# rmcar17/SpectralClusterSupertree

Hardware: AMD Instinct MI355X
Metric: top-level PCG build + Fiedler solve wall-time (s) at N taxa, 1/2/4/8 MI355X (lower is better)
Workload: dtype f64 (loop operator: fp32 image of W; fp64 renewal + confirmation)

## Files before the change

include/scs_hip.h:

```cpp
#ifndef SCS_HIP_H
#define SCS_HIP_H

#include <stddef.h>
#include <stdint.h>

#ifdef __cplusplus
extern "C" {
#endif

#define SCS_OK 0
#define SCS_EINVAL (-1)
#define SCS_EHIP (-2)
#define SCS_ENOMEM (-3)
#define SCS_ECOMM (-4)
#define SCS_ENOCONV (-5)
#define SCS_EUNSUP (-6)

#define SCS_UNIQUE_ID_BYTES 128

typedef struct scs_ctx scs_ctx;
typedef struct scs_tables scs_tables;
typedef struct scs_graph scs_graph;

typedef struct scs_stats {
    int32_t n_vertices;
    int32_t block;
    int32_t iterations;
    int32_t n_apply;
    int32_t converged;
    int32_t used_constraint;
    double lambda[2];
    double resid[2];
    double lambda_next;
    double apply_ms_total;
    double apply_ms_min;
    double solve_ms;
    double apply_bytes;
    double allgather_ms_total;
    double allgather_bytes;
    int32_t n_allgather;
    int32_t n_apply32;
    double apply32_ms_total;
    double apply32_bytes;
    int32_t lowp_renewals;
    int32_t reserved;
    double event_pair_ms;
} scs_stats;

typedef struct scs_build_stats {
    int32_t n_taxa;
    int32_t n_trees;
    int32_t row_begin, row_end;
    int32_t symmetric;
    int32_t n_tiles;
    int32_t n_batches;
    int32_t spec_batches;
    double cell_trees;
    double prep_ms;
    double accumulate_ms;
    double exchange_ms;
    double total_ms;
    double bytes_w;
    double bytes_tables;
    double exchange_bytes;
    int32_t tree_parallel_batches;
    int32_t spec_trees;
    double spec_ms;
    int32_t listed_batches;
    int32_t reserved;
} scs_build_stats;

int scs_version(void);
const char *scs_last_error(void);

int scs_device_count(void);


int scs_comm_unique_id(void *out128);

int scs_ctx_create(int device, int rank, int world, const void *unique_id128, scs_ctx **out);

typedef struct scs_local_group scs_local_group;
int scs_local_group_create(int world, scs_local_group **out);
int scs_local_group_destroy(scs_local_group *group);
int scs_ctx_create_local(int device, int rank, scs_local_group *group, scs_ctx **out);

int scs_ctx_destroy(scs_ctx *ctx);
int scs_ctx_synchronize(scs_ctx *ctx);
int scs_ctx_trim(scs_ctx *ctx, int64_t keep_bytes);
int scs_ctx_reserve(scs_ctx *ctx, int64_t bytes);
int scs_debug_arena_stats(int device, int64_t *out8);
int scs_ctx_comm_info(scs_ctx *ctx, int32_t *kind, int32_t *world, int32_t *rank,
                      int32_t *reported_world, int32_t *reported_rank);


typedef struct scs_forest scs_forest;
typedef struct scs_forest_info {
    int32_t n_trees;
    int32_t monotone;
    int64_t n_nodes;
    int64_t n_leaves;
} scs_forest_info;

int scs_forest_upload(scs_ctx *ctx, int32_t n_taxa, int32_t n_trees, const int64_t *node_off,
                      const int32_t *parent, const int32_t *taxon, const double *length,
                      const double *support, const double *weights, int64_t n_leaves, scs_forest **out);
int scs_forest_free(scs_ctx *ctx, scs_forest *forest);

int scs_forest_split(scs_ctx *ctx, const scs_forest *forest, const int32_t *part_of,
                     const int32_t *new_id, int32_t n_parts, const int32_t *part_taxa, int32_t strategy,
                     scs_forest **out_forests, scs_forest_info *info);

int scs_forest_tables_download(scs_ctx *ctx, const scs_forest *forest, int64_t *tree_off,
                               int32_t *leaf_taxon, int32_t *adj_depth, double *adj_val,
                               int32_t *tree_index, double *tree_w, uint8_t *present);

int scs_forest_tables_host(scs_ctx *ctx, const scs_forest *forest, const int64_t **tree_off,
                           const int32_t **leaf_taxon, const int32_t **adj_depth, const double **adj_val,
                           const int32_t **tree_index, const double **tree_w, const uint8_t **present);

int scs_forest_download(scs_ctx *ctx, const scs_forest *forest, int32_t t_begin, int32_t t_end,
                        int64_t *node_off, int32_t *parent, int32_t *taxon, double *length,
                        double *support, double *weights);

int scs_tables_from_forest(scs_ctx *ctx, const scs_forest *forest, const int32_t *relabel, int32_t n_taxa,
                           scs_tables **out);


int scs_forest_split_level(scs_ctx *ctx, const scs_forest *forest, const int32_t *part_of,
                           const int32_t *new_id, int32_t n_parts, int32_t child_taxa, int32_t strategy,
                           int32_t n_nodes, const int32_t *node_tree_end, scs_forest **out_union,
                           scs_forest_info *info, int32_t *child_trees, int64_t *child_leaves,
                           uint8_t *present, int32_t *comp_root, uint64_t *sig);

int scs_forest_slice(scs_ctx *ctx, const scs_forest *forest, int32_t t_begin, int32_t t_end, scs_forest **out);

int scs_forest_analyze(scs_ctx *ctx, const scs_forest *forest, int32_t *comp_root, uint64_t *sig);

int scs_forest_tables_download_range(scs_ctx *ctx, const scs_forest *forest, int32_t t_begin, int32_t t_end,
                                     int64_t *tree_off, int32_t *leaf_taxon, int32_t *adj_depth,
                                     double *adj_val, double *tree_w);

int scs_tables_from_forest_range(scs_ctx *ctx, const scs_forest *forest, int32_t t_begin, int32_t t_end,
                                 int32_t u_base, int32_t u_size, const int32_t *relabel, int32_t n_taxa,
                                 scs_tables **out);


int scs_host_alloc(size_t bytes, void **out);
int scs_host_free(void *p);

int scs_tables_upload(scs_ctx *ctx, int32_t n_taxa, int32_t n_trees, const int64_t *tree_off,
                      const int32_t *leaf_taxon, const int32_t *adj_depth, const double *adj_val,
                      const double *tree_w, scs_tables **out);
int scs_tables_free(scs_ctx *ctx, scs_tables *tables);


int scs_score_supertree(scs_ctx *ctx, const scs_tables *sources, int32_t n_nodes, const int32_t *parent,
                        const int32_t *taxon, int32_t max_batch_trees, int64_t *n_super, int64_t *n_source,
                        int64_t *shared, int64_t *informative, int64_t *supported);

int scs_score_parsimony(scs_ctx *ctx, const scs_tables *sources, int32_t n_nodes, const int32_t *parent,
                        const int32_t *taxon, int32_t max_batch_trees, int32_t max_pass_words, int64_t *mrp_chars,
                        int64_t *mrp_length, int64_t *mrp_perfect, int64_t *mrp_max, int64_t *char_off,
                        int32_t *char_len, int32_t *char_lo, int32_t *char_hi);

int scs_score_triplets(scs_ctx *ctx, const scs_tables *sources, int32_t n_nodes, const int32_t *parent,
                       const int32_t *taxon, int32_t max_batch_trees, int64_t *t_super, int64_t *t_source,
                       int64_t *t_shared);

int scs_score_conflicts(scs_ctx *ctx, const scs_tables *sources, int32_t n_nodes, const int32_t *parent,
                        const int32_t *taxon, int32_t max_batch_trees, int64_t *n_super_conflict,
                        int64_t *n_source_conflict, int64_t *conflicting);

int scs_score_concordance(scs_ctx *ctx, const scs_tables *sources, int32_t n_nodes, const int32_t *parent,
                          const int32_t *taxon, int32_t max_batch_trees, int64_t *n_decisive, int64_t *n_concordant,
                          int64_t *n_alternative, int64_t *decisive, int64_t *concordant, int64_t *alt1,
                          int64_t *alt2);

int scs_score_branch_triplets(scs_ctx *ctx, const scs_tables *sources, int32_t n_nodes, const int32_t *parent,
                              const int32_t *taxon, int32_t max_batch_trees, int64_t *n_bt_total,
                              int64_t *n_bt_concordant, int64_t *n_bt_alternative, int64_t *bt_total,
                              int64_t *bt_concordant, int64_t *bt_alt1, int64_t *bt_alt2);

int scs_score_taxon_triplets(scs_ctx *ctx, const scs_tables *sources, int32_t n_nodes, const int32_t *parent,
                             const int32_t *taxon, int32_t max_batch_trees, int32_t max_lds_bytes,
                             int64_t *tx_trees, int64_t *tx_total, int64_t *tx_super, int64_t *tx_source,
                             int64_t *tx_shared);

int scs_score_placements(scs_ctx *ctx, const scs_tables *sources, int32_t n_nodes, const int32_t *parent,
                         const int32_t *taxon, int32_t max_batch_trees, int32_t max_lds_bytes, int32_t n_queries,
                         const int32_t *queries, int64_t *pl_trees, int64_t *pl_total, int64_t *pl_source,
                         int64_t *pl_super, int64_t *pl_shared);

int scs_score_clade_placements(scs_ctx *ctx, const scs_tables *sources, int32_t n_nodes, const int32_t *parent,
                               const int32_t *taxon, int32_t max_batch_trees, int32_t max_lds_bytes,
                               int32_t n_queries, const int32_t *query_nodes, int64_t *cp_trees, int64_t *cp_total,
                               int64_t *cp_source, int64_t *cp_super, int64_t *cp_shared);

int scs_score_clade_moves(scs_ctx *ctx, const scs_tables *sources, int32_t n_nodes, const int32_t *parent,
                          const int32_t *taxon, int32_t max_batch_trees, int32_t max_lds_bytes, int32_t n_queries,
                          const int32_t *query_nodes, int32_t top_k, int64_t *cp_trees, int64_t *cp_total,
                          int64_t *cp_source, int64_t *mv_own_super, int64_t *mv_own_shared, int32_t *mv_node,
                          int64_t *mv_super, int64_t *mv_shared);

int scs_score_polytomies(scs_ctx *ctx, const scs_tables *sources, int32_t n_nodes, const int32_t *parent,
                         const int32_t *taxon, int32_t max_batch_trees, int32_t max_lds_bytes, int32_t n_queries,
                         const int32_t *query_nodes, int32_t *py_degree, int64_t *py_trees, int64_t *py_total,
                         int64_t *py_joint);

int scs_score_branch_resample(scs_ctx *ctx, const scs_tables *sources, int32_t n_nodes, const int32_t *parent,
                              const int32_t *taxon, int32_t max_batch_trees, int32_t n_rep, const int32_t *weights,
                              int64_t *rs_point, int32_t *rs_wins, int64_t *rs_rows);


#define SCS_BUILD_MONOTONE 1
#define SCS_BUILD_SHARED 2
#define SCS_BUILD_UPPER 4
#define SCS_BUILD_SCATTER 8
int scs_pcg_build(scs_ctx *ctx, const scs_tables *tables, int32_t row_begin, int32_t row_end,
                  int32_t flags, scs_graph **out, scs_build_stats *stats);

int scs_graph_contract(scs_ctx *ctx, scs_graph *graph, const int32_t *group_start,
                       int32_t n_groups, scs_graph **out);

int scs_graph_shape(const scs_graph *graph, int32_t *n_vertices, int32_t *row_begin,
                    int32_t *row_end);

int scs_graph_download(scs_ctx *ctx, const scs_graph *graph, double *out);

int scs_graph_download_rows(scs_ctx *ctx, const scs_graph *graph, int32_t first, int32_t count,
                            double *out);

int scs_graph_degrees(scs_ctx *ctx, scs_graph *graph, double *out);

int scs_graph_free(scs_ctx *ctx, scs_graph *graph);


int scs_fiedler(scs_ctx *ctx, scs_graph *graph, const double *x_init, double tol,
                int32_t max_iter, int32_t block, double *maps_out, scs_stats *stats);

int scs_graph_matrix_free(scs_ctx *ctx, const scs_tables *tables, int32_t max_block, scs_graph **out);


int scs_small_solve(scs_ctx *ctx, int32_t n_nodes, const int32_t *n_taxa, const int32_t *n_trees,
                    const int32_t *n_groups, const int32_t *tree_off, const int32_t *leaf_taxon,
                    const int32_t *adj_depth, const double *adj_val, const double *tree_w,
                    const int32_t *group_start, double *maps_out, double *lambda_out,
                    double *w_out);

int scs_small_solve_begin(scs_ctx *ctx, int32_t n_nodes, const int32_t *n_taxa,
                          const int32_t *n_trees, const int32_t *n_groups, const int32_t *tree_off,
                          const int32_t *leaf_taxon, const int32_t *adj_depth, const double *adj_val,
                          const double *tree_w, const int32_t *group_start, int32_t want_w,
                          int32_t *ticket_out);
int scs_small_solve_begin_forest(scs_ctx *ctx, const scs_forest *forest, const int32_t *relabel,
                                 int32_t n_taxa, int32_t n_groups, const int32_t *group_start,
                                 int32_t want_w, int32_t *ticket_out);
int scs_small_solve_begin_level(scs_ctx *ctx, const scs_forest *forest, int32_t n_nodes,
                                const int32_t *t_begin, const int32_t *n_trees, const int64_t *n_leaves,
                                const int32_t *u_base, const int32_t *u_size, const int32_t *relabel,
                                const int32_t *n_taxa, const int32_t *n_groups, const int32_t *group_start,
                                int32_t want_w, int32_t *ticket_out);
int scs_small_solve_end(scs_ctx *ctx, int32_t ticket, double *maps_out, double *lambda_out,
                        double *w_out);


int scs_debug_loop_policy(double tol, int32_t lowp_mode, double lowp_tol, double lowp_tol2, int32_t image,
                          int32_t n, const double *residuals, int32_t *actions_out);

int scs_debug_jacobi(scs_ctx *ctx, const double *a, int32_t n, double *w, double *v);

int scs_debug_gram(scs_ctx *ctx, const double *a, const double *b, int32_t n, int32_t ka,
                   int32_t kb, int32_t use_mfma, double *out);

int scs_debug_apply(scs_ctx *ctx, scs_graph *graph, const double *x, int32_t b, double *y);

int scs_debug_apply_ex(scs_ctx *ctx, scs_graph *graph, const double *x, int32_t b, int32_t image,
                       int32_t reps, double *y_out, int32_t *info_out);

int scs_debug_gram_ex(scs_ctx *ctx, const double *a, int32_t lda, int32_t a_col0, int32_t ka,
                      const double *b, int32_t ldb, int32_t b_col0, int32_t kb, int32_t n,
                      int32_t use_mfma, int32_t gram_blocks, double *out);

int scs_debug_update(scs_ctx *ctx, double *y, int32_t ldy, int32_t y_col0, int32_t kc, double alpha,
                     const double *a, int32_t lda, int32_t a_col0, int32_t ka, const double *c,
                     int32_t ldc, double sign, int32_t n);

int scs_debug_comm_selftest(scs_ctx *ctx, int32_t count, const double *host_in, double *host_out);

int scs_debug_copy_bandwidth(scs_ctx *ctx, int64_t bytes, int32_t reps, double *gbs_out);

int scs_debug_scan(scs_ctx *ctx, int32_t op, int32_t n_parts, int64_t n, const int32_t *in, int32_t *out);

int scs_debug_graph_raw(scs_ctx *ctx, scs_graph *graph, int32_t what, void *out, int32_t *info_out);

int scs_debug_split_plan(int32_t n_trees, const int64_t *node_off, int32_t *tpb_out, int32_t *n_groups_out,
                         uint8_t *staged_out);

int scs_debug_score_plan(const scs_tables *sources, int32_t n_trees, const int64_t *tree_off, int32_t super_leaves,
                         int32_t max_batch_trees, int64_t extra_per_leaf, int64_t extra_per_tree,
                         int32_t *n_batches_out, int32_t *bstart_out, int64_t *info_out, int32_t *words_out,
                         int32_t *zb_out, int64_t *wg_out);

int scs_debug_branch_plan(const scs_tables *sources, int32_t n_trees, const int64_t *tree_off, int32_t super_leaves,
                          int32_t max_batch_trees, int64_t extra_per_leaf, int64_t extra_per_tree,
                          int32_t max_lds_bytes, int32_t *n_batches_out, int32_t *bstart_out, int64_t *bt_out,
                          int64_t *tx_out, int64_t *call_out);

int scs_debug_placement_plan(const scs_tables *sources, int32_t n_trees, const int64_t *tree_off, int32_t super_leaves,
                             int32_t max_batch_trees, int32_t max_lds_bytes, int32_t n_queries,
                             int32_t n_sub_queries, int32_t n_degrees, const int32_t *degrees, int32_t *n_batches_out,
                             int32_t *bstart_out, int64_t *pl_out, int64_t *cp_out, int64_t *blk_out, int64_t *py_out);

int scs_debug_parsimony_plan(const scs_tables *sources, int32_t n_trees, const int64_t *tree_off, const int64_t *chars,
                             int32_t n_nodes, const int32_t *parent, int32_t max_batch_trees, int32_t max_pass_words,
                             int32_t *n_batches_out, int32_t *bstart_out, int64_t *info_out, int64_t *batch_out);

#ifdef __cplusplus
}
#endif
#endif
```

spectralclustersupertree_amd/_native.py:

```python

from __future__ import annotations

import ctypes as C
from pathlib import Path

import numpy as np

_PKG = Path(__file__).resolve().parent
LIB_PATH = _PKG / "libscs_hip.so"

UNIQUE_ID_BYTES = 128
BUILD_MONOTONE = 1
BUILD_SHARED = 2
BUILD_UPPER = 4
BUILD_SCATTER = 8


class ScsError(RuntimeError):

    def __init__(self, code: int, message: str) -> None:
        super().__init__(f"libscs_hip error {code}: {message}")
        self.code = code


EINVAL = -1
ENOMEM = -3
ENOCONV = -5
EUNSUP = -6


class ConvergenceError(ScsError):

    def __init__(self, message: str, maps, stats: dict) -> None:
        super().__init__(ENOCONV, message)
        self.maps = maps
        self.stats = stats


class Stats(C.Structure):
    _fields_ = [
        ("n_vertices", C.c_int32),
        ("block", C.c_int32),
        ("iterations", C.c_int32),
        ("n_apply", C.c_int32),
        ("converged", C.c_int32),
        ("used_constraint", C.c_int32),
        ("lambda_", C.c_double * 2),
        ("resid", C.c_double * 2),
        ("lambda_next", C.c_double),
        ("apply_ms_total", C.c_double),
        ("apply_ms_min", C.c_double),
        ("solve_ms", C.c_double),
        ("apply_bytes", C.c_double),
        ("allgather_ms_total", C.c_double),
        ("allgather_bytes", C.c_double),
        ("n_allgather", C.c_int32),
        ("n_apply32", C.c_int32),
        ("apply32_ms_total", C.c_double),
        ("apply32_bytes", C.c_double),
        ("lowp_renewals", C.c_int32),
        ("reserved", C.c_int32),
        ("event_pair_ms", C.c_double),
    ]

    def as_dict(self) -> dict:
        out = {}
        for name, _ in self._fields_:
            v = getattr(self, name)
            out[name.rstrip("_")] = list(v) if hasattr(v, "__len__") else v
        return out


class ForestInfo(C.Structure):
    _fields_ = [
        ("n_trees", C.c_int32),
        ("monotone", C.c_int32),
        ("n_nodes", C.c_int64),
        ("n_leaves", C.c_int64),
    ]


class BuildStats(C.Structure):
    _fields_ = [
        ("n_taxa", C.c_int32),
        ("n_trees", C.c_int32),
        ("row_begin", C.c_int32),
        ("row_end", C.c_int32),
        ("symmetric", C.c_int32),
        ("n_tiles", C.c_int32),
        ("n_batches", C.c_int32),
        ("spec_batches", C.c_int32),
        ("cell_trees", C.c_double),
        ("prep_ms", C.c_double),
        ("accumulate_ms", C.c_double),
        ("exchange_ms", C.c_double),
        ("total_ms", C.c_double),
        ("bytes_w", C.c_double),
        ("bytes_tables", C.c_double),
        ("exchange_bytes", C.c_double),
        ("tree_parallel_batches", C.c_int32),
        ("spec_trees", C.c_int32),
        ("spec_ms", C.c_double),
        ("listed_batches", C.c_int32),
        ("reserved", C.c_int32),
    ]

    def as_dict(self) -> dict:
        return {name: getattr(self, name) for name, _ in self._fields_}


_P = C.c_void_p
_PP = C.POINTER(C.c_void_p)
_I32 = C.c_int32
_DP = _IP = _LP = C.c_void_p
ABI_VERSION = 109

SIGNATURES = {
    "scs_version": (C.c_int, []),
    "scs_last_error": (C.c_char_p, []),
    "scs_device_count": (C.c_int, []),
    "scs_comm_unique_id": (C.c_int, [_P]),
    "scs_ctx_create": (C.c_int, [C.c_int, C.c_int, C.c_int, _P, _PP]),
    "scs_local_group_create": (C.c_int, [C.c_int, _PP]),
    "scs_local_group_destroy": (C.c_int, [_P]),
    "scs_ctx_create_local": (C.c_int, [C.c_int, C.c_int, _P, _PP]),
    "scs_ctx_destroy": (C.c_int, [_P]),
    "scs_ctx_synchronize": (C.c_int, [_P]),
    "scs_ctx_trim": (C.c_int, [_P, C.c_int64]),
    "scs_debug_arena_stats": (C.c_int, [C.c_int, C.POINTER(C.c_int64)]),
    "scs_ctx_reserve": (C.c_int, [_P, C.c_int64]),
    "scs_ctx_comm_info": (C.c_int, [_P, _P, _P, _P, _P, _P]),
    "scs_forest_upload": (C.c_int, [_P, _I32, _I32, _LP, _IP, _IP, _DP, _DP, _DP, C.c_int64, _PP]),
    "scs_forest_free": (C.c_int, [_P, _P]),
    "scs_forest_split": (C.c_int, [_P, _P, _IP, _IP, _I32, _IP, _I32, _P, _P]),
    "scs_forest_tables_download": (C.c_int, [_P, _P, _LP, _IP, _IP, _DP, _IP, _DP, _P]),
    "scs_forest_tables_host": (C.c_int, [_P, _P, _P, _P, _P, _P, _P, _P, _P]),
    "scs_tables_from_forest": (C.c_int, [_P, _P, _IP, _I32, _PP]),
    "scs_forest_download": (C.c_int, [_P, _P, _I32, _I32, _LP, _IP, _IP, _DP, _DP, _DP]),
    "scs_forest_split_level": (C.c_int, [_P, _P, _IP, _IP, _I32, _I32, _I32, _I32, _IP, _PP, _P, _IP, _LP, _P, _IP, _P]),
    "scs_forest_analyze": (C.c_int, [_P, _P, _IP, _P]),
    "scs_forest_slice": (C.c_int, [_P, _P, _I32, _I32, _PP]),
    "scs_forest_tables_download_range": (C.c_int, [_P, _P, _I32, _I32, _LP, _IP, _IP, _DP, _DP]),
    "scs_tables_from_forest_range": (C.c_int, [_P, _P, _I32, _I32, _I32, _I32, _IP, _I32, _PP]),
    "scs_small_solve_begin_level": (C.c_int, [_P, _P, _I32, _IP, _IP, _LP, _IP, _IP, _IP, _IP, _IP, _IP, _I32,
                                              C.POINTER(C.c_int32)]),
    "scs_host_alloc": (C.c_int, [C.c_size_t, _PP]),
    "scs_host_free": (C.c_int, [_P]),
    "scs_tables_upload": (C.c_int, [_P, _I32, _I32, _LP, _IP, _IP, _DP, _DP, _PP]),
    "scs_tables_free": (C.c_int, [_P, _P]),
    "scs_score_supertree": (C.c_int, [_P, _P, _I32, _IP, _IP, _I32, _LP, _LP, _LP, _LP, _LP]),
    "scs_score_triplets": (C.c_int, [_P, _P, _I32, _IP, _IP, _I32, _LP, _LP, _LP]),
    "scs_score_conflicts": (C.c_int, [_P, _P, _I32, _IP, _IP, _I32, _LP, _LP, _LP]),
    "scs_score_concordance": (C.c_int, [_P, _P, _I32, _IP, _IP, _I32, _LP, _LP, _LP, _LP, _LP, _LP, _LP]),
    "scs_score_branch_triplets": (C.c_int, [_P, _P, _I32, _IP, _IP, _I32, _LP, _LP, _LP, _LP, _LP, _LP, _LP]),
    "scs_score_taxon_triplets": (C.c_int, [_P, _P, _I32, _IP, _IP, _I32, _I32, _LP, _LP, _LP, _LP, _LP]),
    "scs_score_placements": (C.c_int, [_P, _P, _I32, _IP, _IP, _I32, _I32, _I32, _IP, _LP, _LP, _LP, _LP, _LP]),
    "scs_score_clade_placements": (C.c_int, [_P, _P, _I32, _IP, _IP, _I32, _I32, _I32, _IP, _LP, _LP, _LP, _LP, _LP]),
    "scs_score_clade_moves": (C.c_int, [_P, _P, _I32, _IP, _IP, _I32, _I32, _I32, _IP, _I32, _LP, _LP, _LP, _LP, _LP,
                                        _IP, _LP, _LP]),
    "scs_score_polytomies": (C.c_int, [_P, _P, _I32, _IP, _IP, _I32, _I32, _I32, _IP, _IP, _LP, _LP, _LP]),
    "scs_score_branch_resample": (C.c_int, [_P, _P, _I32, _IP, _IP, _I32, _I32, _IP, _LP, _IP, _LP]),
    "scs_score_parsimony": (C.c_int, [_P, _P, _I32, _IP, _IP, _I32, _I32, _LP, _LP, _LP, _LP, _LP, _IP, _IP, _IP]),
    "scs_pcg_build": (C.c_int, [_P, _P, _I32, _I32, _I32, _PP, C.POINTER(BuildStats)]),
    "scs_graph_contract": (C.c_int, [_P, _P, _IP, _I32, _PP]),
    "scs_graph_matrix_free": (C.c_int, [_P, _P, _I32, _PP]),
    "scs_graph_shape": (C.c_int, [_P, _IP, _IP, _IP]),
    "scs_graph_download": (C.c_int, [_P, _P, _DP]),
    "scs_graph_download_rows": (C.c_int, [_P, _P, _I32, _I32, _DP]),
    "scs_graph_degrees": (C.c_int, [_P, _P, _DP]),
    "scs_graph_free": (C.c_int, [_P, _P]),
    "scs_fiedler": (C.c_int, [_P, _P, _DP, C.c_double, _I32, _I32, _DP, C.POINTER(Stats)]),
    "scs_small_solve": (C.c_int, [_P, _I32, _IP, _IP, _IP, _IP, _IP, _IP, _DP, _DP, _IP, _DP, _DP, _DP]),
    "scs_small_solve_begin": (C.c_int, [_P, _I32, _IP, _IP, _IP, _IP, _IP, _IP, _DP, _DP, _IP, _I32,
                                        C.POINTER(C.c_int32)]),
    "scs_small_solve_begin_forest": (C.c_int, [_P, _P, _IP, _I32, _I32, _IP, _I32, _P]),
    "scs_small_solve_end": (C.c_int, [_P, _I32, _DP, _DP, _DP]),
    "scs_debug_loop_policy": (C.c_int, [C.c_double, _I32, C.c_double, C.c_double, _I32, _I32, _DP, _IP]),
    "scs_debug_jacobi": (C.c_int, [_P, _DP, _I32, _DP, _DP]),
    "scs_debug_gram": (C.c_int, [_P, _DP, _DP, _I32, _I32, _I32, _I32, _DP]),
    "scs_debug_apply": (C.c_int, [_P, _P, _DP, _I32, _DP]),
    "scs_debug_apply_ex": (C.c_int, [_P, _P, _DP, _I32, _I32, _I32, _DP, _IP]),
    "scs_debug_gram_ex": (C.c_int, [_P, _DP, _I32, _I32, _I32, _DP, _I32, _I32, _I32, _I32, _I32, _I32, _DP]),
    "scs_debug_update": (C.c_int, [_P, _DP, _I32, _I32, _I32, C.c_double, _DP, _I32, _I32, _I32, _DP, _I32,
                                   C.c_double, _I32]),
    "scs_debug_comm_selftest": (C.c_int, [_P, _I32, _DP, _DP]),
    "scs_debug_copy_bandwidth": (C.c_int, [_P, C.c_int64, _I32, _DP]),
    "scs_debug_scan": (C.c_int, [_P, _I32, _I32, C.c_int64, _IP, _IP]),
    "scs_debug_split_plan": (C.c_int, [_I32, _LP, _P, _P, _P]),
    "scs_debug_graph_raw": (C.c_int, [_P, _P, _I32, _P, _IP]),
    "scs_debug_score_plan": (C.c_int, [_P, _I32, _LP, _I32, _I32, C.c_int64, C.c_int64, _P, _IP, _LP, _IP, _IP, _LP]),
    "scs_debug_branch_plan": (C.c_int, [_P, _I32, _LP, _I32, _I32, C.c_int64, C.c_int64, _I32, _P, _IP, _LP, _LP, _LP]),
    "scs_debug_placement_plan": (C.c_int, [_P, _I32, _LP, _I32, _I32, _I32, _I32, _I32, _I32, _IP, _IP, _IP, _LP, _LP,
                                           _LP, _LP]),
    "scs_debug_parsimony_plan": (C.c_int, [_P, _I32, _LP, _LP, _I32, _IP, _I32, _I32, _P, _IP, _LP, _LP]),
}

_lib = None


def load_library() -> C.CDLL:
    global _lib
    if _lib is not None:
        return _lib
    if not LIB_PATH.exists():
        msg = (
            f"{LIB_PATH} not found: build it with `python -c 'import __graft_entry__ as g; g.build()'` "
            "or `make -C spectralclustersupertree_amd/csrc`.  There is no CPU fallback."
        )
        raise ImportError(msg)
    lib = C.CDLL(str(LIB_PATH))
    for name, (restype, argtypes) in SIGNATURES.items():
        fn = getattr(lib, name)
        fn.restype = restype
        fn.argtypes = argtypes
    have = int(lib.scs_version())
    if have != ABI_VERSION:
        msg = f"{LIB_PATH} reports ABI version {have}, this package binds {ABI_VERSION}: rebuild the library"
        raise ImportError(msg)
    _lib = lib
    return lib


def check(rc: int) -> None:
    if rc != 0:
        msg = load_library().scs_last_error()
        raise ScsError(rc, msg.decode() if msg else "unknown error")


class _PinnedBlock:

    def __init__(self, nbytes: int) -> None:
        self._lib = load_library()
        self.ptr = C.c_void_p()
        check(self._lib.scs_host_alloc(nbytes, C.byref(self.ptr)))
        self.nbytes = nbytes

    def __del__(self) -> None:
        try:
            if self.ptr:
                self._lib.scs_host_free(self.ptr)
                self.ptr = C.c_void_p()
        except Exception:
            pass


def pinned_empty(shape, dtype) -> np.ndarray:
    dt = np.dtype(dtype)
    count = int(np.prod(shape)) if np.ndim(shape) else int(shape)
    block = _PinnedBlock(max(count * dt.itemsize, 1))
    buf = (C.c_char * block.nbytes).from_address(block.ptr.value)
    buf._scs_owner = block
    return np.frombuffer(buf, dtype=dt, count=count).reshape(shape)


def dptr(a: np.ndarray):
    assert a.dtype == np.float64
    return a.ctypes.data


def iptr(a: np.ndarray):
    assert a.dtype == np.int32
    return a.ctypes.data


def lptr(a: np.ndarray):
    assert a.dtype == np.int64
    return a.ctypes.data
```

spectralclustersupertree_amd/backend.py:

```python

from __future__ import annotations

import ctypes as C
import os

import numpy as np

from spectralclustersupertree_amd import _env
from spectralclustersupertree_amd import _native as nv
from spectralclustersupertree_amd.flatten import TreeTables

DEFAULT_TOL = 1e-13
DEFAULT_MAX_ITER = 2000

_M, _N, _Q, _QN, _QK = ("m",), ("n_nodes",), ("nq",), ("nq", "n_nodes"), ("nq", "top_k")


def _resident_solve() -> bool:
    return bool(int(_env.probe("SCS_RESIDENT_SOLVE", "1")))


class Device:

    def __init__(self, device: int = 0, rank: int = 0, world: int = 1, unique_id: bytes | None = None,
# ... 435 lines not shown
        return comp_root, sig

    def tables_range(self, t_begin: int, t_end: int):
        m = int(t_end - t_begin)
        tree_off = np.zeros(m + 1, dtype=np.int64)
        nv.check(self.dev._lib.scs_forest_tables_download_range(self.dev._ctx, self._h, int(t_begin), int(t_end),
                                                                nv.lptr(tree_off), None, None, None, None))
        l = int(tree_off[-1])
        leaf_taxon = np.empty(l, dtype=np.int32)
        adj_depth = np.empty(l, dtype=np.int32)
        adj_val = np.empty(l, dtype=np.float64)
        tree_w = np.empty(m, dtype=np.float64)
        nv.check(self.dev._lib.scs_forest_tables_download_range(
            self.dev._ctx, self._h, int(t_begin), int(t_end), nv.lptr(tree_off), nv.iptr(leaf_taxon) if l else None,
            nv.iptr(adj_depth) if l else None, nv.dptr(adj_val) if l else None, nv.dptr(tree_w) if m else None))
        return tree_off, leaf_taxon, adj_depth, adj_val, tree_w

    def tables(self):
        m, l = self.n_trees, self.n_leaves
        ptrs = [C.c_void_p() for _ in range(7)]
        nv.check(self.dev._lib.scs_forest_tables_host(self.dev._ctx, self._h, *[C.byref(x) for x in ptrs]))

        def view(ptr, dtype, count):
            dt = np.dtype(dtype)
            if count == 0:
                return np.empty(0, dtype=dt)
            buf = (C.c_char * (count * dt.itemsize)).from_address(ptr.value)
            buf._scs_owner = self
            a = np.frombuffer(buf, dtype=dt, count=count)
            a.flags.writeable = False
            return a

        return (view(ptrs[0], np.int64, m + 1), view(ptrs[1], np.int32, l), view(ptrs[2], np.int32, l),
                view(ptrs[3], np.float64, l), view(ptrs[4], np.int32, m), view(ptrs[5], np.float64, m),
                view(ptrs[6], np.uint8, max(self.n_taxa, 0)))

    def download(self, t_begin: int = 0, t_end: int | None = None):
        t_end = self.n_trees if t_end is None else t_end
        m = t_end - t_begin
        node_off = np.zeros(m + 1, dtype=np.int64)
        nv.check(self.dev._lib.scs_forest_download(self.dev._ctx, self._h, t_begin, t_end, nv.lptr(node_off),
                                                   None, None, None, None, None))
        n = int(node_off[-1])
        parent = np.empty(n, dtype=np.int32)
        taxon = np.empty(n, dtype=np.int32)
        length = np.empty(n, dtype=np.float64)
        support = np.empty(n, dtype=np.float64)
        weights = np.empty(m, dtype=np.float64)
        nv.check(self.dev._lib.scs_forest_download(self.dev._ctx, self._h, t_begin, t_end, nv.lptr(node_off),
                                                   nv.iptr(parent) if n else None, nv.iptr(taxon) if n else None,
                                                   nv.dptr(length) if n else None, nv.dptr(support) if n else None,
                                                   nv.dptr(weights) if m else None))
        return node_off, parent, taxon, length, support, weights


def debug_split_plan(node_off: np.ndarray):
    node_off = np.ascontiguousarray(node_off, dtype=np.int64)
    m = len(node_off) - 1
    tpb, groups = C.c_int32(0), C.c_int32(0)
    staged = np.zeros((m + 7) // 8 + 1, dtype=np.uint8)
    nv.check(nv.load_library().scs_debug_split_plan(m, nv.lptr(node_off), C.byref(tpb), C.byref(groups), staged.ctypes.data))
    return int(tpb.value), staged[: groups.value].astype(bool)


def debug_score_plan(sources, super_leaves: int, batch_trees: int = 0, extra_per_leaf: int = 0,
                     extra_per_tree: int = 0) -> dict:
    handle, off = (sources._h, None) if isinstance(sources, DeviceTables) else (None, sources)
    if off is not None:
        off = np.ascontiguousarray(off, dtype=np.int64)
    m = sources.n_trees if off is None else len(off) - 1
    nb = C.c_int32(0)
    bstart = np.zeros(m + 1, dtype=np.int32)
    info = np.zeros(2, dtype=np.int64)
    words, zb = np.zeros(max(m, 1), dtype=np.int32), np.zeros(max(m, 1), dtype=np.int32)
    wg = np.zeros(max(m, 1), dtype=np.int64)
    nv.check(nv.load_library().scs_debug_score_plan(
        handle, m, None if off is None else nv.lptr(off), int(super_leaves), int(batch_trees), int(extra_per_leaf),
        int(extra_per_tree), C.byref(nb), nv.iptr(bstart), nv.lptr(info), nv.iptr(words), nv.iptr(zb), nv.lptr(wg)))
    k = int(nb.value)
    return {"bstart": bstart[: k + 1].astype(np.int64), "levels": int(info[0]), "row_stride": int(info[1]),
            "words": words[:k].astype(np.int64), "zb": zb[:k].astype(np.int64), "workgroups": wg[:k].copy()}


def debug_branch_plan(sources, super_leaves: int, batch_trees: int = 0, extra_per_leaf: int = 0,
                      extra_per_tree: int = 0, lds_bytes: int = 0) -> dict:
    handle, off = (sources._h, None) if isinstance(sources, DeviceTables) else (None, sources)
    if off is not None:
        off = np.ascontiguousarray(off, dtype=np.int64)
    m = sources.n_trees if off is None else len(off) - 1
    nb = C.c_int32(0)
    bstart = np.zeros(m + 1, dtype=np.int32)
    bt = np.zeros((max(m, 1), 4), dtype=np.int64)
    tx = np.zeros((max(m, 1), 14), dtype=np.int64)
    call = np.zeros(3, dtype=np.int64)
    nv.check(nv.load_library().scs_debug_branch_plan(
        handle, m, None if off is None else nv.lptr(off), int(super_leaves), int(batch_trees), int(extra_per_leaf),
        int(extra_per_tree), int(lds_bytes), C.byref(nb), nv.iptr(bstart), nv.lptr(bt), nv.lptr(tx), nv.lptr(call)))
    k = int(nb.value)
    bins = tx[:k, :12].reshape(k, 3, 4)
    return {"bstart": bstart[: k + 1].astype(np.int64), "bt_words": bt[:k, 0].copy(), "bt_zb": bt[:k, 1].copy(),
            "bt_lds": bt[:k, 2].copy(), "bt_workgroups": bt[:k, 3].copy(), "tx_zb": bins[:, :, 0].copy(),
            "tx_dcap": bins[:, :, 1].copy(), "tx_lds": bins[:, :, 2].copy(), "tx_workgroups": bins[:, :, 3].copy(),
            "tx_slab_launch": tx[:k, 12].copy(), "tx_slab_lds": tx[:k, 13].copy(), "need_slab": int(call[0]),
            "slab_wgs": int(call[1]),
            "slab_stride": int(call[2])}


def debug_placement_plan(sources, super_leaves: int, batch_trees: int = 0, lds_bytes: int = 0, n_queries: int = 1,
                         n_sub_queries: int = 1, degrees=()) -> dict:
    handle, off = (sources._h, None) if isinstance(sources, DeviceTables) else (None, sources)
    if off is not None:
        off = np.ascontiguousarray(off, dtype=np.int64)
    m = sources.n_trees if off is None else len(off) - 1
    deg = np.ascontiguousarray(degrees, dtype=np.int32)
    nb = np.zeros(3, dtype=np.int32)
    bstart = np.zeros((3, m + 1), dtype=np.int32)
    pair = np.zeros((2, max(m, 1), 6), dtype=np.int64)
    blk = np.zeros((2, m + 1), dtype=np.int64)
    py = np.zeros((max(m, 1), max(len(deg), 1), 4), dtype=np.int64)
    nv.check(nv.load_library().scs_debug_placement_plan(
        handle, m, None if off is None else nv.lptr(off), int(super_leaves), int(batch_trees), int(lds_bytes),
        int(n_queries), int(n_sub_queries), len(deg), nv.iptr(deg) if len(deg) else None, nv.iptr(nb),
        nv.iptr(bstart), nv.lptr(pair[0]), nv.lptr(pair[1]), nv.lptr(blk), nv.lptr(py)))
    out = {}
    for x, name in enumerate(("pl", "cp")):
        k = int(nb[x])
        out[f"{name}_bstart"] = bstart[x, : k + 1].astype(np.int64)
        for i, key in enumerate(("words", "zb", "sums", "lds_full", "lds_last", "workgroups")):
            out[f"{name}_{key}"] = pair[x, :k, i].copy()
        out[f"{name}_blk"] = np.diff(blk[x])
    k = int(nb[2])
    out["py_bstart"] = bstart[2, : k + 1].astype(np.int64)
    rows = py.reshape(-1)[: k * len(deg) * 4].reshape(k, len(deg), 4)
    for i, key in enumerate(("words", "stride", "acc_lds", "lds")):
        out[f"py_{key}"] = rows[:, :, i].copy()
    return out


def debug_parsimony_plan(sources, parent, chars=None, batch_trees: int = 0, pass_words: int = 0) -> dict:
    handle, off = (sources._h, None) if isinstance(sources, DeviceTables) else (None, sources)
    if off is not None:
        off = np.ascontiguousarray(off, dtype=np.int64)
    m = sources.n_trees if off is None else len(off) - 1
    parent = np.ascontiguousarray(parent, dtype=np.int32)
    if chars is not None:
        chars = np.ascontiguousarray(chars, dtype=np.int64)
        if chars.shape != (m,):
            msg = f"chars must have one entry per source tree ({m}), not shape {chars.shape}"
            raise ValueError(msg)
    nb = C.c_int32(0)
    bstart = np.zeros(m + 1, dtype=np.int32)
    info = np.zeros(8, dtype=np.int64)
    rows = np.zeros((max(m, 1), 2), dtype=np.int64)
    nv.check(nv.load_library().scs_debug_parsimony_plan(
        handle, m, None if off is None else nv.lptr(off), None if chars is None else nv.lptr(chars), len(parent),
        nv.iptr(parent), int(batch_trees), int(pass_words), C.byref(nb), nv.iptr(bstart), nv.lptr(info),
        nv.lptr(rows)))
    k = int(nb.value)
    keys = ("pass_words", "frame_depth", "counter_bits", "lds_bytes", "frames_in_block", "extra_per_leaf",
            "extra_per_tree", "super_tips")
    return {"bstart": bstart[: k + 1].astype(np.int64), "passes": rows[:k, 0].copy(), "words": rows[:k, 1].copy(),
            **{key: int(info[i]) for i, key in enumerate(keys)}}


_FAIL_SMALL_FOR_TESTS = False


def _refuse_nonfinite_maps(maps: np.ndarray, lam: np.ndarray, n_groups: np.ndarray) -> None:
    if np.isfinite(maps).all():
        return
    at = 0
    for i, v in enumerate(n_groups):
        if not np.isfinite(maps[at:at + int(v)]).all():
            lam[i] = np.nan
        at += int(v)


class SmallTicket:

    def __init__(self, dev: Device, ticket: int, n_groups: np.ndarray, want_w: bool, nodes=None) -> None:
        self.dev, self._ticket, self._n_groups, self._want_w = dev, ticket, n_groups, want_w
        self._nodes = nodes
        self._out = None

    def _general_path(self, i: int):
        tables, group_start = self._nodes[i]
        dtab = self.dev.upload(tables)
        try:
            graph = dtab.build()
        finally:
            dtab.free()
        try:
            if group_start is not None:
                graph = graph.contract(group_start)
            last = None
            widths = [(b, it) for b, it in ((4, DEFAULT_MAX_ITER), (8, 4 * DEFAULT_MAX_ITER)) if graph.shape[0] > 3 * b + 2]
            for block, iters in widths or [(0, 4 * DEFAULT_MAX_ITER)]:
                try:
                    maps, stats = graph.fiedler(None, block=block, max_iter=iters)
                    lam = np.array([stats["lambda"][0], stats["lambda"][1], stats["lambda_next"]])
                    return maps, lam, (graph.download() if self._want_w else None)
                except nv.ConvergenceError as exc:
                    last = exc
            msg = f"small-node eigen-solve did not converge, nor did the general path ({last})"
            raise RuntimeError(msg)
        finally:
            graph.free()

    def raw(self):
        n_groups = self._n_groups
        maps = np.empty((int(n_groups.sum()), 2))
        lam = np.empty((len(n_groups), 3))
        ticket, self._ticket = self._ticket, -1
        nv.check(self.dev._lib.scs_small_solve_end(self.dev._ctx, ticket, nv.dptr(maps), nv.dptr(lam), None))
        _refuse_nonfinite_maps(maps, lam, n_groups)
        return maps, lam

    def result(self):
        if self._out is None:
            n_groups, want_w = self._n_groups, self._want_w
            k = len(n_groups)
            maps = np.empty((int(n_groups.sum()), 2))
            lam = np.empty((k, 3))
            w = np.empty(int((n_groups.astype(np.int64) ** 2).sum())) if want_w else None
            ticket, self._ticket = self._ticket, -1
            nv.check(self.dev._lib.scs_small_solve_end(self.dev._ctx, ticket, nv.dptr(maps), nv.dptr(lam),
                                                       nv.dptr(w) if want_w else None))
            redo = {}
            _refuse_nonfinite_maps(maps, lam, n_groups)
            if _FAIL_SMALL_FOR_TESTS:
                lam[n_groups > 64] = np.nan
            if not np.all(np.isfinite(lam)):
                bad = [i for i in range(k) if not np.all(np.isfinite(lam[i]))]
                if self._nodes is None:
                    msg = f"small-node eigen-solve did not converge (nodes {bad} of a batch of {k})"
                    raise RuntimeError(msg)
                for i in bad:
                    redo[i] = self._general_path(i)
            out, at, wat = [], 0, 0
            for i in range(k):
                v = int(n_groups[i])
                if i in redo:
                    item = (redo[i][0], redo[i][1]) + ((redo[i][2],) if want_w else ())
                else:
                    item = (maps[at:at + v], lam[i])
                    if want_w:
                        item += (w[wat:wat + v * v].reshape(v, v),)
                if want_w:
                    wat += v * v
                out.append(item)
                at += v
            self._nodes = None
            self._out = out
        return self._out

    def __del__(self) -> None:
        try:
            if self._ticket >= 0 and self.dev._ctx:
                self.dev._lib.scs_small_solve_end(self.dev._ctx, self._ticket, None, None, None)
        except Exception:
            pass


class DeviceTables:
    def __init__(self, dev: Device, handle, n_taxa: int, n_trees: int, monotone: bool = False) -> None:
        self.dev, self._h = dev, handle
        self.n_taxa, self.n_trees = n_taxa, n_trees
        self.monotone = monotone

    def free(self) -> None:
        if self._h:
            self.dev._lib.scs_tables_free(self.dev._ctx, self._h)
            self._h = C.c_void_p()

    def __del__(self) -> None:
        try:
            self.free()
        except Exception:
            pass

    def build(self, row_begin: int = 0, row_end: int | None = None,
              shared: bool | None = None, upper: bool = False, scatter: bool = False) -> "DeviceGraph":
        if row_end is None:
            row_end = self.n_taxa
        handle = C.c_void_p()
        stats = nv.BuildStats()
        flags = nv.BUILD_MONOTONE if self.monotone else 0
        if upper:
            flags |= nv.BUILD_UPPER
            shared = False
        if scatter:
            flags |= nv.BUILD_SCATTER
            shared = False
        if shared is None:
            shared = self.dev.world > 1
        if shared:
            flags |= nv.BUILD_SHARED
        nv.check(self.dev._lib.scs_pcg_build(self.dev._ctx, self._h, row_begin, row_end, flags,
                                             C.byref(handle), C.byref(stats)))
        graph = DeviceGraph(self.dev, handle, stats.as_dict())
        graph.upper = bool(upper)
        return graph


    def matrix_free_graph(self, max_block: int = 8) -> "DeviceGraph":
        handle = C.c_void_p()
        nv.check(self.dev._lib.scs_graph_matrix_free(self.dev._ctx, self._h, int(max_block), C.byref(handle)))
        return DeviceGraph(self.dev, handle, {})


class DeviceGraph:
    def __init__(self, dev: Device, handle, build_stats: dict | None = None) -> None:
        self.dev, self._h = dev, handle
        self.build_stats = build_stats or {}
        self.upper = False

    def free(self) -> None:
        if self._h:
            self.dev._lib.scs_graph_free(self.dev._ctx, self._h)
            self._h = C.c_void_p()

    def __del__(self) -> None:
        try:
            self.free()
        except Exception:
            pass

    @property
    def shape(self) -> tuple[int, int, int]:
        n, rb, re_ = C.c_int32(), C.c_int32(), C.c_int32()
        nv.check(self.dev._lib.scs_graph_shape(self._h, C.byref(n), C.byref(rb), C.byref(re_)))
        return n.value, rb.value, re_.value

    def contract(self, group_start: np.ndarray) -> "DeviceGraph":
        gs = np.ascontiguousarray(group_start, dtype=np.int32)
        handle = C.c_void_p()
        nv.check(self.dev._lib.scs_graph_contract(self.dev._ctx, self._h, nv.iptr(gs), len(gs) - 1,
                                                  C.byref(handle)))
        self._h = C.c_void_p()
        return DeviceGraph(self.dev, handle, self.build_stats)

    def download(self) -> np.ndarray:
        n, rb, re_ = self.shape
        out = np.empty((re_ - rb, n))
        nv.check(self.dev._lib.scs_graph_download(self.dev._ctx, self._h, nv.dptr(out)))
        return out

    def download_rows(self, first: int, count: int) -> np.ndarray:
        out = np.empty((count, self.shape[0]))
        nv.check(self.dev._lib.scs_graph_download_rows(self.dev._ctx, self._h, first, count,
                                                       nv.dptr(out)))
        return out

    def degrees(self) -> np.ndarray:
        n, rb, re_ = self.shape
        out = np.empty(re_ - rb)
        nv.check(self.dev._lib.scs_graph_degrees(self.dev._ctx, self._h, nv.dptr(out)))
        return out

    def apply(self, x: np.ndarray) -> np.ndarray:
        x = np.ascontiguousarray(x, dtype=np.float64)
        n, rb, re_ = self.shape
        y = np.empty((re_ - rb, x.shape[1]))
        nv.check(self.dev._lib.scs_debug_apply(self.dev._ctx, self._h, nv.dptr(x), x.shape[1],
                                               nv.dptr(y)))
        return y

    APPLY_INFO = ("symmetric", "image", "tiles", "segments", "tile_width", "n_apply32", "partial", "matrix_free")

    def apply_ex(self, x: np.ndarray, image: bool = False, reps: int = 1):
        x = np.ascontiguousarray(x, dtype=np.float64)
        n, rb, re_ = self.shape
        y = np.empty((reps, re_ - rb, x.shape[1]))
        info = np.zeros(8, dtype=np.int32)
        nv.check(self.dev._lib.scs_debug_apply_ex(self.dev._ctx, self._h, nv.dptr(x), x.shape[1], int(image),
                                                  int(reps), nv.dptr(y), nv.iptr(info)))
        return y, dict(zip(self.APPLY_INFO, (int(v) for v in info)))

    def raw(self, what: int = 0):
        if what not in (0, 1):
            msg = f"DeviceGraph.raw: what must be 0 (W) or 1 (image), not {what!r}"
            raise ValueError(msg)
        info = np.zeros(4, dtype=np.int32)
        nv.check(self.dev._lib.scs_debug_graph_raw(self.dev._ctx, self._h, int(what), None, nv.iptr(info)))
        rows, ld = int(info[0]), int(info[1])
        out = np.empty((rows, ld), dtype=np.float32 if what else np.float64)
        nv.check(self.dev._lib.scs_debug_graph_raw(self.dev._ctx, self._h, int(what), out.ctypes.data, nv.iptr(info)))
        rb = self.shape[1]
        first = (np.zeros(rows, dtype=np.int64) if (not what or info[3])
                 else (rb + np.arange(rows, dtype=np.int64)) // 512 * 512)
        return out, {"rows": rows, "ld": ld, "col0": int(info[2]), "first_col": first}

    def degrees_all(self) -> np.ndarray:
        info = np.zeros(4, dtype=np.int32)
        out = np.empty(self.shape[0])
        nv.check(self.dev._lib.scs_debug_graph_raw(self.dev._ctx, self._h, 2, out.ctypes.data, nv.iptr(info)))
        return out

    def fiedler(self, x_init: np.ndarray | None = None, tol: float = DEFAULT_TOL,
                max_iter: int = DEFAULT_MAX_ITER, block: int = 0):
        n = self.shape[0]
        maps = np.empty((n, 2))
        stats = nv.Stats()
        x0 = None
        if x_init is not None:
            x_init = np.ascontiguousarray(x_init, dtype=np.float64)
            if x_init.shape != (n,):
                msg = f"x_init must have shape ({n},)"
                raise ValueError(msg)
            x0 = nv.dptr(x_init)
        rc = self.dev._lib.scs_fiedler(self.dev._ctx, self._h, x0, tol, max_iter, block,
                                       nv.dptr(maps), C.byref(stats))
        if rc == nv.ENOCONV:
            msg = self.dev._lib.scs_last_error()
            raise nv.ConvergenceError(msg.decode() if msg else "not converged", maps, stats.as_dict())
        nv.check(rc)
        return maps, stats.as_dict()
```

spectralclustersupertree_amd/csrc/scs_build.hip:

```cpp

#include <algorithm>

#include "scs_internal.h"

typedef unsigned long long u64;
typedef unsigned int u32;

constexpr u32 DEPTH_INF = 0xFFFFFFFFu;


__device__ __forceinline__ void rmq_offsets(int m, int a, int b, int (&o)[2]) {
    const int k = 31 - __clz(b - a);
    o[0] = k * m + a;
    o[1] = k * m + b - (1 << k);
}

template <typename K>
__device__ __forceinline__ K rmq_min(const K *__restrict__ base, int m, int a, int b) {
    int o[2];
    rmq_offsets(m, a, b, o);
    const K x = base[o[0]], y = base[o[1]];
    return x < y ? x : y;
}

__global__ void k_positions_values(const int64_t *__restrict__ tree_off,
                                   const int32_t *__restrict__ leaf_taxon,
                                   const int32_t *__restrict__ adj_depth,
                                   const double *__restrict__ adj_val,
                                   const double *__restrict__ tree_w, int t0,
                                   int32_t *__restrict__ pos, int64_t npad,
                                   const int64_t *__restrict__ st_off, double *__restrict__ stv) {
    const int tl = blockIdx.y;
    const int t = t0 + tl;
    const int64_t off = tree_off[t];
    const int n = (int)(tree_off[t + 1] - off);
    const int p = blockIdx.x * blockDim.x + threadIdx.x;
    if (p >= n) return;
    const unsigned tx = (unsigned)leaf_taxon[off + p];
    if (tx < (unsigned)npad) pos[(int64_t)tl * npad + tx] = p;
    if (p < n - 1)
        stv[st_off[tl] + p] = adj_depth[off + p] ? adj_val[off + p] * tree_w[t] : 0.0;
}

template <typename K>
__global__ void k_sparse_level(const int64_t *__restrict__ tree_off, int t0, int k,
                               const int64_t *__restrict__ st_off, K *__restrict__ st) {
    const int tl = blockIdx.y;
    const int m = (int)(tree_off[t0 + tl + 1] - tree_off[t0 + tl]) - 1;
    const int p = blockIdx.x * blockDim.x + threadIdx.x;
    if (m < (1 << k) || p > m - (1 << k)) return;
    K *base = st + st_off[tl];
    const K a = base[(int64_t)(k - 1) * m + p], b = base[(int64_t)(k - 1) * m + p + (1 << (k - 1))];
    base[(int64_t)k * m + p] = a < b ? a : b;
}

template <typename K, typename MIN>
__global__ __launch_bounds__(1024) void k_sparse_levels_fused(const int64_t *__restrict__ tree_off, int t0,
                                                               const int64_t *__restrict__ st_off,
                                                               K *__restrict__ st, MIN pick) {
    const int tl = blockIdx.x;
    const int m = (int)(tree_off[t0 + tl + 1] - tree_off[t0 + tl]) - 1;
    K *base = st + st_off[tl];
    for (int k = 1; (1 << k) <= m; ++k) {
        const K *prev = base + (int64_t)(k - 1) * m;
        K *cur = base + (int64_t)k * m;
        const int half = 1 << (k - 1), last = m - (1 << k);
        for (int p = threadIdx.x; p <= last; p += 1024) cur[p] = pick(prev[p], prev[p + half]);
        __syncthreads();
    }
}
constexpr int SPARSE_FUSED_MAX_LEAVES = 32768;
struct pick_smaller_value {
    __device__ double operator()(double a, double b) const { return a < b ? a : b; }
};

__device__ __forceinline__ double min_f64(double a, double b) {
#ifdef SCS_MIN_ASM
    double r;
    asm("v_min_f64 %0, %1, %2" : "=v"(r) : "v"(a), "v"(b));
    return r;
#else
    return __builtin_fmin(a, b);
#endif
}

#include "scs_mono.h"
#include "scs_mono_wide.h"
#include "scs_gen.h"
struct pick_shallower_pair {
    __device__ gap_entry operator()(const gap_entry a, const gap_entry b) const { return gap_min(a, b); }
};

__global__ __launch_bounds__(256) void k_scatter_atomic(const int64_t *__restrict__ tree_off,
                                                         const int32_t *__restrict__ leaf_taxon, int t0,
                                                         const int64_t *__restrict__ st_off,
                                                         const double *__restrict__ stv,
                                                         double *__restrict__ w, int64_t ld) {
    const int tl = blockIdx.y;
    const int64_t off = tree_off[t0 + tl];
    const int nl = (int)(tree_off[t0 + tl + 1] - off);
    const int m = nl - 1;
    const int nbk = (nl + 63) / 64;
    int I = 0, rest = blockIdx.x;
    while (I < nbk && rest >= nbk - I) {
        rest -= nbk - I;
        ++I;
    }
    if (I >= nbk) return;
    const int J = I + rest;
    __shared__ int s_ta[64], s_tb[64];
    const int tid = threadIdx.x;
    if (tid < 64) s_ta[tid] = I * 64 + tid < nl ? leaf_taxon[off + I * 64 + tid] : -1;
    else if (tid < 128) s_tb[tid - 64] = J * 64 + tid - 64 < nl ? leaf_taxon[off + J * 64 + tid - 64] : -1;
    __syncthreads();
    const double *st = stv + st_off[tl];
    const int bj = tid & 63;
    const int pb = J * 64 + bj;
#pragma unroll 4
    for (int q = 0; q < 16; ++q) {
        const int ai = (tid >> 6) + 4 * q;
        const int pa = I * 64 + ai;
        if (pa >= pb || pb >= nl) continue;
        const double v = rmq_min<double>(st, m, pa, pb);
        if (v != 0.0) {
            const int ta = s_ta[ai], tb2 = s_tb[bj];
            atomicAdd(&w[(int64_t)ta * ld + tb2], v);
            atomicAdd(&w[(int64_t)tb2 * ld + ta], v);
        }
    }
}

__global__ __launch_bounds__(1024) void k_unpack_tiles(const double *__restrict__ gathered,
                                                      const int2 *__restrict__ tiles, int world,
                                                      int64_t chunk_doubles, int n, int row_begin,
                                                      int row_end, double *__restrict__ w,
                                                      int64_t ld) {
    const int tcw = blockDim.x;
    const int t = blockIdx.x;
    const int2 tile = tiles[t];
    const double *src = gathered + (int64_t)(t % world) * chunk_doubles +
                        (int64_t)(t / world) * SCS_TR * tcw;
    const int c = tile.y * tcw + threadIdx.x;
    if (c >= n) return;
    const int r0 = tile.x * SCS_TR;
    const bool col_is_my_row = c >= row_begin && c < row_end;
    for (int i = 0; i < SCS_TR; ++i) {
        const int r = r0 + i;
        if (r >= n) break;
        const double v = src[i * tcw + threadIdx.x];
        if (r >= row_begin && r < row_end) w[(int64_t)(r - row_begin) * ld + c] = v;
        if (col_is_my_row && ((r / tcw) + 1) * tcw <= (c / SCS_TR) * SCS_TR)
            w[(int64_t)(c - row_begin) * ld + r] = v;
    }
}

__global__ __launch_bounds__(256) void k_pack_tiles(const double *__restrict__ tile_out,
                                                    const int32_t *__restrict__ src_slot, int tcw,
                                                    double *__restrict__ sendbuf) {
    const double2 *src = (const double2 *)(tile_out + (int64_t)src_slot[blockIdx.x] * SCS_TR * tcw);
    double2 *dst = (double2 *)(sendbuf + (int64_t)blockIdx.x * SCS_TR * tcw);
    for (int q = threadIdx.x; q < SCS_TR * tcw / 2; q += 256) dst[q] = src[q];
}

__global__ __launch_bounds__(1024) void k_unpack_received(const double *__restrict__ recvbuf,
                                                         const int2 *__restrict__ tiles, int n,
                                                         int row_begin, int row_end,
                                                         double *__restrict__ w, int64_t ld) {
    const int tcw = blockDim.x;
    const int2 tile = tiles[blockIdx.x];
    const double *src = recvbuf + (int64_t)blockIdx.x * SCS_TR * tcw;
    const int c = tile.y * tcw + threadIdx.x;
    if (c >= n) return;
    const int r0 = tile.x * SCS_TR;
    const bool col_is_my_row = c >= row_begin && c < row_end;
    for (int i = 0; i < SCS_TR; ++i) {
        const int r = r0 + i;
        if (r >= n) break;
        const double v = src[i * tcw + threadIdx.x];
        if (r >= row_begin && r < row_end) w[(int64_t)(r - row_begin) * ld + c] = v;
        if (col_is_my_row && ((r / tcw) + 1) * tcw <= (c / SCS_TR) * SCS_TR)
            w[(int64_t)(c - row_begin) * ld + r] = v;
    }
}

__global__ void k_contract(const double *__restrict__ w, int64_t ld, int old_row_begin,
                           const int32_t *__restrict__ gstart, int g_begin, int g_end, int n_groups,
                           double *__restrict__ out, int64_t ld_out) {
    const int h = blockIdx.x * blockDim.x + threadIdx.x;
    if (h >= n_groups) return;
    const int c0 = gstart[h], c1 = gstart[h + 1];
    for (int g = g_begin + blockIdx.y; g < g_end; g += gridDim.y) {
        double best = 0.0;
        if (h != g) {
            const int r0 = gstart[g], r1 = gstart[g + 1];
            best = w[(int64_t)(r0 - old_row_begin) * ld + c0];
            for (int r = r0; r < r1; ++r)
                for (int c = c0; c < c1; ++c) {
                    const double v = w[(int64_t)(r - old_row_begin) * ld + c];
                    best = v > best ? v : best;
                }
        }
        out[(int64_t)(g - g_begin) * ld_out + h] = best;
    }
}

template <bool IMG>
__global__ __launch_bounds__(256) void k_degrees(const double *__restrict__ w, int64_t ld, int n,
                                                  int rows, int row_begin,
                                                  double *__restrict__ deg_full,
                                                  float *__restrict__ w32 = nullptr, int w32_full = 0) {
    const int lane = threadIdx.x & 63;
    const int r = blockIdx.x * 4 + (threadIdx.x >> 6);
    if (r >= rows) return;
    const double *row = w + (int64_t)r * ld;
    double s0 = 0.0, s1 = 0.0;
    const int n2 = n & ~1;
    const int c0 = w32_full ? 0 : (row_begin + r) / 512 * 512;
    float *row32 = IMG ? w32 + (int64_t)r * ld : nullptr;
    for (int j = lane * 2; j < n2; j += 128) {
        const double2 v = *(const double2 *)(row + j);
        s0 += v.x;
        s1 += v.y;
        if (IMG && j >= c0) *(float2 *)(row32 + j) = make_float2((float)v.x, (float)v.y);
    }
    if (IMG)
        for (int j = n2 + lane; j < ld; j += 64) row32[j] = (float)row[j];
    if ((n & 1) && lane == 0) s0 += row[n - 1];
    double s = s0 + s1;
#pragma unroll
    for (int o = 32; o > 0; o >>= 1) s += __shfl_xor(s, o, 64);
    if (lane == 0) deg_full[row_begin + r] = s;
}

__global__ __launch_bounds__(256) void k_degrees_upper_rows(const double *__restrict__ w, int64_t ld, int n,
                                                             int rows, int row_begin, int col0,
                                                             double *__restrict__ part) {
    const int lane = threadIdx.x & 63;
    const int rl = blockIdx.x * 4 + (threadIdx.x >> 6);
    if (rl >= rows) return;
    const int r = row_begin + rl;
    const int c0 = r / 256 * 256;
    const double *row = w + (int64_t)rl * ld + (c0 - col0);
    const int cnt = n - c0;
    double s0 = 0.0, s1 = 0.0;
    const int n2 = cnt & ~1;
    for (int j = lane * 2; j < n2; j += 128) {
        const double2 v = *(const double2 *)(row + j);
        s0 += v.x;
        s1 += v.y;
    }
    if ((cnt & 1) && lane == 0) s0 += row[cnt - 1];
    double s = s0 + s1;
#pragma unroll
    for (int o = 32; o > 0; o >>= 1) s += __shfl_xor(s, o, 64);
    if (lane == 0) part[r] = s;
}

__global__ __launch_bounds__(256) void k_degrees_upper_cols(const double *__restrict__ w, int64_t ld, int n,
                                                             int row_begin, int row_end, int col0,
                                                             double *__restrict__ part) {
    const int c = col0 + blockIdx.x * blockDim.x + threadIdx.x;
    if (c >= n) return;
    const int r_end = min(row_end, c / 256 * 256);
    double s = 0.0;
    for (int r = row_begin; r < r_end; ++r) s += w[(int64_t)(r - row_begin) * ld + (c - col0)];
    if (r_end > row_begin) part[c] += s;
}

__global__ void k_combine_degrees(const double *__restrict__ gathered, int world, int n,
                                  double *__restrict__ deg) {
    const int i = blockIdx.x * blockDim.x + threadIdx.x;
    if (i >= n) return;
    double d = 0.0;
    for (int r = 0; r < world; ++r) d += gathered[(int64_t)r * n + i];
    deg[i] = d;
}

__global__ void k_dinv(const double *__restrict__ deg, int n, double *__restrict__ dinv) {
    const int i = blockIdx.x * blockDim.x + threadIdx.x;
    if (i >= n) return;
    const double d = deg[i];
    dinv[i] = d == 0.0 ? 1.0 : 1.0 / sqrt(d);
}

namespace {

struct dev_buf {
    scs_ctx *ctx;
    void *p = nullptr;
    explicit dev_buf(scs_ctx *c) : ctx(c) {}
    ~dev_buf() {
        if (p) scs_dev_free(p);
    }
    int alloc(size_t bytes) {
        if (p) scs_dev_free(p);
        p = nullptr;
        SCS_HIP_CHECK(scs_dev_malloc(ctx, &p, bytes ? bytes : 16));
        return SCS_OK;
    }
};

struct cached_buf {
    scs_ctx *ctx;
    void *p = nullptr;
    explicit cached_buf(scs_ctx *c) : ctx(c) {}
    ~cached_buf() {
        if (p) scs_block_release(ctx, p);
    }
    int alloc(size_t bytes) {
        if (p) scs_block_release(ctx, p);
        p = nullptr;
        return scs_block_alloc(ctx, bytes, &p);
    }
};

struct pooled_buf {
    scs_ctx *ctx = nullptr;
    int slot = 0;
    void *p = nullptr;
    pooled_buf(scs_ctx *c, int s) : ctx(c), slot(s) {}
    ~pooled_buf() {
        auto &sl = ctx->scratch[slot];
        if (sl.cap > SCS_SCRATCH_KEEP) {
            scs_dev_free(sl.p);
            sl.p = nullptr;
            sl.cap = 0;
        }
    }
    int alloc(size_t bytes) {
        auto &sl = ctx->scratch[slot];
        if (bytes < 16) bytes = 16;
        if (sl.cap < bytes) {
            if (sl.p) scs_dev_free(sl.p);
            sl.p = nullptr;
            sl.cap = 0;
            SCS_HIP_CHECK(scs_dev_malloc(ctx, &sl.p, bytes));
            sl.cap = bytes;
        }
        p = sl.p;
        return SCS_OK;
    }
};

struct ev_pair {
    hipEvent_t a = nullptr, b = nullptr;
    ~ev_pair() {
        if (a) hipEventDestroy(a);
        if (b) hipEventDestroy(b);
    }
    int init() {
        SCS_HIP_CHECK(hipEventCreate(&a));
        SCS_HIP_CHECK(hipEventCreate(&b));
        return SCS_OK;
    }
};

int levels_for(int64_t m) {
    int l = 0;
    while (((int64_t)1 << l) <= m) ++l;
    return l;
}

}

static int graph_alloc(scs_ctx *ctx, int32_t n, int32_t row_begin, int32_t row_end,
                       hipStream_t stream, scs_graph **out, int32_t col0 = 0) {
    auto *g = new scs_graph();
    g->n = n;
    g->row_begin = row_begin;
    g->row_end = row_end;
    g->col0 = col0;
    g->upper = col0 > 0 || false;
    g->ld = scs_round_up(n - col0, SCS_LD_ALIGN);
    const size_t rows = (size_t)(row_end - row_begin);
    size_t bytes = rows * (size_t)g->ld * sizeof(double);
    if (bytes < 16) bytes = 16;
    {
        const int rc = scs_block_alloc(ctx, bytes, (void **)&g->d_w);
        if (rc != SCS_OK) {
            delete g;
            return rc;
        }
        g->w_bytes = bytes;
        g->w_block = true;
    }
    if (g->ld > n - col0) {
        hipError_t e = hipMemset2DAsync(g->d_w + (n - col0), (size_t)g->ld * 8, 0,
                                        (size_t)(g->ld - (n - col0)) * 8, rows, stream);
        if (e != hipSuccess) {
            if (g->w_block) scs_block_release(ctx, g->d_w);
            else scs_dev_free(g->d_w);
            delete g;
            scs_set_error("cannot clear the padding of W: %s", hipGetErrorString(e));
            return SCS_EHIP;
        }
    }
    *out = g;
    return SCS_OK;
}

extern "C" int scs_graph_free(scs_ctx *ctx, scs_graph *g) {
    if (!g) return SCS_OK;
    if (ctx) hipSetDevice(ctx->device);
    if (g->mf) {
        if (ctx) hipStreamSynchronize(ctx->stream);
        scs_matfree_release(g);
    }
    if (ctx && g->d_w && g->w_block) {
        scs_block_release(ctx, g->d_w);
    } else if (ctx && g->d_w) {
        if (!ctx->w_cache || g->w_bytes >= ctx->w_cache_bytes) {
            if (ctx->w_cache) scs_dev_free(ctx->w_cache);
            ctx->w_cache = g->d_w;
            ctx->w_cache_bytes = g->w_bytes;
        } else {
            scs_dev_free(g->d_w);
        }
    } else {
        scs_dev_free(g->d_w);
    }
    if (ctx && g->deg_stage) {
        hipStreamSynchronize(ctx->stream);
        scs_pinned_release(ctx, g->deg_stage);
    }
    if (ctx) {
        if (g->d_w32) {
            std::lock_guard<std::mutex> lock(ctx->cache_mu);
            if (scs_dbg("SCS_TRACE_SOLVES") && atoi(scs_dbg("SCS_TRACE_SOLVES")) && ctx->w32_cache)
                fprintf(stderr, "[image] hipFree of %.2f GB\n",
                        std::min(g->w32_bytes, ctx->w32_cache_bytes) / 1073741824.0);
            scs_dev_free(g->d_w32);
        }
        if (g->d_deg) scs_block_release(ctx, g->d_deg);
        if (g->d_dinv) scs_block_release(ctx, g->d_dinv);
    } else {
        scs_dev_free(g->d_w32);
        scs_dev_free(g->d_deg);
        scs_dev_free(g->d_dinv);
    }
    delete g;
    return SCS_OK;
}

extern "C" int scs_graph_shape(const scs_graph *g, int32_t *n, int32_t *rb, int32_t *re) {
    SCS_REQUIRE(g != nullptr, "scs_graph_shape: null graph");
    if (n) *n = g->n;
    if (rb) *rb = g->row_begin;
    if (re) *re = g->row_end;
    return SCS_OK;
}

int scs_gather_row_splits(scs_ctx *ctx, int32_t row_begin, int32_t row_end, int32_t n,
                          std::vector<int32_t> &splits) {
    const int world = ctx->comm.world;
    splits.assign(world + 1, 0);
    if (world == 1) {
        splits[0] = row_begin;
        splits[1] = row_end;
        return SCS_OK;
    }
    dev_buf send(ctx), recv(ctx);
    SCS_TRY(send.alloc(8));
    SCS_TRY(recv.alloc(8 * (size_t)world));
    double v = (double)row_begin;
    SCS_HIP_CHECK(hipMemcpyAsync(send.p, &v, 8, hipMemcpyHostToDevice, ctx->stream));
    SCS_TRY(scs_comm_allgather_f64(&ctx->comm, (const double *)send.p, (double *)recv.p, 1, ctx->stream));
    std::vector<double> h(world);
    SCS_HIP_CHECK(hipMemcpyAsync(h.data(), recv.p, 8 * (size_t)world, hipMemcpyDeviceToHost, ctx->stream));
    SCS_HIP_CHECK(hipStreamSynchronize(ctx->stream));
    for (int r = 0; r < world; ++r) splits[r] = (int32_t)h[r];
    splits[world] = n;
    for (int r = 0; r < world; ++r)
        SCS_REQUIRE(splits[r] < splits[r + 1], "row partition is not contiguous by rank");
    SCS_REQUIRE(splits[0] == 0 && splits[ctx->comm.rank] == row_begin && splits[ctx->comm.rank + 1] == row_end,
                "row partition does not tile [0, V)");
    return SCS_OK;
}

__global__ __launch_bounds__(64) void k_col_presence(const int32_t *__restrict__ pos, int64_t npad, int n,
                                                      int cols_per_group, int n_batch,
                                                      unsigned char *__restrict__ pcol) {
    const int cg = blockIdx.x, t = blockIdx.y, lane = threadIdx.x;
    bool any = false;
    for (int c = cg * cols_per_group + lane; c < min(n, (cg + 1) * cols_per_group); c += 64)
        any = any || pos[(int64_t)t * npad + c] >= 0;
    if (__ballot(any) != 0 && lane == 0) pcol[(int64_t)cg * n_batch + t] = 1;
    if (__ballot(any) == 0 && lane == 0) pcol[(int64_t)cg * n_batch + t] = 0;
}

__global__ void k_tile_lists(const int2 *__restrict__ tiles, int n_tiles, const unsigned char *__restrict__ rec,
                             int rec_bytes, int cnt_off, int n_batch, const unsigned char *__restrict__ pcol,
                             int32_t *__restrict__ lists, int32_t *__restrict__ list_cnt) {
    const int i = blockIdx.x * blockDim.x + threadIdx.x;
    if (i >= n_tiles) return;
    const int2 tile = tiles[i];
    const unsigned char *rb = rec + (int64_t)tile.x * n_batch * rec_bytes + cnt_off;
    const unsigned char *pc = pcol + (int64_t)tile.y * n_batch;
    int32_t *out = lists + (int64_t)i * n_batch;
    int c = 0;
    for (int t = 0; t < n_batch; ++t)
        if (pc[t] && *(const int *)(rb + (int64_t)t * rec_bytes) > 0) out[c++] = t;
    list_cnt[i] = c;
}

extern "C" int scs_pcg_build(scs_ctx *ctx, const scs_tables *tb, int32_t row_begin,
                             int32_t row_end, int32_t flags, scs_graph **out,
                             scs_build_stats *stats) {
    SCS_REQUIRE(ctx && tb && out, "scs_pcg_build: null argument");
    SCS_REQUIRE((flags & ~(SCS_BUILD_MONOTONE | SCS_BUILD_SHARED | SCS_BUILD_UPPER | SCS_BUILD_SCATTER)) == 0,
                "scs_pcg_build: unknown flag bits 0x%x", flags);
    const bool scatter = (flags & SCS_BUILD_SCATTER) != 0;
    if (scatter && tb) SCS_TRY(scs_tables_finish(ctx, tb));
    if (scatter) {
        if (!(flags & SCS_BUILD_MONOTONE) || (flags & (SCS_BUILD_SHARED | SCS_BUILD_UPPER)) ||
            row_begin != 0 || row_end != tb->n_taxa || ctx->comm.world != 1) {
            scs_set_error("scs_pcg_build: SCS_BUILD_SCATTER (the atomic comparison variant) takes monotone "
                          "tables, the whole matrix, one rank");
            return SCS_EUNSUP;
        }
    }
    SCS_REQUIRE((flags & (SCS_BUILD_SHARED | SCS_BUILD_UPPER)) != (SCS_BUILD_SHARED | SCS_BUILD_UPPER),
                "scs_pcg_build: SCS_BUILD_SHARED and SCS_BUILD_UPPER exclude each other");
    const bool monotone = (flags & SCS_BUILD_MONOTONE) != 0 &&
                          !(scs_dbg("SCS_NO_MONOTONE") && atoi(scs_dbg("SCS_NO_MONOTONE")));
    const int n = tb->n_taxa;
    SCS_REQUIRE(row_begin >= 0 && row_begin < row_end && row_end <= n,
                "scs_pcg_build: bad row range [%d, %d) for %d taxa", row_begin, row_end, n);
    SCS_HIP_CHECK(hipSetDevice(ctx->device));
    hipStream_t s = ctx->stream;
    const int world = ctx->comm.world, rank = ctx->comm.rank;
    const int cols_per_tile = MONO_TCW;
    static_assert(MONO_TCW == SCS_TCW, "one tile width for all kernels");
    const size_t entry_bytes = monotone ? 8 : sizeof(gap_entry);
    size_t rec_bytes = monotone ? R3_BYTES : G3_BYTES;
    const int n_cgroups = (n + cols_per_tile - 1) / cols_per_tile;
    const int64_t npad = scs_round_up((int64_t)n_cgroups * cols_per_tile, SCS_NPAD);
    bool shared = (flags & SCS_BUILD_SHARED) != 0 && world > 1;
    if (shared) {
        const int64_t nb_all = (n + SCS_TR - 1) / SCS_TR;
        const double tile_bytes = 0.5 * (double)nb_all * n_cgroups * SCS_TR * cols_per_tile * 8.0;
        if (tile_bytes * (1.0 + 1.0 / world) > 96.0 * 1024 * 1024 * 1024) shared = false;
    }
    const int b_row_begin = shared ? 0 : row_begin, b_row_end = shared ? n : row_end;
    const bool sym = !shared && (row_begin == 0 && row_end == n && world == 1);
    const bool trapezoid = (flags & SCS_BUILD_UPPER) != 0;
    if (trapezoid)
        SCS_REQUIRE(row_begin % cols_per_tile == 0,
                    "scs_pcg_build: SCS_BUILD_UPPER needs row_begin (%d) to be a multiple of %d", row_begin,
                    cols_per_tile);
    const bool upper = sym || shared || trapezoid;
    const int gb0 = b_row_begin / SCS_TR;
    const int rows = row_end - row_begin;
    const int n_blocks = (b_row_end - b_row_begin + SCS_TR - 1) / SCS_TR;

    scs_graph *g = nullptr;
    SCS_TRY(graph_alloc(ctx, n, row_begin, row_end, s, &g, trapezoid ? row_begin : 0));
    g->upper = trapezoid;
    if (scatter) SCS_HIP_CHECK(hipMemsetAsync(g->d_w, 0, (size_t)rows * (size_t)g->ld * 8, s));
    double *w_base = g->d_w - g->col0;
    struct guard {
        scs_ctx *c;
        scs_graph *g;
        ~guard() {
            if (g) scs_graph_free(c, g);
        }
    } gd{ctx, g};

    std::vector<int2> tiles;
    tiles.reserve((size_t)n_blocks * n_cgroups);
    for (int b = 0; b < n_blocks; ++b)
        for (int c = 0; c < n_cgroups; ++c) {
            if (upper && (int64_t)(c + 1) * cols_per_tile <= (int64_t)(gb0 + b) * SCS_TR) continue;
            tiles.push_back(make_int2(b, c));
        }
    {
        const bool per_xcd = !(scs_dbg("SCS_TILE_ORDER") && atoi(scs_dbg("SCS_TILE_ORDER")) == 0);
        auto xcd_reorder = [](std::vector<int2> &v) {
            if (v.size() <= 8) return;
            std::vector<int2> per[8];
            for (const int2 &t : v) per[t.x & 7].push_back(t);
            std::vector<int2> ordered;
            ordered.reserve(v.size());
            size_t at[8] = {0, 0, 0, 0, 0, 0, 0, 0};
            while (ordered.size() < v.size())
                for (int x = 0; x < 8; ++x)
                    if (at[x] < per[x].size()) ordered.push_back(per[x][at[x]++]);
            v.swap(ordered);
        };
        if (per_xcd && !shared) {
            xcd_reorder(tiles);
        } else if (per_xcd) {
            std::vector<std::vector<int2>> share(world);
            for (size_t i = 0; i < tiles.size(); ++i) share[i % world].push_back(tiles[i]);
            for (auto &v : share) xcd_reorder(v);
            for (int r = 0; r < world; ++r)
                for (size_t k = 0; k < share[r].size(); ++k) tiles[(size_t)world * k + r] = share[r][k];
        }
    }
    std::vector<int2> all_tiles;
    dev_buf d_all_tiles(ctx);
    cached_buf d_tile_out(ctx), d_gathered(ctx);
    size_t chunk_doubles = 0;
    const bool exchange_allgather =
        scs_dbg("SCS_EXCHANGE") && std::string(scs_dbg("SCS_EXCHANGE")) == "allgather";
    if (shared) {
        all_tiles.swap(tiles);
        for (size_t i = rank; i < all_tiles.size(); i += world) tiles.push_back(all_tiles[i]);
        const size_t slots = (all_tiles.size() + world - 1) / world;
        chunk_doubles = slots * SCS_TR * cols_per_tile;
        SCS_TRY(d_all_tiles.alloc(all_tiles.size() * sizeof(int2)));
        SCS_HIP_CHECK(hipMemcpyAsync(d_all_tiles.p, all_tiles.data(),
                                     all_tiles.size() * sizeof(int2), hipMemcpyHostToDevice, s));
        SCS_TRY(d_tile_out.alloc(chunk_doubles * 8));
        if (exchange_allgather) SCS_TRY(d_gathered.alloc(chunk_doubles * 8 * world));
        if (tiles.size() < slots)
            SCS_HIP_CHECK(hipMemsetAsync((double *)d_tile_out.p + (slots - 1) * SCS_TR * cols_per_tile,
                                         0, (size_t)SCS_TR * cols_per_tile * 8, s));
    }
    pooled_buf d_tiles(ctx, 0);
    SCS_TRY(d_tiles.alloc(std::max<size_t>(tiles.size(), 1) * sizeof(int2)));
    SCS_HIP_CHECK(hipMemcpyAsync(d_tiles.p, tiles.data(), tiles.size() * sizeof(int2),
                                 hipMemcpyHostToDevice, s));

    bool tree_par = sym && !scatter && !tiles.empty() && tiles.size() <= 24 && tb->n_trees >= 128;
    if (const char *e = scs_dbg("SCS_TREE_PARALLEL")) tree_par = sym && !scatter && !tiles.empty() && atoi(e) != 0;
    const size_t cells_per_tree = tiles.size() * (size_t)SCS_TR * cols_per_tile * 8;

    constexpr int PIPE_NG = 2;
    const size_t wide_min_tiles = 13;
    bool listed = monotone && !scatter && !tiles.empty() && tb->n_trees > 0 &&
                  (double)tb->n_leaves / ((double)tb->n_trees * std::max(n, 1)) < 1.0 / 64.0;
    if (const char *e = scs_dbg("SCS_TILE_LISTS")) listed = monotone && !scatter && !tiles.empty() && atoi(e) != 0;
    if (listed) tree_par = false;
    int wide_mode = (monotone && !scatter && !tree_par && !listed && tiles.size() >= wide_min_tiles) ? 3 : 0;
    bool wide_forced = false;
    if (const char *e = scs_dbg("SCS_WIDE")) {
        wide_mode = (monotone && !scatter && !tiles.empty() && atoi(e)) ? 3 : 0;
        wide_forced = wide_mode != 0;
        if (wide_mode) listed = false;
    }
    if (wide_mode && ctx->max_lds_bytes < (int)spec_layout::LDS_BYTES) {
        wide_mode = 0;
        wide_forced = false;
    }
    if (wide_mode) tree_par = false;
    const bool wide = wide_mode != 0;
    const int group_tiles = PIPE_NG;
    std::vector<int4> groups;
    dev_buf d_groups(ctx);
    if (wide) {
        rec_bytes = wide_layout<PIPE_NG>::BYTES;
        std::vector<std::vector<int>> of_block((size_t)n_blocks);
        for (size_t i = 0; i < tiles.size(); ++i) of_block[(size_t)tiles[i].x].push_back((int)i);
        std::vector<int4> per[8];
        for (int b = 0; b < n_blocks; ++b) {
            const std::vector<int> &v = of_block[(size_t)b];
            for (size_t k = 0; k < v.size(); k += group_tiles)
                per[b & 7].push_back(make_int4(v[k], k + 1 < v.size() ? v[k + 1] : -1,
                                               (group_tiles > 2 && k + 2 < v.size()) ? v[k + 2] : -1, 0));
        }
        size_t total = 0, at[8] = {0, 0, 0, 0, 0, 0, 0, 0};
        for (auto &v : per) total += v.size();
        groups.reserve(total);
        while (groups.size() < total)
            for (int x = 0; x < 8; ++x)
                if (at[x] < per[x].size()) groups.push_back(per[x][at[x]++]);
        SCS_TRY(d_groups.alloc(groups.size() * sizeof(int4)));
        SCS_HIP_CHECK(hipMemcpyAsync(d_groups.p, groups.data(), groups.size() * sizeof(int4),
                                     hipMemcpyHostToDevice, s));
    }

    auto table_entries = [](int64_t m) -> int64_t { return (int64_t)levels_for(m) * m; };

    const int M = tb->n_trees;
    std::vector<int> batch_start{0};
    {
        const int batch_trees_env = scs_dbg("SCS_BATCH_TREES") ? atoi(scs_dbg("SCS_BATCH_TREES")) : 0;
        int max_batch_trees = 256;
        {
            const double avg_leaves = (double)tb->n_leaves / std::max(M, 1);
            const double table_bytes =
                (double)table_entries((int64_t)std::max(avg_leaves - 1.0, 1.0)) * (double)entry_bytes;
            max_batch_trees = (int)std::min(256.0, std::max(64.0, 600e6 / std::max(table_bytes, 1.0)));
        }
        if (n <= 2048) max_batch_trees = 4096;
        const int arrived = tb->late_start.empty() ? M : tb->late_start[0];
        if (wide) {
            const int rest = M - (arrived < M ? arrived : 0);
            const int k = std::max(1, (rest + 511) / 512);
            max_batch_trees = std::max(96, (rest + k - 1) / k);
        }
        if (tree_par)
            max_batch_trees = (int)std::max<size_t>(16, std::min<size_t>((size_t)max_batch_trees,
                                                                         SCS_SCRATCH_KEEP / cells_per_tree));
        if (batch_trees_env > 0) max_batch_trees = batch_trees_env;
        if (tree_par)
            max_batch_trees = (int)std::max<size_t>(1, std::min<size_t>((size_t)max_batch_trees,
                                                                        SCS_SCRATCH_KEEP / std::max<size_t>(cells_per_tree, 1)));
        size_t used = 0;
        for (int t = 0; t < M; ++t) {
            const int64_t nt = tb->h_tree_off[t + 1] - tb->h_tree_off[t];
            const int64_t m = nt - 1;
            const size_t need =
                (size_t)table_entries(m) * entry_bytes + (size_t)npad * 4 + (size_t)n_blocks * rec_bytes;
            if ((used + need > ctx->ws_limit || t - batch_start.back() >= max_batch_trees ||
                 (t == arrived && batch_start.size() == 1)) &&
                t > batch_start.back()) {
                batch_start.push_back(t);
                used = 0;
            }
            used += need;
        }
        batch_start.push_back(M);
    }
    const int n_batches = (int)batch_start.size() - 1;

    struct ev_ref {
        hipEvent_t a, b;
    } ev_total, ev_prep, ev_acc;
    for (auto &e : ctx->build_events)
        if (!e) SCS_HIP_CHECK(hipEventCreate(&e));
    ev_total = {ctx->build_events[0], ctx->build_events[1]};
    ev_prep = {ctx->build_events[2], ctx->build_events[3]};
    ev_acc = {ctx->build_events[4], ctx->build_events[5]};
    float prep_ms = 0.f, acc_ms = 0.f;
    SCS_HIP_CHECK(hipEventRecord(ev_total.a, s));

    int spec_batches = 0, spec_trees = 0;
    float spec_ms = 0.f;
    bool single_batch_spec = false;
    pooled_buf d_pos(ctx, 1), d_st(ctx, 3), d_stoff(ctx, 4), d_rec(ctx, 5), d_cells(ctx, 6);
    dev_buf d_pcol(ctx), d_lists(ctx), d_list_cnt(ctx);
    int listed_batches = 0;
    for (int bi = 0; bi < n_batches; ++bi) {
        const int t0 = batch_start[bi], t1 = batch_start[bi + 1];
        const int nb = t1 - t0;
        std::vector<int64_t> st_off(nb + 1);
        int max_levels = 0;
        int64_t max_n = 0;
        st_off[0] = 0;
        for (int t = t0; t < t1; ++t) {
            const int64_t nt = tb->h_tree_off[t + 1] - tb->h_tree_off[t];
            st_off[t - t0 + 1] = st_off[t - t0] + table_entries(nt - 1);
            max_levels = std::max(max_levels, levels_for(nt - 1));
            max_n = std::max(max_n, nt);
        }
        const size_t need_pos = (size_t)nb * npad * 4;
        const size_t need_st = (size_t)st_off[nb] * entry_bytes + 64;
        const size_t need_stoff = (size_t)(nb + 1) * 8;
        const size_t need_rec = (size_t)n_blocks * nb * rec_bytes;
        const int wide_min_trees = wide_forced ? 1 : 96;
        const bool wide_b = wide && (nb >= wide_min_trees || (groups.size() >= 8 * 256 && nb >= 16));
        if (wide_b) {
            ++spec_batches;
            spec_trees += nb;
            single_batch_spec = true;
        }
        SCS_TRY(d_pos.alloc(need_pos));
        SCS_TRY(d_st.alloc(need_st));
        SCS_TRY(d_stoff.alloc(need_stoff));
        SCS_TRY(d_rec.alloc(need_rec));

        SCS_HIP_CHECK(hipEventRecord(ev_prep.a, s));
        SCS_TRY(scs_tables_wait(ctx, tb, t1, s));
        SCS_HIP_CHECK(hipMemcpyAsync(d_stoff.p, st_off.data(), need_stoff, hipMemcpyHostToDevice, s));
        SCS_HIP_CHECK(hipMemsetAsync(d_pos.p, 0xFF, need_pos, s));
        dim3 grid_l((unsigned)((max_n + 255) / 256), (unsigned)nb);
        if (monotone) {
            k_positions_values<<<grid_l, 256, 0, s>>>(tb->d_tree_off, tb->d_leaf_taxon,
                                                      tb->d_adj_depth, tb->d_adj_val, tb->d_tree_w,
                                                      t0, (int32_t *)d_pos.p, npad,
                                                      (const int64_t *)d_stoff.p, (double *)d_st.p);
            if (max_n <= SPARSE_FUSED_MAX_LEAVES && max_levels > 1)
                k_sparse_levels_fused<double><<<(unsigned)nb, 1024, 0, s>>>(
                    tb->d_tree_off, t0, (const int64_t *)d_stoff.p, (double *)d_st.p, pick_smaller_value{});
            else
            for (int k = 1; k < max_levels; ++k)
                k_sparse_level<double><<<grid_l, 256, 0, s>>>(tb->d_tree_off, t0, k,
                                                              (const int64_t *)d_stoff.p,
                                                              (double *)d_st.p);
            if (wide_b)
                k_block_records_wide<PIPE_NG><<<dim3((unsigned)n_blocks, (unsigned)nb), 64, 0, s>>>(
                    tb->d_tree_off, t0, nb, (const int32_t *)d_pos.p, npad, (const int64_t *)d_stoff.p,
                    (const double *)d_st.p, b_row_begin, b_row_end, (unsigned char *)d_rec.p);
            else if (!scatter)
            k_block_records_mono<<<dim3((unsigned)n_blocks, (unsigned)nb), 64, 0, s>>>(
                tb->d_tree_off, t0, nb, (const int32_t *)d_pos.p, npad, (const int64_t *)d_stoff.p,
                (const double *)d_st.p, b_row_begin, b_row_end, (unsigned char *)d_rec.p);
        } else {
            k_positions_pairs<<<grid_l, 256, 0, s>>>(tb->d_tree_off, tb->d_leaf_taxon,
                                                     tb->d_adj_depth, tb->d_adj_val, tb->d_tree_w,
                                                     t0, (int32_t *)d_pos.p, npad,
                                                     (const int64_t *)d_stoff.p, (gap_entry *)d_st.p);
            if (max_n <= SPARSE_FUSED_MAX_LEAVES && max_levels > 1)
                k_sparse_levels_fused<gap_entry><<<(unsigned)nb, 1024, 0, s>>>(
                    tb->d_tree_off, t0, (const int64_t *)d_stoff.p, (gap_entry *)d_st.p, pick_shallower_pair{});
            else
            for (int k = 1; k < max_levels; ++k)
                k_sparse_level_pairs<<<grid_l, 256, 0, s>>>(tb->d_tree_off, t0, k,
                                                            (const int64_t *)d_stoff.p,
                                                            (gap_entry *)d_st.p);
            k_block_records_gen<<<dim3((unsigned)n_blocks, (unsigned)nb), 64, 0, s>>>(
                tb->d_tree_off, t0, nb, (const int32_t *)d_pos.p, npad, (const int64_t *)d_stoff.p,
                (const gap_entry *)d_st.p, b_row_begin, b_row_end, (unsigned char *)d_rec.p);
        }
        SCS_HIP_CHECK(hipEventRecord(ev_prep.b, s));

        SCS_HIP_CHECK(hipEventRecord(ev_acc.a, s));
        const unsigned nt = (unsigned)tiles.size();
        if (scatter) {
            const int64_t nbk = (max_n + 63) / 64;
            k_scatter_atomic<<<dim3((unsigned)(nbk * (nbk + 1) / 2), (unsigned)nb), 256, 0, s>>>(
                tb->d_tree_off, tb->d_leaf_taxon, t0, (const int64_t *)d_stoff.p, (const double *)d_st.p,
                g->d_w, g->ld);
        } else if (monotone) {
            mono_params mp;
            mp.tiles = (const int2 *)d_tiles.p;
            mp.rec = (const unsigned char *)d_rec.p;
            mp.pos = (const int32_t *)d_pos.p;
            mp.npad = npad;
            mp.stv = (const double *)d_st.p;
            mp.n_batch = nb;
            mp.w = w_base;
            mp.ld = g->ld;
            mp.n = n;
            mp.row_begin = b_row_begin;
            mp.row_end = b_row_end;
            mp.load_w = bi > 0;
            mp.mirror = (sym && bi == n_batches - 1) ? 1 : 0;
            mp.tile_out = shared ? (double *)d_tile_out.p : nullptr;
            mp.stamps = nullptr;
            mp.split_tiles = 0;
            mp.lists = nullptr;
            mp.list_cnt = nullptr;
            const bool stamp = scs_dbg("SCS_ACC_STAMP") && atoi(scs_dbg("SCS_ACC_STAMP"));
            if (wide_b) {
                wide_params wp;
                wp.m = mp;
                wp.groups = (const int4 *)d_groups.p;
                wp.producer_prio = 2;
                const unsigned ng = (unsigned)groups.size();
                dev_buf d_st8(ctx);
                if (stamp) {
                    SCS_TRY(d_st8.alloc(64));
                    SCS_HIP_CHECK(hipMemsetAsync(d_st8.p, 0, 64, s));
                    wp.m.stamps = (unsigned long long *)d_st8.p;
                }
#define SCS_LAUNCH_SPEC(SYM_, STAMP_)                                                                   \
    do {                                                                                                \
        SCS_HIP_CHECK(hipFuncSetAttribute((const void *)k_accumulate_spec<SYM_, STAMP_>,                \
                                          hipFuncAttributeMaxDynamicSharedMemorySize,                   \
                                          (int)spec_layout::LDS_BYTES));                                \
        k_accumulate_spec<SYM_, STAMP_><<<ng, spec_layout::THREADS, spec_layout::LDS_BYTES, s>>>(wp);   \
    } while (0)
                if (ng) {
                    if (stamp && sym) SCS_LAUNCH_SPEC(true, true);
                    else if (stamp) SCS_LAUNCH_SPEC(false, true);
                    else if (sym) SCS_LAUNCH_SPEC(true, false);
                    else SCS_LAUNCH_SPEC(false, false);
                }
#undef SCS_LAUNCH_SPEC
                if (stamp) {
                    unsigned long long h[8];
                    SCS_HIP_CHECK(hipMemcpyAsync(h, d_st8.p, 64, hipMemcpyDeviceToHost, s));
                    SCS_HIP_CHECK(hipStreamSynchronize(s));
                    const char *nm[5] = {"producer: pairs of the next tree", "producer: records + search + wait",
                                         "consumer: pair + table state", "consumer: cells + expansion", "barrier"};
                    double tot = 0;
                    for (int i = 0; i < 5; ++i) tot += (double)h[i];
                    for (int i = 0; i < 5; ++i)
                        fprintf(stderr, "[stamp spec] %-36s %6.2f %%  (%.0f cycles per wave-step)\n", nm[i],
                                100.0 * h[i] / tot, (double)h[i] / ((double)h[7] * nb));
                }
            } else if (nt && stamp) {
                dev_buf d_st8(ctx);
                SCS_TRY(d_st8.alloc(64));
                SCS_HIP_CHECK(hipMemsetAsync(d_st8.p, 0, 64, s));
                mp.stamps = (unsigned long long *)d_st8.p;
                if (sym) k_accumulate_mono<true, true><<<nt, MONO_TCW, 0, s>>>(mp);
                else k_accumulate_mono<false, true><<<nt, MONO_TCW, 0, s>>>(mp);
                unsigned long long h[8];
                SCS_HIP_CHECK(hipMemcpyAsync(h, d_st8.p, 64, hipMemcpyDeviceToHost, s));
                SCS_HIP_CHECK(hipStreamSynchronize(s));
                const char *nm[7] = {"wait loads+record", "barrier A", "combine", "search + issue",
                                     "expand", "barrier B", "cells"};
                double tot = 0;
                for (int i = 0; i < 7; ++i) tot += (double)h[i];
                for (int i = 0; i < 7; ++i)
                    fprintf(stderr, "[stamp] %-24s %6.2f %%  (%.0f cycles per wave-step)\n", nm[i],
                            100.0 * h[i] / tot, (double)h[i] / ((double)h[7] * nb));
            } else if (nt && tree_par) {
                SCS_TRY(d_cells.alloc((size_t)nb * cells_per_tree));
                mono_params ap = mp;
                ap.split_tiles = (int)nt;
                ap.load_w = 0;
                ap.mirror = 0;
                ap.tile_out = (double *)d_cells.p;
                k_accumulate_mono<true, false><<<nt * (unsigned)nb, MONO_TCW, 0, s>>>(ap);
                k_sum_tree_tiles<true, mono_params><<<nt * SCS_TR, MONO_TCW, 0, s>>>(mp, (const double *)d_cells.p,
                                                                                    (int)nt);
            } else if (nt && listed) {
                SCS_TRY(d_pcol.alloc((size_t)n_cgroups * nb));
                SCS_TRY(d_lists.alloc((size_t)nt * nb * 4));
                SCS_TRY(d_list_cnt.alloc((size_t)nt * 4));
                k_col_presence<<<dim3((unsigned)n_cgroups, (unsigned)nb), 64, 0, s>>>(
                    (const int32_t *)d_pos.p, npad, n, cols_per_tile, nb, (unsigned char *)d_pcol.p);
                k_tile_lists<<<(nt + 255) / 256, 256, 0, s>>>((const int2 *)d_tiles.p, (int)nt,
                                                             (const unsigned char *)d_rec.p, R3_BYTES, R3_CNT, nb,
                                                             (const unsigned char *)d_pcol.p, (int32_t *)d_lists.p,
                                                             (int32_t *)d_list_cnt.p);
                mp.lists = (const int32_t *)d_lists.p;
                mp.list_cnt = (const int32_t *)d_list_cnt.p;
                if (sym) k_accumulate_mono<true, false, true><<<nt, MONO_TCW, 0, s>>>(mp);
                else k_accumulate_mono<false, false, true><<<nt, MONO_TCW, 0, s>>>(mp);
                ++listed_batches;
            } else if (nt) {
                if (sym) k_accumulate_mono<true, false><<<nt, MONO_TCW, 0, s>>>(mp);
                else k_accumulate_mono<false, false><<<nt, MONO_TCW, 0, s>>>(mp);
            }
        } else {
            gen_params gp;
            gp.tiles = (const int2 *)d_tiles.p;
            gp.rec = (const unsigned char *)d_rec.p;
            gp.pos = (const int32_t *)d_pos.p;
            gp.npad = npad;
            gp.ste = (const gap_entry *)d_st.p;
            gp.n_batch = nb;
            gp.w = w_base;
            gp.ld = g->ld;
            gp.n = n;
            gp.row_begin = b_row_begin;
            gp.row_end = b_row_end;
            gp.load_w = bi > 0;
            gp.mirror = (sym && bi == n_batches - 1) ? 1 : 0;
            gp.tile_out = shared ? (double *)d_tile_out.p : nullptr;
            gp.split_tiles = 0;
            if (nt && tree_par) {
                SCS_TRY(d_cells.alloc((size_t)nb * cells_per_tree));
                gen_params ap = gp;
                ap.split_tiles = (int)nt;
                ap.load_w = 0;
                ap.mirror = 0;
                ap.tile_out = (double *)d_cells.p;
                k_accumulate_gen<true><<<nt * (unsigned)nb, MONO_TCW, 0, s>>>(ap);
                k_sum_tree_tiles<true, gen_params><<<nt * SCS_TR, MONO_TCW, 0, s>>>(gp, (const double *)d_cells.p,
                                                                                   (int)nt);
            } else if (nt) {
                if (sym) k_accumulate_gen<true><<<nt, MONO_TCW, 0, s>>>(gp);
                else k_accumulate_gen<false><<<nt, MONO_TCW, 0, s>>>(gp);
            }
        }
        SCS_HIP_CHECK(hipGetLastError());
        SCS_HIP_CHECK(hipEventRecord(ev_acc.b, s));
        if (n_batches > 1) {
            SCS_HIP_CHECK(hipEventSynchronize(ev_acc.b));
            float ms = 0.f;
            SCS_HIP_CHECK(hipEventElapsedTime(&ms, ev_prep.a, ev_prep.b));
            prep_ms += ms;
            SCS_HIP_CHECK(hipEventElapsedTime(&ms, ev_acc.a, ev_acc.b));
            acc_ms += ms;
            if (wide_b) spec_ms += ms;
        }
    }
    float exch_ms = 0.f;
    double exch_bytes = 0.0;
    if (shared && exchange_allgather) {
        ev_pair ev_x;
        SCS_TRY(ev_x.init());
        SCS_HIP_CHECK(hipEventRecord(ev_x.a, s));
        SCS_TRY(scs_comm_allgather_f64(&ctx->comm, (const double *)d_tile_out.p,
                                       (double *)d_gathered.p, chunk_doubles, s));
        k_unpack_tiles<<<(unsigned)all_tiles.size(), cols_per_tile, 0, s>>>(
            (const double *)d_gathered.p, (const int2 *)d_all_tiles.p, world,
            (int64_t)chunk_doubles, n, row_begin, row_end, g->d_w, g->ld);
        SCS_HIP_CHECK(hipGetLastError());
        SCS_HIP_CHECK(hipEventRecord(ev_x.b, s));
        SCS_HIP_CHECK(hipEventSynchronize(ev_x.b));
        SCS_HIP_CHECK(hipEventElapsedTime(&exch_ms, ev_x.a, ev_x.b));
        exch_bytes = (double)chunk_doubles * 8.0 * (world - 1);
    } else if (shared) {
        std::vector<int32_t> splits;
        SCS_TRY(scs_gather_row_splits(ctx, row_begin, row_end, n, splits));
        auto needs = [&](int dst, const int2 &t) {
            const int64_t lo = splits[dst], hi = splits[dst + 1];
            const int64_t r_lo = (int64_t)t.x * SCS_TR, r_hi = std::min<int64_t>(r_lo + SCS_TR, n);
            const int64_t c_lo = (int64_t)t.y * cols_per_tile, c_hi = std::min<int64_t>(c_lo + cols_per_tile, n);
            return (r_lo < hi && lo < r_hi) || (c_lo < hi && lo < c_hi);
        };
        std::vector<int64_t> send_off(world + 1, 0), recv_off(world + 1, 0);
        std::vector<int32_t> send_slots;
        std::vector<int2> recv_tiles;
        for (int p = 0; p < world; ++p) {
            for (size_t i = rank; i < all_tiles.size(); i += world)
                if (needs(p, all_tiles[i])) send_slots.push_back((int32_t)(i / world));
            send_off[p + 1] = (int64_t)send_slots.size() * SCS_TR * cols_per_tile;
            for (size_t i = p; i < all_tiles.size(); i += world)
                if (needs(rank, all_tiles[i])) recv_tiles.push_back(all_tiles[i]);
            recv_off[p + 1] = (int64_t)recv_tiles.size() * SCS_TR * cols_per_tile;
        }
        cached_buf d_send(ctx), d_recv(ctx);
        dev_buf d_slots(ctx), d_rtiles(ctx);
        SCS_TRY(d_send.alloc((size_t)send_off[world] * 8));
        SCS_TRY(d_recv.alloc((size_t)recv_off[world] * 8));
        SCS_TRY(d_slots.alloc(send_slots.size() * 4));
        SCS_TRY(d_rtiles.alloc(recv_tiles.size() * sizeof(int2)));
        ev_pair ev_x;
        SCS_TRY(ev_x.init());
        SCS_HIP_CHECK(hipEventRecord(ev_x.a, s));
        SCS_HIP_CHECK(hipMemcpyAsync(d_slots.p, send_slots.data(), send_slots.size() * 4,
                                     hipMemcpyHostToDevice, s));
        SCS_HIP_CHECK(hipMemcpyAsync(d_rtiles.p, recv_tiles.data(), recv_tiles.size() * sizeof(int2),
                                     hipMemcpyHostToDevice, s));
        if (!send_slots.empty())
            k_pack_tiles<<<(unsigned)send_slots.size(), 256, 0, s>>>(
                (const double *)d_tile_out.p, (const int32_t *)d_slots.p, cols_per_tile, (double *)d_send.p);
        SCS_HIP_CHECK(hipGetLastError());
        SCS_TRY(scs_comm_alltoallv_f64(&ctx->comm, (const double *)d_send.p, send_off.data(),
                                       (double *)d_recv.p, recv_off.data(), s));
        if (!recv_tiles.empty())
            k_unpack_received<<<(unsigned)recv_tiles.size(), cols_per_tile, 0, s>>>(
                (const double *)d_recv.p, (const int2 *)d_rtiles.p, n, row_begin, row_end, g->d_w,
                g->ld);
        SCS_HIP_CHECK(hipGetLastError());
        SCS_HIP_CHECK(hipEventRecord(ev_x.b, s));
        SCS_HIP_CHECK(hipEventSynchronize(ev_x.b));
        SCS_HIP_CHECK(hipEventElapsedTime(&exch_ms, ev_x.a, ev_x.b));
        exch_bytes = (double)(recv_off[world] - (recv_off[rank + 1] - recv_off[rank])) * 8.0;
    }
    SCS_HIP_CHECK(hipEventRecord(ev_total.b, s));
    SCS_HIP_CHECK(hipEventSynchronize(ev_total.b));
    SCS_TRY(scs_tables_finish(ctx, tb));
    float total_ms = 0.f;
    SCS_HIP_CHECK(hipEventElapsedTime(&total_ms, ev_total.a, ev_total.b));
    if (n_batches == 1) {
        SCS_HIP_CHECK(hipEventElapsedTime(&prep_ms, ev_prep.a, ev_prep.b));
        SCS_HIP_CHECK(hipEventElapsedTime(&acc_ms, ev_acc.a, ev_acc.b));
        if (single_batch_spec) spec_ms = acc_ms;
    }

    if (stats) {
        memset(stats, 0, sizeof(*stats));
        stats->n_taxa = n;
        stats->n_trees = M;
        stats->row_begin = row_begin;
        stats->row_end = row_end;
        stats->symmetric = shared ? 2 : (sym ? 1 : 0);
        stats->exchange_ms = exch_ms;
        stats->exchange_bytes = exch_bytes;
        stats->n_tiles = (int32_t)tiles.size();
        stats->n_batches = n_batches;
        stats->spec_batches = spec_batches;
        stats->tree_parallel_batches = tree_par ? n_batches : 0;
        stats->spec_trees = spec_trees;
        stats->listed_batches = listed_batches;
        stats->spec_ms = spec_ms;
        stats->cell_trees = (double)tiles.size() * SCS_TR * cols_per_tile * (double)M;
        stats->prep_ms = prep_ms;
        stats->accumulate_ms = acc_ms;
        stats->total_ms = total_ms;
        stats->bytes_w = 8.0 * rows * (double)n;
        stats->bytes_tables = 16.0 * (double)tb->n_leaves + 8.0 * M;
    }
    gd.g = nullptr;
    *out = g;
    return SCS_OK;
}

extern "C" int scs_graph_contract(scs_ctx *ctx, scs_graph *g, const int32_t *group_start,
                                  int32_t n_groups, scs_graph **out) {
    SCS_REQUIRE(ctx && g && group_start && out, "scs_graph_contract: null argument");
    if (g->mf) {
        scs_set_error("scs_graph_contract: a matrix-free graph has no matrix to contract");
        return SCS_EUNSUP;
    }
    if (g->upper) {
        scs_set_error("scs_graph_contract: an SCS_BUILD_UPPER graph holds no whole rows; build it "
                      "row-partitioned (SCS_BUILD_SHARED) when the node contracts");
        return SCS_EUNSUP;
    }
    SCS_REQUIRE(n_groups >= 1 && n_groups <= g->n, "scs_graph_contract: bad group count %d",
                n_groups);
    SCS_REQUIRE(group_start[0] == 0 && group_start[n_groups] == g->n,
                "scs_graph_contract: group_start must span [0, %d]", g->n);
    int g_begin = -1, g_end = -1;
    for (int i = 0; i < n_groups; ++i) {
        SCS_REQUIRE(group_start[i] < group_start[i + 1], "scs_graph_contract: empty group %d", i);
        if (group_start[i] == g->row_begin) g_begin = i;
        if (group_start[i + 1] == g->row_end) g_end = i + 1;
    }
    SCS_REQUIRE(g_begin >= 0 && g_end > g_begin,
                "scs_graph_contract: a group straddles this rank's row block [%d, %d)",
                g->row_begin, g->row_end);
    SCS_HIP_CHECK(hipSetDevice(ctx->device));
    scs_graph *ng = nullptr;
    SCS_TRY(graph_alloc(ctx, n_groups, g_begin, g_end, ctx->stream, &ng));
    int32_t *d_gs = nullptr;
    hipError_t e = scs_dev_malloc(ctx, (void **)&d_gs, (size_t)(n_groups + 1) * 4);
    if (e != hipSuccess) {
        scs_graph_free(ctx, ng);
        scs_set_error("scs_graph_contract: hipMalloc failed: %s", hipGetErrorString(e));
        return SCS_ENOMEM;
    }
    hipMemcpyAsync(d_gs, group_start, (size_t)(n_groups + 1) * 4, hipMemcpyHostToDevice,
                   ctx->stream);
    dim3 grid((unsigned)((n_groups + 255) / 256), (unsigned)std::min(g_end - g_begin, 65535));
    k_contract<<<grid, 256, 0, ctx->stream>>>(g->d_w, g->ld, g->row_begin, d_gs, g_begin, g_end,
                                              n_groups, ng->d_w, ng->ld);
    e = hipGetLastError();
    if (e == hipSuccess) e = hipStreamSynchronize(ctx->stream);
    scs_dev_free(d_gs);
    if (e != hipSuccess) {
        scs_graph_free(ctx, ng);
        scs_set_error("scs_graph_contract: kernel failed: %s", hipGetErrorString(e));
        return SCS_EHIP;
    }
    scs_graph_free(ctx, g);
    *out = ng;
    return SCS_OK;
}

extern "C" int scs_graph_download_rows(scs_ctx *ctx, const scs_graph *g, int32_t first, int32_t count,
                                       double *out);

extern "C" int scs_graph_download(scs_ctx *ctx, const scs_graph *g, double *out) {
    SCS_REQUIRE(ctx && g && out, "scs_graph_download: null argument");
    SCS_REQUIRE(!g->mf, "scs_graph_download: a matrix-free graph has no matrix");
    SCS_HIP_CHECK(hipSetDevice(ctx->device));
    SCS_HIP_CHECK(hipStreamSynchronize(ctx->stream));
    const size_t rows = (size_t)(g->row_end - g->row_begin);
    if (g->upper) return scs_graph_download_rows(ctx, g, g->row_begin, (int32_t)rows, out);
    SCS_HIP_CHECK(hipMemcpy2D(out, (size_t)g->n * 8, g->d_w, (size_t)g->ld * 8, (size_t)g->n * 8,
                              rows, hipMemcpyDeviceToHost));
    return SCS_OK;
}

extern "C" int scs_graph_download_rows(scs_ctx *ctx, const scs_graph *g, int32_t first,
                                       int32_t count, double *out) {
    SCS_REQUIRE(ctx && g && out, "scs_graph_download_rows: null argument");
    SCS_REQUIRE(!g->mf, "scs_graph_download_rows: a matrix-free graph has no matrix");
    SCS_REQUIRE(count >= 1 && first >= g->row_begin && first + count <= g->row_end,
                "scs_graph_download_rows: rows [%d, %d) outside this rank's block [%d, %d)", first,
                first + count, g->row_begin, g->row_end);
    SCS_HIP_CHECK(hipSetDevice(ctx->device));
    SCS_HIP_CHECK(hipStreamSynchronize(ctx->stream));
    if (g->upper) {
        const size_t wcols = (size_t)(g->n - g->col0);
        for (int32_t i = 0; i < count; ++i) memset(out + (size_t)i * g->n, 0, (size_t)g->n * 8);
        SCS_HIP_CHECK(hipMemcpy2D(out + g->col0, (size_t)g->n * 8,
                                  g->d_w + (int64_t)(first - g->row_begin) * g->ld, (size_t)g->ld * 8,
                                  wcols * 8, (size_t)count, hipMemcpyDeviceToHost));
        for (int32_t i = 0; i < count; ++i) {
            const int32_t c0 = (first + i) / 256 * 256;
            if (c0 > g->col0) memset(out + (size_t)i * g->n + g->col0, 0, (size_t)(c0 - g->col0) * 8);
        }
        return SCS_OK;
    }
    SCS_HIP_CHECK(hipMemcpy2D(out, (size_t)g->n * 8, g->d_w + (int64_t)(first - g->row_begin) * g->ld,
                              (size_t)g->ld * 8, (size_t)g->n * 8, (size_t)count,
                              hipMemcpyDeviceToHost));
    return SCS_OK;
}

int scs_graph_prepare_degrees_begin(scs_ctx *ctx, scs_graph *g, bool want_w32) {
    if (g->deg_stage) return SCS_OK;
    const int n = g->n;
    const int rows = g->row_end - g->row_begin;
    if (g->mf && !g->have_deg) {
        SCS_HIP_CHECK(hipSetDevice(ctx->device));
        hipStream_t s = ctx->stream;
        if (!g->d_deg) SCS_TRY(scs_block_alloc(ctx, (size_t)n * 8, (void **)&g->d_deg));
        if (!g->d_dinv) SCS_TRY(scs_block_alloc(ctx, (size_t)n * 8, (void **)&g->d_dinv));
        SCS_TRY(scs_matfree_apply(ctx, g, nullptr, 0, 4, nullptr, s));
        k_dinv<<<(n + 255) / 256, 256, 0, s>>>(g->d_deg, n, g->d_dinv);
        SCS_HIP_CHECK(hipGetLastError());
        SCS_TRY(scs_pinned_get(ctx, (size_t)n * 8, &g->deg_stage));
        SCS_HIP_CHECK(hipMemcpyAsync(g->deg_stage, g->d_deg, (size_t)n * 8, hipMemcpyDeviceToHost, s));
        return SCS_OK;
    }
    const bool img_rows = ctx->comm.world > 1 && !g->upper;
    bool need_img = want_w32 && !g->have_w32 && !g->upper &&
                    (img_rows || (ctx->comm.world == 1 && g->row_begin == 0 && rows == n));
    if (g->have_deg && !need_img) return SCS_OK;
    SCS_HIP_CHECK(hipSetDevice(ctx->device));
    hipStream_t s = ctx->stream;
    if (need_img && !g->d_w32) {
        const size_t need = (size_t)rows * g->ld * 4;
        std::lock_guard<std::mutex> lock(ctx->cache_mu);
        if (ctx->w32_cache && ctx->w32_cache_bytes >= need) {
            g->d_w32 = ctx->w32_cache;
            g->w32_bytes = ctx->w32_cache_bytes;
            ctx->w32_cache = nullptr;
            ctx->w32_cache_bytes = 0;
        } else if (scs_dev_malloc(ctx, (void **)&g->d_w32, need) == hipSuccess) {
            g->w32_bytes = need;
            if (scs_dbg("SCS_TRACE_SOLVES") && atoi(scs_dbg("SCS_TRACE_SOLVES")))
                fprintf(stderr, "[image] hipMalloc of %.2f GB\n", need / 1073741824.0);
        } else {
            (void)hipGetLastError();
            g->d_w32 = nullptr;
            need_img = false;
        }
    }
    if (!need_img && g->have_deg) return SCS_OK;
    if (need_img && img_rows && g->have_deg) {
        dev_buf tmp(ctx);
        SCS_TRY(tmp.alloc((size_t)n * 8));
        k_degrees<true><<<(rows + 3) / 4, 256, 0, s>>>(g->d_w, g->ld, n, rows, g->row_begin, (double *)tmp.p, g->d_w32, 1);
        SCS_HIP_CHECK(hipGetLastError());
        SCS_HIP_CHECK(hipStreamSynchronize(s));
        g->have_w32 = true;
        return SCS_OK;
    }
    if (!g->d_deg) SCS_TRY(scs_block_alloc(ctx, (size_t)n * 8, (void **)&g->d_deg));
    if (!g->d_dinv) SCS_TRY(scs_block_alloc(ctx, (size_t)n * 8, (void **)&g->d_dinv));
    const int world = ctx->comm.world;
    if (need_img && !img_rows) {
        k_degrees<true><<<(rows + 3) / 4, 256, 0, s>>>(g->d_w, g->ld, n, rows, g->row_begin, g->d_deg, g->d_w32);
        g->have_w32 = true;
    } else if (world == 1 && !g->upper) {
        k_degrees<false><<<(rows + 3) / 4, 256, 0, s>>>(g->d_w, g->ld, n, rows, g->row_begin, g->d_deg);
    } else {
        dev_buf send(ctx), recv(ctx);
        SCS_TRY(send.alloc((size_t)n * 8));
        SCS_TRY(recv.alloc((size_t)n * 8 * world));
        SCS_HIP_CHECK(hipMemsetAsync(send.p, 0, (size_t)n * 8, s));
        if (g->upper) {
            k_degrees_upper_rows<<<(rows + 3) / 4, 256, 0, s>>>(g->d_w, g->ld, n, rows, g->row_begin,
                                                                g->col0, (double *)send.p);
            k_degrees_upper_cols<<<(n - g->col0 + 255) / 256, 256, 0, s>>>(
                g->d_w, g->ld, n, g->row_begin, g->row_end, g->col0, (double *)send.p);
        } else if (need_img) {
            k_degrees<true><<<(rows + 3) / 4, 256, 0, s>>>(g->d_w, g->ld, n, rows, g->row_begin, (double *)send.p,
                                                           g->d_w32, 1);
            g->have_w32 = true;
        } else
        k_degrees<false><<<(rows + 3) / 4, 256, 0, s>>>(g->d_w, g->ld, n, rows, g->row_begin,
                                                        (double *)send.p);
        SCS_TRY(scs_comm_allgather_f64(&ctx->comm, (const double *)send.p, (double *)recv.p,
                                       (size_t)n, s));
        k_combine_degrees<<<(n + 255) / 256, 256, 0, s>>>((const double *)recv.p, world, n, g->d_deg);
        SCS_HIP_CHECK(hipGetLastError());
        SCS_HIP_CHECK(hipStreamSynchronize(s));
    }
    if (g->have_deg) {
        SCS_HIP_CHECK(hipGetLastError());
        return SCS_OK;
    }
    k_dinv<<<(n + 255) / 256, 256, 0, s>>>(g->d_deg, n, g->d_dinv);
    SCS_HIP_CHECK(hipGetLastError());
    SCS_TRY(scs_pinned_get(ctx, (size_t)n * 8, &g->deg_stage));
    SCS_HIP_CHECK(hipMemcpyAsync(g->deg_stage, g->d_deg, (size_t)n * 8, hipMemcpyDeviceToHost, s));
    return SCS_OK;
}

int scs_graph_prepare_degrees(scs_ctx *ctx, scs_graph *g) {
    if (g->have_deg) return SCS_OK;
    SCS_TRY(scs_graph_prepare_degrees_begin(ctx, g));
    const hipError_t e = hipStreamSynchronize(ctx->stream);
    const double *deg = (const double *)g->deg_stage;
    int iso = 0;
    double nrm2 = 0.0;
    if (e == hipSuccess)
        for (int i = 0; i < g->n; ++i) {
            if (deg[i] == 0.0) {
                ++iso;
                nrm2 += 1.0;
            } else {
                nrm2 += deg[i];
            }
        }
    scs_pinned_release(ctx, g->deg_stage);
    g->deg_stage = nullptr;
    SCS_HIP_CHECK(e);
    g->n_isolated = iso;
    g->dd_norm = sqrt(nrm2);
    g->have_deg = true;
    return SCS_OK;
}

extern "C" int scs_graph_degrees(scs_ctx *ctx, scs_graph *g, double *out) {
    SCS_REQUIRE(ctx && g && out, "scs_graph_degrees: null argument");
    SCS_TRY(scs_graph_prepare_degrees(ctx, g));
    SCS_HIP_CHECK(hipMemcpy(out, g->d_deg + g->row_begin,
                            (size_t)(g->row_end - g->row_begin) * 8, hipMemcpyDeviceToHost));
    return SCS_OK;
}

extern "C" int scs_debug_graph_raw(scs_ctx *ctx, scs_graph *g, int32_t what, void *out, int32_t *info_out) {
    SCS_REQUIRE(ctx && g && info_out, "scs_debug_graph_raw: null argument");
    SCS_REQUIRE(what >= 0 && what <= 2, "scs_debug_graph_raw: what must be 0 (W), 1 (image) or 2 (degrees), not %d",
                what);
    if (g->mf && what != 2) {
        scs_set_error("scs_debug_graph_raw: a matrix-free graph has neither a matrix nor an image");
        return SCS_EUNSUP;
    }
    const int rows = g->row_end - g->row_begin;
    const bool img_rows = ctx->comm.world > 1;
    if (what == 1) {
        if (g->upper) {
            scs_set_error("scs_debug_graph_raw: an SCS_BUILD_UPPER graph has no image");
            return SCS_EUNSUP;
        }
        if (!img_rows && !(g->row_begin == 0 && rows == g->n)) {
            scs_set_error("scs_debug_graph_raw: a row block [%d, %d) of %d on one rank has no image", g->row_begin,
                          g->row_end, g->n);
            return SCS_EUNSUP;
        }
    }
    info_out[0] = rows;
    info_out[1] = (int32_t)g->ld;
    info_out[2] = g->col0;
    info_out[3] = (what == 1 && img_rows) ? 1 : 0;
    if (!out) return SCS_OK;
    SCS_HIP_CHECK(hipSetDevice(ctx->device));
    if (what == 1) {
        SCS_TRY(scs_graph_prepare_degrees_begin(ctx, g, true));
        SCS_TRY(scs_graph_prepare_degrees(ctx, g));
        if (!g->have_w32 || !g->d_w32) {
            scs_set_error("scs_debug_graph_raw: the image could not be made (no memory)");
            return SCS_EUNSUP;
        }
    }
    if (what == 2) SCS_TRY(scs_graph_prepare_degrees(ctx, g));
    SCS_HIP_CHECK(hipStreamSynchronize(ctx->stream));
    if (what == 2)
        SCS_HIP_CHECK(hipMemcpy(out, g->d_deg, (size_t)g->n * 8, hipMemcpyDeviceToHost));
    else if (what == 1)
        SCS_HIP_CHECK(hipMemcpy(out, g->d_w32, (size_t)rows * (size_t)g->ld * 4, hipMemcpyDeviceToHost));
    else
        SCS_HIP_CHECK(hipMemcpy(out, g->d_w, (size_t)rows * (size_t)g->ld * 8, hipMemcpyDeviceToHost));
    return SCS_OK;
}
```

spectralclustersupertree_amd/csrc/scs_gen.h:

```cpp
#pragma once

struct __attribute__((aligned(16))) gap_entry {
    u32 d;
    u32 vlo, vhi;
    u32 pad;
    __device__ __forceinline__ double v() const { return __hiloint2double((int)vhi, (int)vlo); }
    __device__ __forceinline__ void set_v(double x) {
        vlo = (u32)__double2loint(x);
        vhi = (u32)__double2hiint(x);
    }
};
typedef u32 gap_words __attribute__((ext_vector_type(3)));

__device__ __forceinline__ gap_entry gap_min(const gap_entry a, const gap_entry b) {
    return b.d < a.d ? b : a;
}

__device__ __forceinline__ gap_entry rmq_gap(const gap_entry *__restrict__ base, int m, int a, int b) {
    int o[2];
    rmq_offsets(m, a, b, o);
    return gap_min(base[o[0]], base[o[1]]);
}

constexpr int G3_SPOS = 0;
constexpr int G3_GV = 256;
constexpr int G3_GD = 768;
constexpr int G3_SEEDV = G3_GD + 6 * 256;
constexpr int G3_SEEDD = G3_SEEDV + (MONO_WAVES - 1) * 512;
constexpr int G3_ARGPOS = G3_SEEDD + (MONO_WAVES - 1) * 256;
constexpr int G3_SORIG = G3_ARGPOS + 256;
constexpr int G3_RANK = G3_SORIG + 64;
constexpr int G3_PIV = G3_RANK + 64;
constexpr int G3_CNT = G3_PIV + 32;
constexpr int G3_M = G3_CNT + 4;
constexpr int G3_STOFF = G3_M + 4;
constexpr int G3_PIECE = (G3_STOFF + 8 + MONO_WAVES * 16 - 1) / (MONO_WAVES * 16) * 16;
constexpr int G3_BYTES = G3_PIECE * MONO_WAVES;
static_assert(G3_PIECE > 1024 && G3_PIECE <= 2048, "a wave stages its piece of a record with two DMAs");

__global__ void k_positions_pairs(const int64_t *__restrict__ tree_off,
                                  const int32_t *__restrict__ leaf_taxon,
                                  const int32_t *__restrict__ adj_depth,
                                  const double *__restrict__ adj_val,
                                  const double *__restrict__ tree_w, int t0,
                                  int32_t *__restrict__ pos, int64_t npad,
                                  const int64_t *__restrict__ st_off, gap_entry *__restrict__ ste) {
    const int tl = blockIdx.y;
    const int t = t0 + tl;
    const int64_t off = tree_off[t];
    const int n = (int)(tree_off[t + 1] - off);
    const int p = blockIdx.x * blockDim.x + threadIdx.x;
    if (p >= n) return;
    const unsigned tx = (unsigned)leaf_taxon[off + p];
    if (tx < (unsigned)npad) pos[(int64_t)tl * npad + tx] = p;
    if (p < n - 1) {
        gap_entry e;
        e.d = (u32)adj_depth[off + p];
        e.set_v(e.d ? adj_val[off + p] * tree_w[t] : 0.0);
        e.pad = 0;
        ste[st_off[tl] + p] = e;
    }
}

__global__ void k_sparse_level_pairs(const int64_t *__restrict__ tree_off, int t0, int k,
                                     const int64_t *__restrict__ st_off,
                                     gap_entry *__restrict__ ste) {
    const int tl = blockIdx.y;
    const int m = (int)(tree_off[t0 + tl + 1] - tree_off[t0 + tl]) - 1;
    const int p = blockIdx.x * blockDim.x + threadIdx.x;
    if (m < (1 << k) || p > m - (1 << k)) return;
    gap_entry *base = ste + st_off[tl];
    base[(int64_t)k * m + p] =
        gap_min(base[(int64_t)(k - 1) * m + p], base[(int64_t)(k - 1) * m + p + (1 << (k - 1))]);
}

__global__ __launch_bounds__(64) void k_block_records_gen(
    const int64_t *__restrict__ tree_off, int t0, int n_batch, const int32_t *__restrict__ pos,
    int64_t npad, const int64_t *__restrict__ st_off, const gap_entry *__restrict__ ste,
    int row_begin, int row_end, unsigned char *__restrict__ rec_all) {
    const int blk = blockIdx.x;
    const int tl = blockIdx.y;
    const int lane = threadIdx.x;
    const int m = (int)(tree_off[t0 + tl + 1] - tree_off[t0 + tl]) - 1;
    const int row = row_begin + blk * SCS_TR + lane;
    int p = -1;
    if (row < row_end) p = pos[(int64_t)tl * npad + row];
    const u32 pk = p < 0 ? 0x7FFFFFFFu : (u32)p;
    u64 key = ((u64)pk << 32) | (u32)lane;
    for (int k = 2; k <= 64; k <<= 1) {
        for (int j = k >> 1; j > 0; j >>= 1) {
            const u64 other = __shfl_xor(key, j, 64);
            const bool take_min = ((lane & j) == 0) == ((lane & k) == 0);
            const u64 lo = key < other ? key : other;
            const u64 hi = key < other ? other : key;
            key = take_min ? lo : hi;
        }
    }
    const int spos = (int)(key >> 32);
    const int orig = (int)(key & 63);
    const bool present = spos != 0x7FFFFFFF;
    const int cnt = __popcll(__ballot(present));
    const int next_pos = __shfl_down(spos, 1, 64);
    const gap_entry *st = ste + st_off[tl];
    u32 gd = 0;
    double gv = 0.0;
    int argpos = 0;
    if (lane < cnt - 1) {
        const gap_entry g = rmq_gap(st, m, spos, next_pos);
        gd = g.d;
        gv = g.v();
        int lo = spos, hi = next_pos;
        while (hi - lo > 1) {
            const int mid = (lo + hi) >> 1;
            if (rmq_gap(st, m, lo, mid).d == gd) hi = mid;
            else lo = mid;
        }
        argpos = lo;
    }
    unsigned char *rec = rec_all + ((int64_t)blk * n_batch + tl) * G3_BYTES;
    ((int *)(rec + G3_SPOS))[lane] = spos;
    ((double *)(rec + G3_GV))[lane] = gv;
    ((int *)(rec + G3_ARGPOS))[lane] = argpos;
    if ((lane & 7) == 7) ((int *)(rec + G3_PIV))[lane >> 3] = spos;
    rec[G3_SORIG + lane] = (unsigned char)orig;
    rec[G3_RANK + orig] = (unsigned char)lane;
    if (lane == 0) {
        *(int *)(rec + G3_CNT) = cnt;
        *(int *)(rec + G3_M) = m;
        *(int64_t *)(rec + G3_STOFF) = st_off[tl];
    }
    {
        u32 *sp = (u32 *)(rec + G3_GD);
        u32 mine = gd;
        sp[lane] = mine;
#pragma unroll
        for (int j = 1; j < 6; ++j) {
            const u32 other = __shfl_down(mine, 1 << (j - 1), 64);
            if (lane + (1 << (j - 1)) < 64) mine = other < mine ? other : mine;
            sp[j * 64 + lane] = mine;
        }
    }
    {
        double *seedv = (double *)(rec + G3_SEEDV);
        u32 *seedd = (u32 *)(rec + G3_SEEDD);
#pragma unroll
        for (int w = 1; w < MONO_WAVES; ++w) {
            const int end = mono_seg(w);
            u32 md = lane < end ? gd : DEPTH_INF;
            double mv = gv;
#pragma unroll
            for (int off = 1; off < 64; off <<= 1) {
                const u32 od = __shfl_down(md, off, 64);
                const double ov = __shfl_down(mv, off, 64);
                if (lane + off < end && od < md) {
                    md = od;
                    mv = ov;
                }
            }
            seedd[(w - 1) * 64 + lane] = md;
            seedv[(w - 1) * 64 + lane] = mv;
        }
    }
}

struct gen_params {
    const int2 *tiles;
    const unsigned char *rec;
    const int32_t *pos;
    int64_t npad;
    const gap_entry *ste;
    int n_batch;
    double *w;
    int64_t ld;
    int n;
    int row_begin, row_end;
    int load_w;
    int mirror;
    double *tile_out;
    int split_tiles;
};

template <bool SYM>
__global__ __launch_bounds__(MONO_TCW, 3) void k_accumulate_gen(gen_params p) {
    __shared__ __attribute__((aligned(16))) double s_dv[DT_DOUBLES];
    __shared__ __attribute__((aligned(16))) unsigned char s_rec[2][G3_BYTES];
    typedef __attribute__((address_space(3))) void *lds_ptr;

    const int tid = threadIdx.x;
    const int lane = tid & 63;
    const int wave = __builtin_amdgcn_readfirstlane(tid >> 6);
    const int split = p.split_tiles;
    const int2 tile = p.tiles[split > 0 ? (int)blockIdx.x % split : (int)blockIdx.x];
    const int blk = tile.x;
    const int row0 = p.row_begin + blk * SCS_TR;
    const int col = tile.y * MONO_TCW + tid;
    const int nt = p.n_batch;
    const int tl0 = split > 0 ? (int)blockIdx.x / split : 0;
    const int tl1 = split > 0 ? tl0 + 1 : nt;
    const int self = (col >= row0 && col < row0 + SCS_TR && col < p.row_end) ? col - row0 : -1;

    double acc[SCS_TR];
#pragma unroll
    for (int i = 0; i < SCS_TR; ++i) {
        double v = 0.0;
        if (p.load_w && p.tile_out)
            v = p.tile_out[((int64_t)blockIdx.x * SCS_TR + i) * MONO_TCW + tid];
        else if (p.load_w && col < p.n && row0 + i < p.row_end)
            v = p.w[(int64_t)(row0 - p.row_begin + i) * p.ld + col];
        acc[i] = v;
    }

    const unsigned char *rec_base = p.rec + (int64_t)blk * nt * G3_BYTES;
    const __amdgpu_buffer_rsrc_t r_rec =
        __builtin_amdgcn_make_buffer_rsrc((void *)rec_base, 0, nt * G3_BYTES, 0x00020000);
    const __amdgpu_buffer_rsrc_t r_pos =
        __builtin_amdgcn_make_buffer_rsrc((void *)p.pos, 0, (int)(nt * p.npad * 4), 0x00020000);
    const int lane16 = lane * 16;
    const int col4 = col * 4;
    auto issue_record = [&](int tl, int b) {
        __builtin_amdgcn_raw_ptr_buffer_load_lds(r_rec, (lds_ptr)(s_rec[b] + wave * G3_PIECE), 16,
                                                 lane16, tl * G3_BYTES + wave * G3_PIECE, 0, 0);
        if (lane < (G3_PIECE - 1024) / 16)
            __builtin_amdgcn_raw_ptr_buffer_load_lds(r_rec, (lds_ptr)(s_rec[b] + wave * G3_PIECE + 1024),
                                                     16, lane16, tl * G3_BYTES + wave * G3_PIECE + 1024,
                                                     0, 0);
    };

    gap_words qx = {0, 0, 0}, qy = {0, 0, 0};
    int cstate = 0;
    int cpos_next = -1;

    auto column_issue = [&](int tl, int cpos) {
        const unsigned char *rb = s_rec[tl & 1];
        const int *s_spos = (const int *)(rb + G3_SPOS);
        const int *s_arg = (const int *)(rb + G3_ARGPOS);
        const unsigned char *s_sorig = rb + G3_SORIG;
        const int *s_piv = (const int *)(rb + G3_PIV);
        const int cnt = __builtin_amdgcn_readfirstlane(*(const int *)(rb + G3_CNT));
        const bool present = cpos >= 0 && cnt > 0;
        int lo;
        {
            const int4 pa = *(const int4 *)&s_piv[0];
            const int4 pb = *(const int4 *)&s_piv[4];
            lo = ((pa.x < cpos) + (pa.y < cpos) + (pa.z < cpos) + (pa.w < cpos) + (pb.x < cpos) +
                  (pb.y < cpos) + (pb.z < cpos) + (pb.w < cpos)) * 8;
            const int base = min(lo, 56);
            int l2 = base;
#pragma unroll
            for (int s = 4; s > 0; s >>= 1)
                if (s_spos[l2 + s - 1] < cpos) l2 += s;
            lo = lo == 64 ? 64 : l2;
        }
        const bool hasl = present && self < 0 && lo > 0;
        const bool hasr = present && self < 0 && lo < cnt;
        const int il = max(lo - 1, 0), ir = min(lo, 63);
        const bool left = hasl && (!hasr || s_arg[il] >= cpos);
        const int ra = left ? il : ir;
        const int q_anchor = s_spos[ra];
        const int nbrow = s_sorig[ra];
        cstate = nbrow | ((hasl || hasr) ? 256 : 0) | ((present && self >= 0) ? 512 : 0) |
                 (left ? 1024 : 0) | (ra << 16);
        const int m = __builtin_amdgcn_readfirstlane(*(const int *)(rb + G3_M));
        const unsigned so_lo = __builtin_amdgcn_readfirstlane(*(const unsigned *)(rb + G3_STOFF));
        const unsigned so_hi = __builtin_amdgcn_readfirstlane(*(const unsigned *)(rb + G3_STOFF + 4));
        const unsigned char *st = (const unsigned char *)(p.ste + (((u64)so_hi << 32) | so_lo));
        const bool any = hasl || hasr;
        int o[2];
        rmq_offsets(m, any ? (left ? q_anchor : cpos) : 0, any ? (left ? cpos : q_anchor) : 1, o);
        qx = *(const gap_words *)(st + (unsigned)o[0] * 16u);
        qy = *(const gap_words *)(st + (unsigned)o[1] * 16u);
        cpos_next = __builtin_amdgcn_raw_buffer_load_b32(
            r_pos, col4, min(tl + 1, nt - 1) * (int)p.npad * 4, 0);
    };

    auto expand = [&](int tl) {
        const unsigned char *rb = s_rec[tl & 1];
        const int b0 = mono_seg(wave), b1 = mono_seg(wave + 1);
        const double gv_rank = ((const double *)(rb + G3_GV))[lane];
        const int gd_rank = ((const int *)(rb + G3_GD))[lane];
        const int so_rank = rb[G3_SORIG + lane];
        const int rho = rb[G3_RANK + lane];
        u32 curd = DEPTH_INF;
        double curv = 0.0;
        if (rho < b0) {
            curd = ((const u32 *)(rb + G3_SEEDD))[(wave - 1) * 64 + rho];
            curv = ((const double *)(rb + G3_SEEDV))[(wave - 1) * 64 + rho];
        }
        double *row_a = &s_dv[lane * DV_LD];
        double *col_a = &s_dv[lane];
#pragma unroll
        for (int j = 0; j < MONO_MAXSEG; ++j) {
            const int b = b0 + j;
            if (b >= b1) break;
            const int lo32 = __builtin_amdgcn_readlane((int)__double2loint(gv_rank), b);
            const int hi32 = __builtin_amdgcn_readlane(__double2hiint(gv_rank), b);
            const u32 gdb = (u32)__builtin_amdgcn_readlane(gd_rank, b);
            const int so_b = __builtin_amdgcn_readlane(so_rank, b);
            const double gvb = __hiloint2double(hi32, lo32);
            if (rho <= b) {
                row_a[so_b] = curv;
                col_a[so_b * DV_LD] = curv;
                const bool take = gdb < curd;
                curd = take ? gdb : curd;
                curv = take ? gvb : curv;
            }
        }
    };

    issue_record(tl0, tl0 & 1);
    issue_record(min(tl0 + 1, nt - 1), (tl0 + 1) & 1);
    cpos_next = __builtin_amdgcn_raw_buffer_load_b32(r_pos, col4, tl0 * (int)p.npad * 4, 0);
    asm volatile("s_waitcnt vmcnt(0)" ::: "memory");
    __syncthreads();
    column_issue(tl0, cpos_next);

    for (int tl = tl0; tl < tl1; ++tl) {
        asm volatile("s_waitcnt vmcnt(0)" ::: "memory");
        SCS_BARE_BARRIER();
        const unsigned char *rb = s_rec[tl & 1];
        int nb = 0;
        double vv = 0.0;
        unsigned tlo = 0, tw = 63;
        if (cstate & 256) {
            const gap_words g = qy.x < qx.x ? qy : qx;
            const u32 dn = g.x;
            vv = __hiloint2double((int)g.z, (int)g.y);
            nb = cstate & 255;
            const int ra = (cstate >> 16) & 63;
            const bool left = (cstate & 1024) != 0;
            const u32 *sp = (const u32 *)(rb + G3_GD);
            int pos = ra;
#pragma unroll
            for (int j = 5; j >= 0; --j) {
                const int step = 1 << j;
                const int idx = left ? pos - step : pos;
                const bool ok = left ? idx >= 0 : pos + step <= 63;
                const u32 dmin = sp[j * 64 + (ok ? idx : 0)];
                if (ok && dmin >= dn) pos = left ? idx : pos + step;
            }
            tlo = left ? pos : ra;
            tw = left ? ra - pos : pos - ra;
        } else if (cstate & 512) {
            nb = self;
            tlo = 64;
            tw = 0;
        }
        column_issue(min(tl + 1, nt - 1), cpos_next);
        expand(tl);
        const int rank_pack = ((const int *)(rb + G3_RANK))[lane & 15];
        SCS_BARE_BARRIER();
        issue_record(min(tl + 2, nt - 1), tl & 1);
        {
            int rp[16];
#pragma unroll
            for (int k = 0; k < 16; ++k) rp[k] = __builtin_amdgcn_readlane(rank_pack, k);
            double tmp[SCS_CELLS_GEN_DEPTH];
            unsigned tt;
            int sr;
            const unsigned addr =
                (unsigned)(size_t)(__attribute__((address_space(3))) double *)&s_dv[nb * DV_LD];
            SCS_CELLS_GEN_ASM(acc, tmp, tt, sr, addr, vv, tlo, tw, rp);
        }
    }

    tile_store<SYM>(p, acc, tile, row0, col, self, tid, lane, wave, s_dv);
}
```

spectralclustersupertree_amd/csrc/scs_mono.h:

```cpp
#pragma once

#include "scs_cells_asm.h"

constexpr int DV_LD = 65;
constexpr int DT_DOUBLES = 64 * DV_LD;
constexpr int R3_SPOS = 0;
constexpr int R3_G = 256;
constexpr int MONO_WAVES = 4;
constexpr int MONO_TCW = 64 * MONO_WAVES;
__host__ __device__ constexpr int mono_seg(int w) { return 64 * w / MONO_WAVES; }
constexpr int MONO_MAXSEG = (64 + MONO_WAVES - 1) / MONO_WAVES;
constexpr int R3_SEED = 768;
constexpr int R3_ARGPOS = R3_SEED + (MONO_WAVES - 1) * 512;
constexpr int R3_SORIG = R3_ARGPOS + 256;
constexpr int R3_RANK = R3_SORIG + 64;
constexpr int R3_PIV = R3_RANK + 64;
constexpr int R3_CNT = R3_PIV + 32;
constexpr int R3_M = R3_CNT + 4;
constexpr int R3_STOFF = R3_M + 4;
constexpr int R3_PIECE = (R3_STOFF + 8 + MONO_WAVES * 16 - 1) / (MONO_WAVES * 16) * 16;
constexpr int R3_BYTES = R3_PIECE * MONO_WAVES;
static_assert(R3_STOFF + 8 <= R3_BYTES && R3_PIECE <= 1024, "record layout");

#define SCS_BARE_BARRIER()                                        \
    do {                                                          \
        asm volatile("s_waitcnt lgkmcnt(0)" ::: "memory");        \
        __builtin_amdgcn_s_barrier();                             \
        asm volatile("" ::: "memory");                            \
    } while (0)

__global__ __launch_bounds__(64) void k_block_records_mono(
    const int64_t *__restrict__ tree_off, int t0, int n_batch, const int32_t *__restrict__ pos,
    int64_t npad, const int64_t *__restrict__ st_off, const double *__restrict__ stv,
    int row_begin, int row_end, unsigned char *__restrict__ rec_all) {
    const int blk = blockIdx.x;
    const int tl = blockIdx.y;
    const int lane = threadIdx.x;
    const int m = (int)(tree_off[t0 + tl + 1] - tree_off[t0 + tl]) - 1;
    const int row = row_begin + blk * SCS_TR + lane;
    int p = -1;
    if (row < row_end) p = pos[(int64_t)tl * npad + row];
    const u32 pk = p < 0 ? 0x7FFFFFFFu : (u32)p;
    u64 key = ((u64)pk << 32) | (u32)lane;
    for (int k = 2; k <= 64; k <<= 1) {
        for (int j = k >> 1; j > 0; j >>= 1) {
            const u64 other = __shfl_xor(key, j, 64);
            const bool take_min = ((lane & j) == 0) == ((lane & k) == 0);
            const u64 lo = key < other ? key : other;
            const u64 hi = key < other ? other : key;
            key = take_min ? lo : hi;
        }
    }
    const int spos = (int)(key >> 32);
    const int orig = (int)(key & 63);
    const bool present = spos != 0x7FFFFFFF;
    const int cnt = __popcll(__ballot(present));
    const int next_pos = __shfl_down(spos, 1, 64);
    const double *st = stv + st_off[tl];
    double g = 0.0;
    int argpos = 0;
    if (lane < cnt - 1) {
        g = rmq_min<double>(st, m, spos, next_pos);
        int lo = spos, hi = next_pos;
        while (hi - lo > 1) {
            const int mid = (lo + hi) >> 1;
            if (rmq_min<double>(st, m, lo, mid) == g) hi = mid;
            else lo = mid;
        }
        argpos = lo;
    }
    unsigned char *rec = rec_all + ((int64_t)blk * n_batch + tl) * R3_BYTES;
    ((int *)(rec + R3_SPOS))[lane] = spos;
    ((double *)(rec + R3_G))[lane] = g;
    ((int *)(rec + R3_ARGPOS))[lane] = argpos;
    if ((lane & 7) == 7) ((int *)(rec + R3_PIV))[lane >> 3] = spos;
    rec[R3_SORIG + lane] = (unsigned char)orig;
    rec[R3_RANK + orig] = (unsigned char)lane;
    if (lane == 0) {
        *(int *)(rec + R3_CNT) = cnt;
        *(int *)(rec + R3_M) = m;
        *(int64_t *)(rec + R3_STOFF) = st_off[tl];
    }
    {
        const double inf = __longlong_as_double(0x7FF0000000000000ll);
        double *seed = (double *)(rec + R3_SEED);
#pragma unroll
        for (int w = 1; w < MONO_WAVES; ++w) {
            const int end = mono_seg(w);
            double mine = lane < end ? g : inf;
#pragma unroll
            for (int off = 1; off < 64; off <<= 1) {
                const double other = __shfl_down(mine, off, 64);
                if (lane + off < end) mine = min_f64(mine, other);
            }
            seed[(w - 1) * 64 + lane] = mine;
        }
    }
}

struct mono_params {
    const int2 *tiles;
    const unsigned char *rec;
    const int32_t *pos;
    int64_t npad;
    const double *stv;
    int n_batch;
    double *w;
    int64_t ld;
    int n;
    int row_begin, row_end;
    int load_w;
    int mirror;
    double *tile_out;
    unsigned long long *stamps;
    int split_tiles;
    const int32_t *lists;
    const int32_t *list_cnt;
};

template <bool SYM, typename P>
__device__ __forceinline__ void tile_store(const P &p, double (&acc)[SCS_TR], const int2 tile,
                                           const int row0, const int col, const int self,
                                           const int tid, const int lane, const int wave,
                                           double *s_dv) {
    if (self >= 0) {
#pragma unroll
        for (int i = 0; i < SCS_TR; ++i)
            if (i == self) acc[i] = 0.0;
    }
    if (p.tile_out) {
        double *tp = p.tile_out + (int64_t)blockIdx.x * SCS_TR * MONO_TCW + tid;
        if (p.split_tiles > 0) {
            if (col < p.n) {
#pragma unroll
                for (int i = 0; i < SCS_TR; ++i)
                    if (row0 + i < p.row_end) tp[i * MONO_TCW] = acc[i];
            }
            return;
        }
#pragma unroll
        for (int i = 0; i < SCS_TR; ++i) tp[i * MONO_TCW] = acc[i];
        return;
    }
    if (col < p.n) {
#pragma unroll
        for (int i = 0; i < SCS_TR; ++i) {
            const int r = row0 + i;
            if (r < p.row_end) p.w[(int64_t)(r - p.row_begin) * p.ld + col] = acc[i];
        }
    }
    if (SYM && p.mirror) {
        __shared__ double t_own[MONO_TCW * 9 > DT_DOUBLES ? MONO_TCW * 9 : 1];
        double *t = MONO_TCW * 9 > DT_DOUBLES ? t_own : s_dv;
        const bool wave_mirrors = ((row0 / MONO_TCW) + 1) * MONO_TCW <= ((tile.y * MONO_TCW + wave * 64) / SCS_TR) * SCS_TR;
#pragma unroll
        for (int q = 0; q < SCS_TR / 8; ++q) {
            SCS_BARE_BARRIER();
#pragma unroll
            for (int j = 0; j < 8; ++j) t[tid * 9 + j] = acc[q * 8 + j];
            SCS_BARE_BARRIER();
            if (wave_mirrors) {
#pragma unroll
                for (int it = 0; it < 8; ++it) {
                    const int cl = wave * 64 + it * 8 + (lane >> 3);
                    const int c = tile.y * MONO_TCW + cl;
                    const int r = row0 + q * 8 + (lane & 7);
                    if (c < p.n && r < p.row_end) p.w[(int64_t)c * p.ld + r] = t[cl * 9 + (lane & 7)];
                }
            }
        }
    }
}

template <bool SYM, bool STAMPED, bool LISTED = false>
__global__ __launch_bounds__(MONO_TCW, MONO_TCW / 256) void k_accumulate_mono(mono_params p) {
    __shared__ __attribute__((aligned(16))) double s_dv[DT_DOUBLES];
    __shared__ __attribute__((aligned(16))) unsigned char s_rec[2][R3_BYTES];
    typedef __attribute__((address_space(3))) void *lds_ptr;

    unsigned long long ts[7] = {0, 0, 0, 0, 0, 0, 0}, tprev = 0;
    auto stamp = [&](int k) {
        if (STAMPED) {
            __builtin_amdgcn_sched_barrier(0);
            unsigned long long tnow;
            asm volatile("s_memtime %0\n\ts_waitcnt lgkmcnt(0)" : "=s"(tnow)::"memory");
            ts[k] += tnow - tprev;
            tprev = tnow;
            __builtin_amdgcn_sched_barrier(0);
        }
    };

    const int tid = threadIdx.x;
    const int lane = tid & 63;
    const int wave = __builtin_amdgcn_readfirstlane(tid >> 6);
    const int split = p.split_tiles;
    const int2 tile = p.tiles[split > 0 ? (int)blockIdx.x % split : (int)blockIdx.x];
    const int blk = tile.x;
    const int row0 = p.row_begin + blk * SCS_TR;
    const int col = tile.y * MONO_TCW + tid;
    const int nt = p.n_batch;
    typedef const __attribute__((address_space(4))) int32_t *clist;
    const clist lst = LISTED ? (clist)(size_t)(p.lists + (int64_t)blockIdx.x * nt) : nullptr;
    const int nl = LISTED ? __builtin_amdgcn_readfirstlane(p.list_cnt[blockIdx.x]) : nt;
    auto T = [&](int k) -> int { return LISTED ? lst[min(k, max(nl - 1, 0))] : k; };
    const int tl0 = LISTED ? 0 : (split > 0 ? (int)blockIdx.x / split : 0);
    const int tl1 = LISTED ? nl : (split > 0 ? tl0 + 1 : nt);
    const double inf = __longlong_as_double(0x7FF0000000000000ll);
    const int self = (col >= row0 && col < row0 + SCS_TR && col < p.row_end) ? col - row0 : -1;

    double acc[SCS_TR];
#pragma unroll
    for (int i = 0; i < SCS_TR; ++i) {
        double v = 0.0;
        if (p.load_w && p.tile_out)
            v = p.tile_out[((int64_t)blockIdx.x * SCS_TR + i) * MONO_TCW + tid];
        else if (p.load_w && col < p.n && row0 + i < p.row_end)
            v = p.w[(int64_t)(row0 - p.row_begin + i) * p.ld + col];
        acc[i] = v;
    }

    const unsigned char *rec_base = p.rec + (int64_t)blk * nt * R3_BYTES;
    const __amdgpu_buffer_rsrc_t r_rec =
        __builtin_amdgcn_make_buffer_rsrc((void *)rec_base, 0, nt * R3_BYTES, 0x00020000);
    const __amdgpu_buffer_rsrc_t r_pos =
        __builtin_amdgcn_make_buffer_rsrc((void *)p.pos, 0, (int)(nt * p.npad * 4), 0x00020000);
    const int lane16 = lane * 16;
    const int col4 = col * 4;
    auto issue_record = [&](int tl, int b) {
        if (lane < R3_PIECE / 16)
            __builtin_amdgcn_raw_ptr_buffer_load_lds(r_rec, (lds_ptr)(s_rec[b] + wave * R3_PIECE), 16,
                                                     lane16, tl * R3_BYTES + wave * R3_PIECE, 0, 0);
    };

    double qx = 0.0, qy = 0.0;
    int cstate = 0;
    int cpos_next = -1;

    auto column_issue = [&](int tl, int cpos, int t_next) {
        const unsigned char *rb = s_rec[tl & 1];
        const int *s_spos = (const int *)(rb + R3_SPOS);
        const int *s_arg = (const int *)(rb + R3_ARGPOS);
        const unsigned char *s_sorig = rb + R3_SORIG;
        const int *s_piv = (const int *)(rb + R3_PIV);
        const int cnt = __builtin_amdgcn_readfirstlane(*(const int *)(rb + R3_CNT));
        const bool present = cpos >= 0 && cnt > 0;
        int lo;
        {
            const int4 pa = *(const int4 *)&s_piv[0];
            const int4 pb = *(const int4 *)&s_piv[4];
            lo = ((pa.x < cpos) + (pa.y < cpos) + (pa.z < cpos) + (pa.w < cpos) + (pb.x < cpos) +
                  (pb.y < cpos) + (pb.z < cpos) + (pb.w < cpos)) * 8;
            const int base = min(lo, 56);
            int l2 = base;
#pragma unroll
            for (int s = 4; s > 0; s >>= 1)
                if (s_spos[l2 + s - 1] < cpos) l2 += s;
            lo = lo == 64 ? 64 : l2;
        }
        const bool hasl = present && self < 0 && lo > 0;
        const bool hasr = present && self < 0 && lo < cnt;
        const int il = max(lo - 1, 0), ir = min(lo, 63);
        const bool left = hasl && (!hasr || s_arg[il] >= cpos);
        const int q_anchor = s_spos[left ? il : ir];
        const int nbrow = s_sorig[left ? il : ir];
        cstate = nbrow | ((hasl || hasr) ? 256 : 0) | ((present && self >= 0) ? 512 : 0);
        const int m = __builtin_amdgcn_readfirstlane(*(const int *)(rb + R3_M));
        const unsigned so_lo = __builtin_amdgcn_readfirstlane(*(const unsigned *)(rb + R3_STOFF));
        const unsigned so_hi = __builtin_amdgcn_readfirstlane(*(const unsigned *)(rb + R3_STOFF + 4));
        const unsigned char *st = (const unsigned char *)(p.stv + (((u64)so_hi << 32) | so_lo));
        const bool any = hasl || hasr;
        int o[2];
        rmq_offsets(m, any ? (left ? q_anchor : cpos) : 0, any ? (left ? cpos : q_anchor) : 1, o);
        qx = *(const double *)(st + (unsigned)o[0] * 8u);
        qy = *(const double *)(st + (unsigned)o[1] * 8u);
        cpos_next = __builtin_amdgcn_raw_buffer_load_b32(r_pos, col4, t_next * (int)p.npad * 4, 0);
    };

    auto expand = [&](int tl) {
        const unsigned char *rb = s_rec[tl & 1];
        const int b0 = mono_seg(wave), b1 = mono_seg(wave + 1);
        const double g_rank = ((const double *)(rb + R3_G))[lane];
        const int so_rank = rb[R3_SORIG + lane];
        const int rho = rb[R3_RANK + lane];
        double cur = inf;
        if (rho < b0) cur = ((const double *)(rb + R3_SEED))[(wave - 1) * 64 + rho];
        double *row_a = &s_dv[lane * DV_LD];
        double *col_a = &s_dv[lane];
#pragma unroll
        for (int j = 0; j < MONO_MAXSEG; ++j) {
            const int b = b0 + j;
            if (b >= b1) break;
            const int lo32 = __builtin_amdgcn_readlane((int)__double2loint(g_rank), b);
            const int hi32 = __builtin_amdgcn_readlane(__double2hiint(g_rank), b);
            const int so_b = __builtin_amdgcn_readlane(so_rank, b);
            const double gb = __hiloint2double(hi32, lo32);
            if (rho <= b) {
                row_a[so_b] = cur;
                col_a[so_b * DV_LD] = cur;
                cur = min_f64(cur, gb);
            }
        }
    };

    if (LISTED && nl == 0) {
        tile_store<SYM>(p, acc, tile, row0, col, self, tid, lane, wave, s_dv);
        return;
    }
    issue_record(T(tl0), tl0 & 1);
    issue_record(T(min(tl0 + 1, nl - 1)), (tl0 + 1) & 1);
    cpos_next = __builtin_amdgcn_raw_buffer_load_b32(r_pos, col4, T(tl0) * (int)p.npad * 4, 0);
    asm volatile("s_waitcnt vmcnt(0)" ::: "memory");
    __syncthreads();
    column_issue(tl0, cpos_next, T(min(tl0 + 1, nl - 1)));
    if (STAMPED) asm volatile("s_memtime %0\n\ts_waitcnt lgkmcnt(0)" : "=s"(tprev)::"memory");

    for (int tl = tl0; tl < tl1; ++tl) {
        asm volatile("s_waitcnt vmcnt(0)" ::: "memory");
        stamp(0);
        SCS_BARE_BARRIER();
        stamp(1);
        int nb = 0;
        double vn = 0.0;
        if (cstate & 256) {
            vn = min_f64(qx, qy);
            nb = cstate & 255;
        } else if (cstate & 512) {
            nb = self;
            vn = inf;
        }
        stamp(2);
        column_issue(min(tl + 1, nl - 1), cpos_next, T(min(tl + 2, nl - 1)));
        stamp(3);
        expand(tl);
        stamp(4);
        SCS_BARE_BARRIER();
        stamp(5);
        issue_record(T(min(tl + 2, nl - 1)), tl & 1);
        {
            double tmp[SCS_CELLS_DEPTH];
            const unsigned addr =
                (unsigned)(size_t)(__attribute__((address_space(3))) double *)&s_dv[nb * DV_LD];
            SCS_CELLS_ASM(acc, tmp, addr, vn);
        }
        stamp(6);
    }

    if (STAMPED && lane == 0 && p.stamps) {
#pragma unroll
        for (int k = 0; k < 7; ++k) atomicAdd(&p.stamps[k], ts[k]);
        atomicAdd(&p.stamps[7], 1ull);
    }
    tile_store<SYM>(p, acc, tile, row0, col, self, tid, lane, wave, s_dv);
}

template <bool SYM, typename P>
__global__ __launch_bounds__(MONO_TCW) void k_sum_tree_tiles(P p, const double *__restrict__ cells, int n_tiles) {
    const int tile_i = (int)blockIdx.x / SCS_TR, i = (int)blockIdx.x % SCS_TR;
    const int2 tile = p.tiles[tile_i];
    const int row = p.row_begin + tile.x * SCS_TR + i;
    const int col = tile.y * MONO_TCW + (int)threadIdx.x;
    if (row >= p.row_end || col >= p.n) return;
    double *wcell = p.w + (int64_t)(row - p.row_begin) * p.ld + col;
    double acc = p.load_w ? *wcell : 0.0;
    const double *src = cells + ((int64_t)tile_i * SCS_TR + i) * MONO_TCW + threadIdx.x;
    const int64_t stride = (int64_t)n_tiles * SCS_TR * MONO_TCW;
    int t = 0;
    for (; t + 16 <= p.n_batch; t += 16) {
        double v[16];
#pragma unroll
        for (int k = 0; k < 16; ++k) v[k] = src[(int64_t)(t + k) * stride];
#pragma unroll
        for (int k = 0; k < 16; ++k) acc += v[k];
    }
// ... 6 lines not shown
```

spectralclustersupertree_amd/csrc/scs_mono_wide.h:

```cpp
#pragma once

template <int NG>
struct wide_layout {
    static constexpr int NSEG = 4 * NG;
    static constexpr int SPOS = 0;
    static constexpr int G = 256;
    static constexpr int SEED = 768;
    static constexpr int ARGPOS = SEED + (NSEG - 1) * 512;
    static constexpr int SORIG = ARGPOS + 256;
    static constexpr int RANK = SORIG + 64;
    static constexpr int PIV = RANK + 64;
    static constexpr int CNT = PIV + 32;
    static constexpr int M = CNT + 4;
    static constexpr int STOFF = M + 4;
    static constexpr int BYTES = (STOFF + 8 + 15) / 16 * 16;
    static constexpr int PIECES = (BYTES + 1023) / 1024;
    __host__ __device__ static constexpr int seg(int w) { return 64 * w / NSEG; }
    static constexpr int MAXSEG = (64 + NSEG - 1) / NSEG;
    static_assert(STOFF % 8 == 0 && PIECES <= NSEG, "record layout");
};

template <int NG>
__global__ __launch_bounds__(64) void k_block_records_wide(
    const int64_t *__restrict__ tree_off, int t0, int n_batch, const int32_t *__restrict__ pos,
    int64_t npad, const int64_t *__restrict__ st_off, const double *__restrict__ stv,
    int row_begin, int row_end, unsigned char *__restrict__ rec_all) {
    using L = wide_layout<NG>;
    const int blk = blockIdx.x;
    const int tl = blockIdx.y;
    const int lane = threadIdx.x;
    const int m = (int)(tree_off[t0 + tl + 1] - tree_off[t0 + tl]) - 1;
    const int row = row_begin + blk * SCS_TR + lane;
    int p = -1;
    if (row < row_end) p = pos[(int64_t)tl * npad + row];
    const u32 pk = p < 0 ? 0x7FFFFFFFu : (u32)p;
    u64 key = ((u64)pk << 32) | (u32)lane;
    for (int k = 2; k <= 64; k <<= 1) {
        for (int j = k >> 1; j > 0; j >>= 1) {
            const u64 other = __shfl_xor(key, j, 64);
            const bool take_min = ((lane & j) == 0) == ((lane & k) == 0);
            const u64 lo = key < other ? key : other;
            const u64 hi = key < other ? other : key;
            key = take_min ? lo : hi;
        }
    }
    const int spos = (int)(key >> 32);
    const int orig = (int)(key & 63);
    const bool present = spos != 0x7FFFFFFF;
    const int cnt = __popcll(__ballot(present));
    const int next_pos = __shfl_down(spos, 1, 64);
    const double *st = stv + st_off[tl];
    double g = 0.0;
    int argpos = 0;
    if (lane < cnt - 1) {
        g = rmq_min<double>(st, m, spos, next_pos);
        int lo = spos, hi = next_pos;
        while (hi - lo > 1) {
            const int mid = (lo + hi) >> 1;
            if (rmq_min<double>(st, m, lo, mid) == g) hi = mid;
            else lo = mid;
        }
        argpos = lo;
    }
    unsigned char *rec = rec_all + ((int64_t)blk * n_batch + tl) * L::BYTES;
    ((int *)(rec + L::SPOS))[lane] = spos;
    ((double *)(rec + L::G))[lane] = g;
    ((int *)(rec + L::ARGPOS))[lane] = argpos;
    if ((lane & 7) == 7) ((int *)(rec + L::PIV))[lane >> 3] = spos;
    rec[L::SORIG + lane] = (unsigned char)orig;
    rec[L::RANK + orig] = (unsigned char)lane;
    if (lane == 0) {
        *(int *)(rec + L::CNT) = cnt;
        *(int *)(rec + L::M) = m;
        *(int64_t *)(rec + L::STOFF) = st_off[tl];
    }
    const double inf = __longlong_as_double(0x7FF0000000000000ll);
    double *seed = (double *)(rec + L::SEED);
#pragma unroll
    for (int w = 1; w < L::NSEG; ++w) {
        const int end = L::seg(w);
        double mine = lane < end ? g : inf;
#pragma unroll
        for (int off = 1; off < 64; off <<= 1) {
            const double other = __shfl_down(mine, off, 64);
            if (lane + off < end) mine = min_f64(mine, other);
        }
        seed[(w - 1) * 64 + lane] = mine;
    }
}

typedef int scs_int4 __attribute__((ext_vector_type(4)));

struct wide_params {
    mono_params m;
    const int4 *groups;
    int producer_prio;
};

template <bool SYM>
__device__ __forceinline__ void tile_store_wide(const mono_params &p, double (&acc)[SCS_TR],
                                                const int2 tile, const bool active, const int slot,
                                                const int row0, const int col, const int self,
                                                const int ltid, const int lane, const int wl,
                                                double *t) {
    if (self >= 0) {
#pragma unroll
        for (int i = 0; i < SCS_TR; ++i)
            if (i == self) acc[i] = 0.0;
    }
    if (p.tile_out) {
        if (active) {
            double *tp = p.tile_out + (int64_t)slot * SCS_TR * MONO_TCW + ltid;
#pragma unroll
            for (int i = 0; i < SCS_TR; ++i) tp[i * MONO_TCW] = acc[i];
        }
        return;
    }
    if (active && col < p.n) {
#pragma unroll
        for (int i = 0; i < SCS_TR; ++i) {
            const int r = row0 + i;
            if (r < p.row_end) p.w[(int64_t)(r - p.row_begin) * p.ld + col] = acc[i];
        }
    }
    if (SYM && p.mirror) {
        const bool wave_mirrors =
            active && ((row0 / MONO_TCW) + 1) * MONO_TCW <= ((tile.y * MONO_TCW + wl * 64) / SCS_TR) * SCS_TR;
#pragma unroll
        for (int q = 0; q < SCS_TR / 8; ++q) {
            SCS_BARE_BARRIER();
#pragma unroll
            for (int j = 0; j < 8; ++j) t[ltid * 9 + j] = acc[q * 8 + j];
            SCS_BARE_BARRIER();
            if (wave_mirrors) {
#pragma unroll
                for (int it = 0; it < 8; ++it) {
                    const int cl = wl * 64 + it * 8 + (lane >> 3);
                    const int c = tile.y * MONO_TCW + cl;
                    const int r = row0 + q * 8 + (lane & 7);
                    if (c < p.n && r < p.row_end) p.w[(int64_t)c * p.ld + r] = t[cl * 9 + (lane & 7)];
                }
            }
        }
    }
}

struct spec_layout {
    using L = wide_layout<2>;
    static constexpr int CONSUMERS = 8, PRODUCERS = 4, THREADS = 64 * (CONSUMERS + PRODUCERS);
    static constexpr size_t O_T = 0;
    static constexpr int NREC = 6;
    static constexpr size_t O_REC = 2 * (size_t)DT_DOUBLES * 8;
    static constexpr size_t O_VN = O_REC + NREC * (size_t)L::BYTES;
    static constexpr size_t O_ADDR = O_VN + 2 * 512 * 8;
    static constexpr size_t LDS_BYTES = O_ADDR + 2 * 512 * 4;
    static_assert(O_VN % 16 == 0 && 3 * (size_t)MONO_TCW * 9 * 8 <= LDS_BYTES, "layout");
};

template <bool SYM, bool STAMPED>
__global__ __launch_bounds__(spec_layout::THREADS) void k_accumulate_spec(wide_params wp) {
    using S = spec_layout;
    using L = wide_layout<2>;
    extern __shared__ __attribute__((aligned(16))) unsigned char s_mem[];
    double *const s_t = (double *)(s_mem + S::O_T);
    unsigned char *const s_rec = s_mem + S::O_REC;
    double *const s_vn = (double *)(s_mem + S::O_VN);
    unsigned *const s_addr = (unsigned *)(s_mem + S::O_ADDR);
    const mono_params &p = wp.m;

    unsigned long long ts[7] = {0, 0, 0, 0, 0, 0, 0}, tprev = 0;
    auto stamp = [&](int k) {
        if (STAMPED) {
            __builtin_amdgcn_sched_barrier(0);
            unsigned long long tnow;
            asm volatile("s_memtime %0\n\ts_waitcnt lgkmcnt(0)" : "=s"(tnow)::"memory");
            ts[k] += tnow - tprev;
            tprev = tnow;
            __builtin_amdgcn_sched_barrier(0);
        }
    };

    const int tid = threadIdx.x;
    const int lane = tid & 63;
    const int wave = __builtin_amdgcn_readfirstlane(tid >> 6);
    const bool producer = wave >= S::CONSUMERS;
    const int pw = wave - S::CONSUMERS;
    const int4 grp = wp.groups[blockIdx.x];
    const int nt = p.n_batch;
    const double inf = __longlong_as_double(0x7FF0000000000000ll);
    const int cw = producer ? 2 * pw : wave;
    const int sub = cw >> 2, wl = cw & 3;
    const int ltid = (cw & 3) * 64 + lane;
    const int ti = sub == 0 ? grp.x : grp.y;
    const bool active = ti >= 0;
    const int2 tile = p.tiles[active ? ti : grp.x];
    const int blk = tile.x;
    const int row0 = p.row_begin + blk * SCS_TR;
    const int col = tile.y * MONO_TCW + ltid;
    const int self = (col >= row0 && col < row0 + SCS_TR && col < p.row_end) ? col - row0 : -1;

    const unsigned char *rec_base = p.rec + (int64_t)blk * nt * L::BYTES;
    const __amdgpu_buffer_rsrc_t r_pos =
        __builtin_amdgcn_make_buffer_rsrc((void *)p.pos, 0, (int)(nt * p.npad * 4), 0x00020000);
    const int lane16 = lane * 16;

    const __amdgpu_buffer_rsrc_t r_rec =
        __builtin_amdgcn_make_buffer_rsrc((void *)rec_base, 0, nt * L::BYTES, 0x00020000);
    struct pieces {
        scs_int4 v[2];
    };
    auto load_record = [&](int t, pieces &r) {
        if (t >= nt) return;
#pragma unroll
        for (int pc = 0; pc < L::PIECES; pc += S::PRODUCERS) {
            const int piece = pc + pw;
            if (piece < L::PIECES) {
                const int left = (L::BYTES - piece * 1024) / 16;
                if (lane < left)
                    r.v[pc / S::PRODUCERS] =
                        __builtin_amdgcn_raw_buffer_load_b128(r_rec, lane16, t * L::BYTES + piece * 1024, 0);
            }
        }
    };
    auto store_record = [&](int t, const pieces &r) {
        if (t >= nt) return;
#pragma unroll
        for (int pc = 0; pc < L::PIECES; pc += S::PRODUCERS) {
            const int piece = pc + pw;
            if (piece < L::PIECES) {
                const int left = (L::BYTES - piece * 1024) / 16;
                if (lane < left)
                    *(scs_int4 *)(s_rec + (t % S::NREC) * L::BYTES + piece * 1024 + lane16) = r.v[pc / S::PRODUCERS];
            }
        }
    };
    int pcol4[2], pself[2], cpos[2], cpos2[2];
#pragma unroll
    for (int k = 0; k < 2; ++k) {
        const int c = tile.y * MONO_TCW + (((2 * pw + k) & 3) * 64) + lane;
        pcol4[k] = c * 4;
        pself[k] = (c >= row0 && c < row0 + SCS_TR && c < p.row_end) ? c - row0 : -1;
        cpos[k] = -1;
        cpos2[k] = -1;
    }
    struct query {
        double qx[2], qy[2];
        int cstate[2];
    };
    typedef const __attribute__((address_space(4))) int *cint;
    int tail[12];
    auto request_tail = [&](int t) {
        cint gpiv = (cint)(size_t)(rec_base + (int64_t)min(t, nt - 1) * L::BYTES + L::PIV);
#pragma unroll
        for (int k = 0; k < 12; ++k) tail[k] = gpiv[k];
    };
    auto search = [&](int t_raw, query &q) {
        const int t = min(t_raw, nt - 1);
        const unsigned char *rb = s_rec + (t % S::NREC) * L::BYTES;
        const int *s_spos = (const int *)(rb + L::SPOS);
        const int *s_arg = (const int *)(rb + L::ARGPOS);
        const unsigned char *s_sorig = rb + L::SORIG;
        const int4 pa = make_int4(tail[0], tail[1], tail[2], tail[3]);
        const int4 pb = make_int4(tail[4], tail[5], tail[6], tail[7]);
        const int cnt = tail[8], m = tail[9];
        const unsigned so_lo = (unsigned)tail[10], so_hi = (unsigned)tail[11];
        static_assert(L::CNT == L::PIV + 32 && L::M == L::PIV + 36 && L::STOFF == L::PIV + 40, "record tail");
        const unsigned char *st = (const unsigned char *)(p.stv + (((u64)so_hi << 32) | so_lo));
        int cp_now[2];
#pragma unroll
        for (int k = 0; k < 2; ++k) {
            cp_now[k] = cpos[k];
            cpos[k] = cpos2[k];
            cpos2[k] = __builtin_amdgcn_raw_buffer_load_b32(r_pos, pcol4[k], min(t + 2, nt - 1) * (int)p.npad * 4, 0);
        }
#pragma unroll
        for (int k = 0; k < 2; ++k) {
            const int cp = cp_now[k];
            const bool present = cp >= 0 && cnt > 0;
            int lo = ((pa.x < cp) + (pa.y < cp) + (pa.z < cp) + (pa.w < cp) + (pb.x < cp) + (pb.y < cp) +
                      (pb.z < cp) + (pb.w < cp)) * 8;
            const int base = min(lo, 56);
            const int4 qa = *(const int4 *)&s_spos[base];
            const int4 qb = *(const int4 *)&s_spos[base + 4];
            const int l2 = base + (qa.x < cp) + (qa.y < cp) + (qa.z < cp) + (qa.w < cp) + (qb.x < cp) +
                           (qb.y < cp) + (qb.z < cp);
            lo = lo == 64 ? 64 : l2;
            const bool hasl = present && pself[k] < 0 && lo > 0;
            const bool hasr = present && pself[k] < 0 && lo < cnt;
            const int il = max(lo - 1, 0), ir = min(lo, 63);
            const int a_il = s_arg[il];
            const int sp_il = s_spos[il], sp_ir = s_spos[ir];
            const int so_il = s_sorig[il], so_ir = s_sorig[ir];
            const bool left = hasl && (!hasr || a_il >= cp);
            const int q_anchor = left ? sp_il : sp_ir;
            const int nbrow = left ? so_il : so_ir;
            q.cstate[k] = nbrow | ((hasl || hasr) ? 256 : 0) | ((present && pself[k] >= 0) ? 512 : 0);
            const bool any = hasl || hasr;
            int o[2];
            rmq_offsets(m, any ? (left ? q_anchor : cp) : 0, any ? (left ? cp : q_anchor) : 1, o);
            q.qx[k] = *(const double *)(st + (unsigned)o[0] * 8u);
            q.qy[k] = *(const double *)(st + (unsigned)o[1] * 8u);
        }
        request_tail(t_raw + 1);
    };
    auto finish = [&](int t, const query &q) {
        const unsigned tbase =
            (unsigned)(size_t)(__attribute__((address_space(3))) double *)&s_t[(t & 1) * DT_DOUBLES];
#pragma unroll
        for (int k = 0; k < 2; ++k) {
            int nb = 0;
            double vn = 0.0;
            if (q.cstate[k] & 256) {
                vn = min_f64(q.qx[k], q.qy[k]);
                nb = q.cstate[k] & 255;
            } else if (q.cstate[k] & 512) {
                nb = pself[k];
                vn = inf;
            }
            const int slot = (t & 1) * 512 + (2 * pw + k) * 64 + lane;
            s_vn[slot] = vn;
            s_addr[slot] = tbase + (unsigned)nb * (DV_LD * 8);
        }
    };

    auto expand_whole = [&](int t) {
        const unsigned char *rb = s_rec + (t % S::NREC) * L::BYTES;
        double *dv = s_t + (t & 1) * DT_DOUBLES;
        const int b0 = L::seg(wave);
        const double g_rank = ((const double *)(rb + L::G))[lane];
        const int so_rank = rb[L::SORIG + lane];
        const int rho = rb[L::RANK + lane];
        double cur = inf;
        if (rho < b0) cur = ((const double *)(rb + L::SEED))[(wave - 1) * 64 + rho];
        double *row_a = &dv[lane * DV_LD];
        double *col_a = &dv[lane];
#pragma unroll
        for (int j = 0; j < 8; ++j) {
            const int b = b0 + j;
            const int lo32 = __builtin_amdgcn_readlane((int)__double2loint(g_rank), b);
            const int hi32 = __builtin_amdgcn_readlane(__double2hiint(g_rank), b);
            const int so_b = __builtin_amdgcn_readlane(so_rank, b);
            const double gb = __hiloint2double(hi32, lo32);
            if (rho <= b) {
                row_a[so_b] = cur;
                col_a[so_b * DV_LD] = cur;
                cur = min_f64(cur, gb);
            }
        }
    };

    if (producer) {
        pieces ra = {{{0, 0, 0, 0}, {0, 0, 0, 0}}}, rb = ra, rc = ra;
        {
            pieces first[5] = {ra, ra, ra, ra, ra};
#pragma unroll
            for (int t = 0; t < 5; ++t) load_record(t, first[t]);
#pragma unroll
            for (int t = 0; t < 5; ++t) store_record(t, first[t]);
        }
        load_record(5, ra);
        load_record(6, rb);
        load_record(7, rc);
#pragma unroll
        for (int k = 0; k < 2; ++k) {
            cpos[k] = __builtin_amdgcn_raw_buffer_load_b32(r_pos, pcol4[k], 0, 0);
            cpos2[k] = __builtin_amdgcn_raw_buffer_load_b32(r_pos, pcol4[k], min(1, nt - 1) * (int)p.npad * 4, 0);
// ... 90 lines not shown
```

Before: 0.01422.

## Store argmin offsets in sparse tables to replace binary-search argpos lookup

Extends the sparse-table build to also record, per level, the 16-bit offset of the minimum, so block-record kernels find the argmin position in O(1) instead of a log-depth binary search of repeated RMQ queries. Preparation is split into per-piece launches with a tree offset (tl0), the fused level kernel is unrolled, and table offsets are staged through pinned host memory. This adds memory traffic and workspace for the argmin arrays, which shrinks batch sizes, and it adds a debug entry point for inspecting block records.

Result: faster. 0.01396 (median of 6 runs) (-1.9%).

```diff
diff --git a/include/scs_hip.h b/include/scs_hip.h
--- a/include/scs_hip.h
+++ b/include/scs_hip.h
@@ -67,7 +67,7 @@
     int32_t spec_trees;
     double spec_ms;
     int32_t listed_batches;
-    int32_t reserved;
+    int32_t prep_pieces;
 } scs_build_stats;
 
 int scs_version(void);
@@ -294,6 +294,10 @@
 
 int scs_debug_graph_raw(scs_ctx *ctx, scs_graph *graph, int32_t what, void *out, int32_t *info_out);
 
+int scs_debug_block_records(scs_ctx *ctx, const scs_tables *tables, int32_t t_begin, int32_t t_end, int32_t row_begin,
+                            int32_t row_end, int32_t kind, int32_t *spos_out, double *gap_out, int32_t *argpos_out,
+                            int32_t *depth_out, int32_t *cnt_out);
+
 int scs_debug_split_plan(int32_t n_trees, const int64_t *node_off, int32_t *tpb_out, int32_t *n_groups_out,
                          uint8_t *staged_out);
 
diff --git a/spectralclustersupertree_amd/_native.py b/spectralclustersupertree_amd/_native.py
--- a/spectralclustersupertree_amd/_native.py
+++ b/spectralclustersupertree_amd/_native.py
@@ -102,7 +102,7 @@
         ("spec_trees", C.c_int32),
         ("spec_ms", C.c_double),
         ("listed_batches", C.c_int32),
-        ("reserved", C.c_int32),
+        ("prep_pieces", C.c_int32),
     ]
 
     def as_dict(self) -> dict:
@@ -188,6 +188,7 @@
     "scs_debug_scan": (C.c_int, [_P, _I32, _I32, C.c_int64, _IP, _IP]),
     "scs_debug_split_plan": (C.c_int, [_I32, _LP, _P, _P, _P]),
     "scs_debug_graph_raw": (C.c_int, [_P, _P, _I32, _P, _IP]),
+    "scs_debug_block_records": (C.c_int, [_P, _P, _I32, _I32, _I32, _I32, _I32, _IP, _DP, _IP, _IP, _IP]),
     "scs_debug_score_plan": (C.c_int, [_P, _I32, _LP, _I32, _I32, C.c_int64, C.c_int64, _P, _IP, _LP, _IP, _IP, _LP]),
     "scs_debug_branch_plan": (C.c_int, [_P, _I32, _LP, _I32, _I32, C.c_int64, C.c_int64, _I32, _P, _IP, _LP, _LP, _LP]),
     "scs_debug_placement_plan": (C.c_int, [_P, _I32, _LP, _I32, _I32, _I32, _I32, _I32, _I32, _IP, _IP, _IP, _LP, _LP,
diff --git a/spectralclustersupertree_amd/backend.py b/spectralclustersupertree_amd/backend.py
--- a/spectralclustersupertree_amd/backend.py
+++ b/spectralclustersupertree_amd/backend.py
@@ -761,6 +761,22 @@
         graph.upper = bool(upper)
         return graph
 
+    def block_records(self, kind: str, t_begin: int = 0, t_end: int | None = None, row_begin: int = 0,
+                      row_end: int | None = None) -> dict:
+        t_end = self.n_trees if t_end is None else t_end
+        row_end = self.n_taxa if row_end is None else row_end
+        code = {"mono": 0, "wide": 1, "general": 2}[kind]
+        nb, nt = (max(row_end - row_begin, 0) + 63) // 64, max(t_end - t_begin, 0)
+        spos = np.empty((nb, nt, 64), dtype=np.int32)
+        gap = np.empty((nb, nt, 64), dtype=np.float64)
+        argpos = np.empty((nb, nt, 64), dtype=np.int32)
+        depth = np.empty((nb, nt, 64), dtype=np.int32) if code == 2 else None
+        cnt = np.empty((nb, nt), dtype=np.int32)
+        nv.check(self.dev._lib.scs_debug_block_records(
+            self.dev._ctx, self._h, int(t_begin), int(t_end), int(row_begin), int(row_end), code, nv.iptr(spos),
+            nv.dptr(gap), nv.iptr(argpos), nv.iptr(depth) if depth is not None else None, nv.iptr(cnt)))
+        return {"spos": spos, "gap": gap, "argpos": argpos, "depth": depth, "cnt": cnt}
+
 
     def matrix_free_graph(self, max_block: int = 8) -> "DeviceGraph":
         handle = C.c_void_p()
diff --git a/spectralclustersupertree_amd/csrc/scs_build.hip b/spectralclustersupertree_amd/csrc/scs_build.hip
--- a/spectralclustersupertree_amd/csrc/scs_build.hip
+++ b/spectralclustersupertree_amd/csrc/scs_build.hip
@@ -23,14 +23,47 @@
     return x < y ? x : y;
 }
 
+typedef unsigned short argmin_t;
+constexpr int ARGMIN_MAX_LEVEL = 16;
+__host__ __device__ inline int argmin_levels(int levels) {
+    return levels - 1 < ARGMIN_MAX_LEVEL ? (levels > 1 ? levels - 1 : 0) : ARGMIN_MAX_LEVEL;
+}
+__device__ __forceinline__ int argmin_position(const argmin_t *__restrict__ am, int m, int k, int a, int b,
+                                               bool right_smaller) {
+    const int q = right_smaller ? b - (1 << k) : a;
+    return q + (int)am[(int64_t)(k - 1) * m + q];
+}
+__device__ __forceinline__ double rmq_min_at(const double *__restrict__ st, const argmin_t *__restrict__ am, int m,
+                                             int a, int b, int &at) {
+    int o[2];
+    rmq_offsets(m, a, b, o);
+    const int k = 31 - __clz(b - a);
+    const double x = st[o[0]], y = st[o[1]];
+    const double g = x < y ? x : y;
+    if (k == 0) {
+        at = a;
+    } else if (k <= ARGMIN_MAX_LEVEL) {
+        at = argmin_position(am, m, k, a, b, y < x);
+    } else {
+        int lo = a, hi = b;
+        while (hi - lo > 1) {
+            const int mid = (lo + hi) >> 1;
+            if (rmq_min<double>(st, m, lo, mid) == g) hi = mid;
+            else lo = mid;
+        }
+        at = lo;
+    }
+    return g;
+}
+
 __global__ void k_positions_values(const int64_t *__restrict__ tree_off,
                                    const int32_t *__restrict__ leaf_taxon,
                                    const int32_t *__restrict__ adj_depth,
                                    const double *__restrict__ adj_val,
-                                   const double *__restrict__ tree_w, int t0,
+                                   const double *__restrict__ tree_w, int t0, int tl0,
                                    int32_t *__restrict__ pos, int64_t npad,
                                    const int64_t *__restrict__ st_off, double *__restrict__ stv) {
-    const int tl = blockIdx.y;
+    const int tl = tl0 + blockIdx.y;
     const int t = t0 + tl;
     const int64_t off = tree_off[t];
     const int n = (int)(tree_off[t + 1] - off);
@@ -42,36 +75,76 @@
         stv[st_off[tl] + p] = adj_depth[off + p] ? adj_val[off + p] * tree_w[t] : 0.0;
 }
 
-template <typename K>
-__global__ void k_sparse_level(const int64_t *__restrict__ tree_off, int t0, int k,
-                               const int64_t *__restrict__ st_off, K *__restrict__ st) {
-    const int tl = blockIdx.y;
+template <typename K, typename PICK>
+__global__ void k_sparse_level(const int64_t *__restrict__ tree_off, int t0, int tl0, int k,
+                               const int64_t *__restrict__ st_off, K *__restrict__ st,
+                               const int64_t *__restrict__ am_off, argmin_t *__restrict__ am_all, PICK pick) {
+    const int tl = tl0 + blockIdx.y;
     const int m = (int)(tree_off[t0 + tl + 1] - tree_off[t0 + tl]) - 1;
     const int p = blockIdx.x * blockDim.x + threadIdx.x;
     if (m < (1 << k) || p > m - (1 << k)) return;
     K *base = st + st_off[tl];
-    const K a = base[(int64_t)(k - 1) * m + p], b = base[(int64_t)(k - 1) * m + p + (1 << (k - 1))];
-    base[(int64_t)k * m + p] = a < b ? a : b;
-}
-
-template <typename K, typename MIN>
-__global__ __launch_bounds__(1024) void k_sparse_levels_fused(const int64_t *__restrict__ tree_off, int t0,
+    const int half = 1 << (k - 1);
+    const K a = base[(int64_t)(k - 1) * m + p], b = base[(int64_t)(k - 1) * m + p + half];
+    base[(int64_t)k * m + p] = pick(a, b);
+    if (k > ARGMIN_MAX_LEVEL) return;
+    argmin_t *am = am_all + am_off[tl];
+    const bool right = pick.right_less(a, b);
+    int off = right ? half : 0;
+    if (k > 1) off += (int)am[(int64_t)(k - 2) * m + p + (right ? half : 0)];
+    am[(int64_t)(k - 1) * m + p] = (argmin_t)off;
+}
+
+constexpr int FUSED_UNROLL = 4;
+template <typename K, typename PICK>
+__global__ __launch_bounds__(1024) void k_sparse_levels_fused(const int64_t *__restrict__ tree_off, int t0, int tl0,
                                                                const int64_t *__restrict__ st_off,
-                                                               K *__restrict__ st, MIN pick) {
-    const int tl = blockIdx.x;
+                                                               K *__restrict__ st,
+                                                               const int64_t *__restrict__ am_off,
+                                                               argmin_t *__restrict__ am_all, PICK pick) {
+    const int tl = tl0 + blockIdx.x;
     const int m = (int)(tree_off[t0 + tl + 1] - tree_off[t0 + tl]) - 1;
     K *base = st + st_off[tl];
+    argmin_t *am = am_all + am_off[tl];
     for (int k = 1; (1 << k) <= m; ++k) {
         const K *prev = base + (int64_t)(k - 1) * m;
         K *cur = base + (int64_t)k * m;
         const int half = 1 << (k - 1), last = m - (1 << k);
-        for (int p = threadIdx.x; p <= last; p += 1024) cur[p] = pick(prev[p], prev[p + half]);
+        const argmin_t *am_prev = am + (int64_t)(k - 2) * m;
+        argmin_t *am_cur = am + (int64_t)(k - 1) * m;
+        for (int p0 = threadIdx.x; p0 <= last; p0 += 1024 * FUSED_UNROLL) {
+            K a[FUSED_UNROLL], b[FUSED_UNROLL];
+            int oa[FUSED_UNROLL], ob[FUSED_UNROLL];
+#pragma unroll
+            for (int u = 0; u < FUSED_UNROLL; ++u) {
+                const int p = p0 + u * 1024;
+                oa[u] = ob[u] = 0;
+                if (p <= last) {
+                    a[u] = prev[p];
+                    b[u] = prev[p + half];
+                    if (k > 1) {
+                        oa[u] = (int)am_prev[p];
+                        ob[u] = (int)am_prev[p + half];
+                    }
+                }
+            }
+#pragma unroll
+            for (int u = 0; u < FUSED_UNROLL; ++u) {
+                const int p = p0 + u * 1024;
+                if (p <= last) {
+                    cur[p] = pick(a[u], b[u]);
+                    am_cur[p] = (argmin_t)(pick.right_less(a[u], b[u]) ? half + ob[u] : oa[u]);
+                }
+            }
+        }
         __syncthreads();
     }
 }
 constexpr int SPARSE_FUSED_MAX_LEAVES = 32768;
+static_assert(SPARSE_FUSED_MAX_LEAVES <= (1 << ARGMIN_MAX_LEVEL), "every level of a fused table has an argmin level");
 struct pick_smaller_value {
     __device__ double operator()(double a, double b) const { return a < b ? a : b; }
+    __device__ bool right_less(double a, double b) const { return b < a; }
 };
 
 __device__ __forceinline__ double min_f64(double a, double b) {
@@ -89,6 +162,7 @@
 #include "scs_gen.h"
 struct pick_shallower_pair {
     __device__ gap_entry operator()(const gap_entry a, const gap_entry b) const { return gap_min(a, b); }
+    __device__ bool right_less(const gap_entry a, const gap_entry b) const { return b.d < a.d; }
 };
 
 __global__ __launch_bounds__(256) void k_scatter_atomic(const int64_t *__restrict__ tree_off,
@@ -501,6 +575,92 @@
     for (int t = 0; t < n_batch; ++t)
         if (pc[t] && *(const int *)(rb + (int64_t)t * rec_bytes) > 0) out[c++] = t;
     list_cnt[i] = c;
+}
+
+constexpr int PIPE_NG = 2;
+
+namespace {
+
+enum { PREP_MONO = 0, PREP_WIDE = 1, PREP_GEN = 2, PREP_NO_RECORDS = 3 };
+
+struct prep_batch {
+    const scs_tables *tb;
+    int t0, nb;
+    int kind;
+    int32_t *pos;
+    int64_t npad;
+    const int64_t *st_off;
+    const int64_t *am_off;
+    void *st;
+    argmin_t *am;
+    unsigned char *rec;
+    int n_blocks, row_begin, row_end;
+};
+
+int64_t table_entries(int64_t m) { return (int64_t)levels_for(m) * m; }
+int64_t argmin_entries(int64_t m) { return (int64_t)argmin_levels(levels_for(m)) * m; }
+
+int prep_piece(const prep_batch &b, int tl0, int np, hipStream_t s) {
+    if (np <= 0) return SCS_OK;
+    const scs_tables *tb = b.tb;
+    int max_levels = 0;
+    int64_t max_n = 0;
+    for (int t = b.t0 + tl0; t < b.t0 + tl0 + np; ++t) {
+        const int64_t nt = tb->h_tree_off[t + 1] - tb->h_tree_off[t];
+        max_levels = std::max(max_levels, levels_for(nt - 1));
+        max_n = std::max(max_n, nt);
+    }
+    const dim3 grid_l((unsigned)((max_n + 255) / 256), (unsigned)np);
+    const dim3 grid_r((unsigned)b.n_blocks, (unsigned)np);
+    const bool fused = max_n <= SPARSE_FUSED_MAX_LEAVES && max_levels > 1;
+    if (b.kind != PREP_GEN) {
+        double *st = (double *)b.st;
+        k_positions_values<<<grid_l, 256, 0, s>>>(tb->d_tree_off, tb->d_leaf_taxon, tb->d_adj_depth, tb->d_adj_val,
+                                                  tb->d_tree_w, b.t0, tl0, b.pos, b.npad, b.st_off, st);
+        if (fused)
+            k_sparse_levels_fused<double><<<(unsigned)np, 1024, 0, s>>>(tb->d_tree_off, b.t0, tl0, b.st_off, st, b.am_off,
+                                                                        b.am, pick_smaller_value{});
+        else
+            for (int k = 1; k < max_levels; ++k)
+                k_sparse_level<double><<<grid_l, 256, 0, s>>>(tb->d_tree_off, b.t0, tl0, k, b.st_off, st, b.am_off, b.am,
+                                                              pick_smaller_value{});
+        if (b.kind == PREP_WIDE)
+            k_block_records_wide<PIPE_NG><<<grid_r, 64, 0, s>>>(tb->d_tree_off, b.t0, tl0, b.nb, b.pos, b.npad, b.st_off, st,
+                                                          b.am_off, b.am, b.row_begin, b.row_end, b.rec);
+        else if (b.kind == PREP_MONO)
+            k_block_records_mono<<<grid_r, 64, 0, s>>>(tb->d_tree_off, b.t0, tl0, b.nb, b.pos, b.npad, b.st_off, st,
+                                                       b.am_off, b.am, b.row_begin, b.row_end, b.rec);
+    } else {
+        gap_entry *st = (gap_entry *)b.st;
+        k_positions_pairs<<<grid_l, 256, 0, s>>>(tb->d_tree_off, tb->d_leaf_taxon, tb->d_adj_depth, tb->d_adj_val,
+                                                 tb->d_tree_w, b.t0, tl0, b.pos, b.npad, b.st_off, st);
+        if (fused)
+            k_sparse_levels_fused<gap_entry><<<(unsigned)np, 1024, 0, s>>>(tb->d_tree_off, b.t0, tl0, b.st_off, st,
+                                                                           b.am_off, b.am, pick_shallower_pair{});
+        else
+            for (int k = 1; k < max_levels; ++k)
+                k_sparse_level<gap_entry><<<grid_l, 256, 0, s>>>(tb->d_tree_off, b.t0, tl0, k, b.st_off, st, b.am_off,
+                                                                 b.am, pick_shallower_pair{});
+        k_block_records_gen<<<grid_r, 64, 0, s>>>(tb->d_tree_off, b.t0, tl0, b.nb, b.pos, b.npad, b.st_off, st, b.am_off,
+                                                  b.am, b.row_begin, b.row_end, b.rec);
+    }
+    SCS_HIP_CHECK(hipGetLastError());
+    return SCS_OK;
+}
+
+struct pinned_ref {
+    scs_ctx *ctx;
+    hipStream_t stream;
+    void *p = nullptr;
+    bool in_flight = false;
+    pinned_ref(scs_ctx *c, hipStream_t s) : ctx(c), stream(s) {}
+    ~pinned_ref() {
+        if (!p) return;
+        if (in_flight) hipStreamSynchronize(stream);
+        scs_pinned_release(ctx, p);
+    }
+};
+
 }
 
 extern "C" int scs_pcg_build(scs_ctx *ctx, const scs_tables *tb, int32_t row_begin,
@@ -626,7 +786,6 @@
     if (const char *e = scs_dbg("SCS_TREE_PARALLEL")) tree_par = sym && !scatter && !tiles.empty() && atoi(e) != 0;
     const size_t cells_per_tree = tiles.size() * (size_t)SCS_TR * cols_per_tile * 8;
 
-    constexpr int PIPE_NG = 2;
     const size_t wide_min_tiles = 13;
     bool listed = monotone && !scatter && !tiles.empty() && tb->n_trees > 0 &&
                   (double)tb->n_leaves / ((double)tb->n_trees * std::max(n, 1)) < 1.0 / 64.0;
@@ -670,8 +829,6 @@
                                      hipMemcpyHostToDevice, s));
     }
 
-    auto table_entries = [](int64_t m) -> int64_t { return (int64_t)levels_for(m) * m; };
-
     const int M = tb->n_trees;
     std::vector<int> batch_start{0};
     {
@@ -701,8 +858,8 @@
         for (int t = 0; t < M; ++t) {
             const int64_t nt = tb->h_tree_off[t + 1] - tb->h_tree_off[t];
             const int64_t m = nt - 1;
-            const size_t need =
-                (size_t)table_entries(m) * entry_bytes + (size_t)npad * 4 + (size_t)n_blocks * rec_bytes;
+            const size_t need = (size_t)table_entries(m) * entry_bytes + (size_t)argmin_entries(m) * sizeof(argmin_t) +
+                                (size_t)npad * 4 + (size_t)n_blocks * rec_bytes;
             if ((used + need > ctx->ws_limit || t - batch_start.back() >= max_batch_trees ||
                  (t == arrived && batch_start.size() == 1)) &&
                 t > batch_start.back()) {
@@ -729,25 +886,41 @@
     int spec_batches = 0, spec_trees = 0;
     float spec_ms = 0.f;
     bool single_batch_spec = false;
-    pooled_buf d_pos(ctx, 1), d_st(ctx, 3), d_stoff(ctx, 4), d_rec(ctx, 5), d_cells(ctx, 6);
+    pooled_buf d_pos(ctx, 1), d_am(ctx, 2), d_st(ctx, 3), d_stoff(ctx, 4), d_rec(ctx, 5), d_cells(ctx, 6);
     dev_buf d_pcol(ctx), d_lists(ctx), d_list_cnt(ctx);
     int listed_batches = 0;
+    std::vector<size_t> off_at((size_t)n_batches + 1, 0);
+    for (int bi = 0; bi < n_batches; ++bi)
+        off_at[bi + 1] = off_at[bi] + 2 * (size_t)(batch_start[bi + 1] - batch_start[bi] + 1);
+    pinned_ref h_off(ctx, s);
+    SCS_TRY(scs_pinned_get(ctx, std::max<size_t>(off_at[n_batches], 2) * 8, &h_off.p));
+    {
+        int64_t *h = (int64_t *)h_off.p;
+        for (int bi = 0; bi < n_batches; ++bi) {
+            const int t0 = batch_start[bi], nb = batch_start[bi + 1] - t0;
+            int64_t *st_off = h + off_at[bi], *am_off = st_off + nb + 1;
+            st_off[0] = am_off[0] = 0;
+            for (int t = 0; t < nb; ++t) {
+                const int64_t m = tb->h_tree_off[t0 + t + 1] - tb->h_tree_off[t0 + t] - 1;
+                st_off[t + 1] = st_off[t] + table_entries(m);
+                am_off[t + 1] = am_off[t] + argmin_entries(m);
+            }
+        }
+        SCS_TRY(d_stoff.alloc(off_at[n_batches] * 8));
+        h_off.in_flight = true;
+        SCS_HIP_CHECK(hipMemcpyAsync(d_stoff.p, h, off_at[n_batches] * 8, hipMemcpyHostToDevice, s));
+    }
+    const bool by_arrival = !(scs_dbg("SCS_PREP_BY_ARRIVAL") && atoi(scs_dbg("SCS_PREP_BY_ARRIVAL")) == 0);
+    int prep_pieces = 0;
     for (int bi = 0; bi < n_batches; ++bi) {
         const int t0 = batch_start[bi], t1 = batch_start[bi + 1];
         const int nb = t1 - t0;
-        std::vector<int64_t> st_off(nb + 1);
-        int max_levels = 0;
+        const int64_t *h_st_off = (const int64_t *)h_off.p + off_at[bi], *h_am_off = h_st_off + nb + 1;
         int64_t max_n = 0;
-        st_off[0] = 0;
-        for (int t = t0; t < t1; ++t) {
-            const int64_t nt = tb->h_tree_off[t + 1] - tb->h_tree_off[t];
-            st_off[t - t0 + 1] = st_off[t - t0] + table_entries(nt - 1);
-            max_levels = std::max(max_levels, levels_for(nt - 1));
-            max_n = std::max(max_n, nt);
-        }
+        for (int t = t0; t < t1; ++t) max_n = std::max(max_n, tb->h_tree_off[t + 1] - tb->h_tree_off[t]);
         const size_t need_pos = (size_t)nb * npad * 4;
-        const size_t need_st = (size_t)st_off[nb] * entry_bytes + 64;
-        const size_t need_stoff = (size_t)(nb + 1) * 8;
+        const size_t need_st = (size_t)h_st_off[nb] * entry_bytes + 64;
+        const size_t need_am = (size_t)h_am_off[nb] * sizeof(argmin_t) + 64;
         const size_t need_rec = (size_t)n_blocks * nb * rec_bytes;
         const int wide_min_trees = wide_forced ? 1 : 96;
         const bool wide_b = wide && (nb >= wide_min_trees || (groups.size() >= 8 * 256 && nb >= 16));
@@ -758,51 +931,35 @@
         }
         SCS_TRY(d_pos.alloc(need_pos));
         SCS_TRY(d_st.alloc(need_st));
-        SCS_TRY(d_stoff.alloc(need_stoff));
+        SCS_TRY(d_am.alloc(need_am));
         SCS_TRY(d_rec.alloc(need_rec));
 
         SCS_HIP_CHECK(hipEventRecord(ev_prep.a, s));
-        SCS_TRY(scs_tables_wait(ctx, tb, t1, s));
-        SCS_HIP_CHECK(hipMemcpyAsync(d_stoff.p, st_off.data(), need_stoff, hipMemcpyHostToDevice, s));
         SCS_HIP_CHECK(hipMemsetAsync(d_pos.p, 0xFF, need_pos, s));
-        dim3 grid_l((unsigned)((max_n + 255) / 256), (unsigned)nb);
-        if (monotone) {
-            k_positions_values<<<grid_l, 256, 0, s>>>(tb->d_tree_off, tb->d_leaf_taxon,
-                                                      tb->d_adj_depth, tb->d_adj_val, tb->d_tree_w,
-                                                      t0, (int32_t *)d_pos.p, npad,
-                                                      (const int64_t *)d_stoff.p, (double *)d_st.p);
-            if (max_n <= SPARSE_FUSED_MAX_LEAVES && max_levels > 1)
-                k_sparse_levels_fused<double><<<(unsigned)nb, 1024, 0, s>>>(
-                    tb->d_tree_off, t0, (const int64_t *)d_stoff.p, (double *)d_st.p, pick_smaller_value{});
-            else
-            for (int k = 1; k < max_levels; ++k)
-                k_sparse_level<double><<<grid_l, 256, 0, s>>>(tb->d_tree_off, t0, k,
-                                                              (const int64_t *)d_stoff.p,
-                                                              (double *)d_st.p);
-            if (wide_b)
-                k_block_records_wide<PIPE_NG><<<dim3((unsigned)n_blocks, (unsigned)nb), 64, 0, s>>>(
-                    tb->d_tree_off, t0, nb, (const int32_t *)d_pos.p, npad, (const int64_t *)d_stoff.p,
-                    (const double *)d_st.p, b_row_begin, b_row_end, (unsigned char *)d_rec.p);
-            else if (!scatter)
-            k_block_records_mono<<<dim3((unsigned)n_blocks, (unsigned)nb), 64, 0, s>>>(
-                tb->d_tree_off, t0, nb, (const int32_t *)d_pos.p, npad, (const int64_t *)d_stoff.p,
-                (const double *)d_st.p, b_row_begin, b_row_end, (unsigned char *)d_rec.p);
-        } else {
-            k_positions_pairs<<<grid_l, 256, 0, s>>>(tb->d_tree_off, tb->d_leaf_taxon,
-                                                     tb->d_adj_depth, tb->d_adj_val, tb->d_tree_w,
-                                                     t0, (int32_t *)d_pos.p, npad,
-                                                     (const int64_t *)d_stoff.p, (gap_entry *)d_st.p);
-            if (max_n <= SPARSE_FUSED_MAX_LEAVES && max_levels > 1)
-                k_sparse_levels_fused<gap_entry><<<(unsigned)nb, 1024, 0, s>>>(
-                    tb->d_tree_off, t0, (const int64_t *)d_stoff.p, (gap_entry *)d_st.p, pick_shallower_pair{});
-            else
-            for (int k = 1; k < max_levels; ++k)
-                k_sparse_level_pairs<<<grid_l, 256, 0, s>>>(tb->d_tree_off, t0, k,
-                                                            (const int64_t *)d_stoff.p,
-                                                            (gap_entry *)d_st.p);
-            k_block_records_gen<<<dim3((unsigned)n_blocks, (unsigned)nb), 64, 0, s>>>(
-                tb->d_tree_off, t0, nb, (const int32_t *)d_pos.p, npad, (const int64_t *)d_stoff.p,
-                (const gap_entry *)d_st.p, b_row_begin, b_row_end, (unsigned char *)d_rec.p);
+        prep_batch pb;
+        pb.tb = tb;
+        pb.t0 = t0;
+        pb.nb = nb;
+        pb.kind = !monotone ? PREP_GEN : wide_b ? PREP_WIDE : scatter ? PREP_NO_RECORDS : PREP_MONO;
+        pb.pos = (int32_t *)d_pos.p;
+        pb.npad = npad;
+        pb.st_off = (const int64_t *)d_stoff.p + off_at[bi];
+        pb.am_off = pb.st_off + nb + 1;
+        pb.st = d_st.p;
+        pb.am = (argmin_t *)d_am.p;
+        pb.rec = (unsigned char *)d_rec.p;
+        pb.n_blocks = n_blocks;
+        pb.row_begin = b_row_begin;
+        pb.row_end = b_row_end;
+        for (int p0 = t0; p0 < t1;) {
+            int p1 = t1;
+            if (by_arrival)
+                for (const int32_t c : tb->late_start)
+                    if (c > p0 && c < p1) p1 = c;
+            SCS_TRY(scs_tables_wait(ctx, tb, p1, s));
+            SCS_TRY(prep_piece(pb, p0 - t0, p1 - p0, s));
+            ++prep_pieces;
+            p0 = p1;
         }
         SCS_HIP_CHECK(hipEventRecord(ev_prep.b, s));
 
@@ -811,7 +968,7 @@
         if (scatter) {
             const int64_t nbk = (max_n + 63) / 64;
             k_scatter_atomic<<<dim3((unsigned)(nbk * (nbk + 1) / 2), (unsigned)nb), 256, 0, s>>>(
-                tb->d_tree_off, tb->d_leaf_taxon, t0, (const int64_t *)d_stoff.p, (const double *)d_st.p,
+                tb->d_tree_off, tb->d_leaf_taxon, t0, pb.st_off, (const double *)d_st.p,
                 g->d_w, g->ld);
         } else if (monotone) {
             mono_params mp;
@@ -1029,6 +1186,7 @@
     }
     SCS_HIP_CHECK(hipEventRecord(ev_total.b, s));
     SCS_HIP_CHECK(hipEventSynchronize(ev_total.b));
+    h_off.in_flight = false;
     SCS_TRY(scs_tables_finish(ctx, tb));
     float total_ms = 0.f;
     SCS_HIP_CHECK(hipEventElapsedTime(&total_ms, ev_total.a, ev_total.b));
@@ -1053,6 +1211,7 @@
         stats->tree_parallel_batches = tree_par ? n_batches : 0;
         stats->spec_trees = spec_trees;
         stats->listed_batches = listed_batches;
+        stats->prep_pieces = prep_pieces;
         stats->spec_ms = spec_ms;
         stats->cell_trees = (double)tiles.size() * SCS_TR * cols_per_tile * (double)M;
         stats->prep_ms = prep_ms;
@@ -1331,3 +1490,72 @@
         SCS_HIP_CHECK(hipMemcpy(out, g->d_w, (size_t)rows * (size_t)g->ld * 8, hipMemcpyDeviceToHost));
     return SCS_OK;
 }
+
+extern "C" int scs_debug_block_records(scs_ctx *ctx, const scs_tables *tb, int32_t t_begin, int32_t t_end,
+                                       int32_t row_begin, int32_t row_end, int32_t kind, int32_t *spos_out,
+                                       double *gap_out, int32_t *argpos_out, int32_t *depth_out, int32_t *cnt_out) {
+    SCS_REQUIRE(ctx && tb && spos_out && gap_out && argpos_out && cnt_out, "scs_debug_block_records: null argument");
+    SCS_REQUIRE(kind == PREP_MONO || kind == PREP_WIDE || kind == PREP_GEN,
+                "scs_debug_block_records: kind must be 0 (mono), 1 (wide) or 2 (general), not %d", kind);
+    SCS_REQUIRE(t_begin >= 0 && t_begin < t_end && t_end <= tb->n_trees,
+                "scs_debug_block_records: bad tree range [%d, %d) of %d", t_begin, t_end, tb->n_trees);
+    SCS_REQUIRE(row_begin >= 0 && row_begin < row_end && row_end <= tb->n_taxa,
+                "scs_debug_block_records: bad row range [%d, %d) for %d taxa", row_begin, row_end, tb->n_taxa);
+    SCS_HIP_CHECK(hipSetDevice(ctx->device));
+    hipStream_t s = ctx->stream;
+    const int n = tb->n_taxa, nb = t_end - t_begin;
+    const int n_blocks = (row_end - row_begin + SCS_TR - 1) / SCS_TR;
+    const int n_cgroups = (n + MONO_TCW - 1) / MONO_TCW;
+    const int64_t npad = scs_round_up((int64_t)n_cgroups * MONO_TCW, SCS_NPAD);
+    const size_t entry_bytes = kind == PREP_GEN ? sizeof(gap_entry) : 8;
+    const size_t rec_bytes = kind == PREP_GEN ? G3_BYTES : kind == PREP_WIDE ? wide_layout<PIPE_NG>::BYTES : R3_BYTES;
+    std::vector<int64_t> off(2 * (size_t)(nb + 1), 0);
+    int64_t *st_off = off.data(), *am_off = off.data() + nb + 1;
+    for (int t = 0; t < nb; ++t) {
+        const int64_t m = tb->h_tree_off[t_begin + t + 1] - tb->h_tree_off[t_begin + t] - 1;
+        st_off[t + 1] = st_off[t] + table_entries(m);
+        am_off[t + 1] = am_off[t] + argmin_entries(m);
+    }
+    dev_buf d_pos(ctx), d_st(ctx), d_am(ctx), d_off(ctx), d_rec(ctx);
+    const size_t need_pos = (size_t)nb * npad * 4, need_rec = (size_t)n_blocks * nb * rec_bytes;
+    SCS_TRY(d_pos.alloc(need_pos));
+    SCS_TRY(d_st.alloc((size_t)st_off[nb] * entry_bytes + 64));
+    SCS_TRY(d_am.alloc((size_t)am_off[nb] * sizeof(argmin_t) + 64));
+    SCS_TRY(d_off.alloc(off.size() * 8));
+    SCS_TRY(d_rec.alloc(need_rec));
+    SCS_HIP_CHECK(hipMemcpy(d_off.p, off.data(), off.size() * 8, hipMemcpyHostToDevice));
+    SCS_HIP_CHECK(hipMemsetAsync(d_pos.p, 0xFF, need_pos, s));
+    prep_batch pb;
+    pb.tb = tb;
+    pb.t0 = t_begin;
+    pb.nb = nb;
+    pb.kind = kind;
+    pb.pos = (int32_t *)d_pos.p;
+    pb.npad = npad;
+    pb.st_off = (const int64_t *)d_off.p;
+    pb.am_off = pb.st_off + nb + 1;
+    pb.st = d_st.p;
+    pb.am = (argmin_t *)d_am.p;
+    pb.rec = (unsigned char *)d_rec.p;
+    pb.n_blocks = n_blocks;
+    pb.row_begin = row_begin;
+    pb.row_end = row_end;
+    SCS_TRY(scs_tables_wait(ctx, tb, t_end, s));
+    SCS_TRY(prep_piece(pb, 0, nb, s));
+    std::vector<unsigned char> rec(need_rec);
+    SCS_HIP_CHECK(hipMemcpyAsync(rec.data(), d_rec.p, need_rec, hipMemcpyDeviceToHost, s));
+    SCS_HIP_CHECK(hipStreamSynchronize(s));
+    const int o_spos = kind == PREP_GEN ? G3_SPOS : kind == PREP_WIDE ? wide_layout<PIPE_NG>::SPOS : R3_SPOS;
+    const int o_gap = kind == PREP_GEN ? G3_GV : kind == PREP_WIDE ? wide_layout<PIPE_NG>::G : R3_G;
+    const int o_arg = kind == PREP_GEN ? G3_ARGPOS : kind == PREP_WIDE ? wide_layout<PIPE_NG>::ARGPOS : R3_ARGPOS;
+    const int o_cnt = kind == PREP_GEN ? G3_CNT : kind == PREP_WIDE ? wide_layout<PIPE_NG>::CNT : R3_CNT;
+    for (size_t i = 0; i < (size_t)n_blocks * nb; ++i) {
+        const unsigned char *r = rec.data() + i * rec_bytes;
+        memcpy(spos_out + i * 64, r + o_spos, 256);
+        memcpy(gap_out + i * 64, r + o_gap, 512);
+        memcpy(argpos_out + i * 64, r + o_arg, 256);
+        if (kind == PREP_GEN && depth_out) memcpy(depth_out + i * 64, r + G3_GD, 256);
+        memcpy(cnt_out + i, r + o_cnt, 4);
+    }
+    return SCS_OK;
+}
diff --git a/spectralclustersupertree_amd/csrc/scs_gen.h b/spectralclustersupertree_amd/csrc/scs_gen.h
--- a/spectralclustersupertree_amd/csrc/scs_gen.h
+++ b/spectralclustersupertree_amd/csrc/scs_gen.h
@@ -42,10 +42,10 @@
                                   const int32_t *__restrict__ leaf_taxon,
                                   const int32_t *__restrict__ adj_depth,
                                   const double *__restrict__ adj_val,
-                                  const double *__restrict__ tree_w, int t0,
+                                  const double *__restrict__ tree_w, int t0, int tl0,
                                   int32_t *__restrict__ pos, int64_t npad,
                                   const int64_t *__restrict__ st_off, gap_entry *__restrict__ ste) {
-    const int tl = blockIdx.y;
+    const int tl = tl0 + blockIdx.y;
     const int t = t0 + tl;
     const int64_t off = tree_off[t];
     const int n = (int)(tree_off[t + 1] - off);
@@ -62,24 +62,13 @@
     }
 }
 
-__global__ void k_sparse_level_pairs(const int64_t *__restrict__ tree_off, int t0, int k,
-                                     const int64_t *__restrict__ st_off,
-                                     gap_entry *__restrict__ ste) {
-    const int tl = blockIdx.y;
-    const int m = (int)(tree_off[t0 + tl + 1] - tree_off[t0 + tl]) - 1;
-    const int p = blockIdx.x * blockDim.x + threadIdx.x;
-    if (m < (1 << k) || p > m - (1 << k)) return;
-    gap_entry *base = ste + st_off[tl];
-    base[(int64_t)k * m + p] =
-        gap_min(base[(int64_t)(k - 1) * m + p], base[(int64_t)(k - 1) * m + p + (1 << (k - 1))]);
-}
-
 __global__ __launch_bounds__(64) void k_block_records_gen(
-    const int64_t *__restrict__ tree_off, int t0, int n_batch, const int32_t *__restrict__ pos,
+    const int64_t *__restrict__ tree_off, int t0, int tl0, int n_batch, const int32_t *__restrict__ pos,
     int64_t npad, const int64_t *__restrict__ st_off, const gap_entry *__restrict__ ste,
+    const int64_t *__restrict__ am_off, const argmin_t *__restrict__ am_all,
     int row_begin, int row_end, unsigned char *__restrict__ rec_all) {
     const int blk = blockIdx.x;
-    const int tl = blockIdx.y;
+    const int tl = tl0 + blockIdx.y;
     const int lane = threadIdx.x;
     const int m = (int)(tree_off[t0 + tl + 1] - tree_off[t0 + tl]) - 1;
     const int row = row_begin + blk * SCS_TR + lane;
@@ -106,16 +95,26 @@
     double gv = 0.0;
     int argpos = 0;
     if (lane < cnt - 1) {
-        const gap_entry g = rmq_gap(st, m, spos, next_pos);
+        int o[2];
+        rmq_offsets(m, spos, next_pos, o);
+        const int k = 31 - __clz(next_pos - spos);
+        const gap_entry x = st[o[0]], y = st[o[1]];
+        const gap_entry g = gap_min(x, y);
         gd = g.d;
         gv = g.v();
-        int lo = spos, hi = next_pos;
-        while (hi - lo > 1) {
-            const int mid = (lo + hi) >> 1;
-            if (rmq_gap(st, m, lo, mid).d == gd) hi = mid;
-            else lo = mid;
-        }
-        argpos = lo;
+        if (k == 0) {
+            argpos = spos;
+        } else if (k <= ARGMIN_MAX_LEVEL) {
+            argpos = argmin_position(am_all + am_off[tl], m, k, spos, next_pos, y.d < x.d);
+        } else {
+            int lo = spos, hi = next_pos;
+            while (hi - lo > 1) {
+                const int mid = (lo + hi) >> 1;
+                if (rmq_gap(st, m, lo, mid).d == gd) hi = mid;
+                else lo = mid;
+            }
+            argpos = lo;
+        }
     }
     unsigned char *rec = rec_all + ((int64_t)blk * n_batch + tl) * G3_BYTES;
     ((int *)(rec + G3_SPOS))[lane] = spos;
diff --git a/spectralclustersupertree_amd/csrc/scs_mono.h b/spectralclustersupertree_amd/csrc/scs_mono.h
--- a/spectralclustersupertree_amd/csrc/scs_mono.h
+++ b/spectralclustersupertree_amd/csrc/scs_mono.h
@@ -30,11 +30,12 @@
     } while (0)
 
 __global__ __launch_bounds__(64) void k_block_records_mono(
-    const int64_t *__restrict__ tree_off, int t0, int n_batch, const int32_t *__restrict__ pos,
+    const int64_t *__restrict__ tree_off, int t0, int tl0, int n_batch, const int32_t *__restrict__ pos,
     int64_t npad, const int64_t *__restrict__ st_off, const double *__restrict__ stv,
+    const int64_t *__restrict__ am_off, const argmin_t *__restrict__ am_all,
     int row_begin, int row_end, unsigned char *__restrict__ rec_all) {
     const int blk = blockIdx.x;
-    const int tl = blockIdx.y;
+    const int tl = tl0 + blockIdx.y;
     const int lane = threadIdx.x;
     const int m = (int)(tree_off[t0 + tl + 1] - tree_off[t0 + tl]) - 1;
     const int row = row_begin + blk * SCS_TR + lane;
@@ -59,16 +60,7 @@
     const double *st = stv + st_off[tl];
     double g = 0.0;
     int argpos = 0;
-    if (lane < cnt - 1) {
-        g = rmq_min<double>(st, m, spos, next_pos);
-        int lo = spos, hi = next_pos;
-        while (hi - lo > 1) {
-            const int mid = (lo + hi) >> 1;
-            if (rmq_min<double>(st, m, lo, mid) == g) hi = mid;
-            else lo = mid;
-        }
-        argpos = lo;
-    }
+    if (lane < cnt - 1) g = rmq_min_at(st, am_all + am_off[tl], m, spos, next_pos, argpos);
     unsigned char *rec = rec_all + ((int64_t)blk * n_batch + tl) * R3_BYTES;
     ((int *)(rec + R3_SPOS))[lane] = spos;
     ((double *)(rec + R3_G))[lane] = g;
diff --git a/spectralclustersupertree_amd/csrc/scs_mono_wide.h b/spectralclustersupertree_amd/csrc/scs_mono_wide.h
--- a/spectralclustersupertree_amd/csrc/scs_mono_wide.h
+++ b/spectralclustersupertree_amd/csrc/scs_mono_wide.h
@@ -22,12 +22,13 @@
 
 template <int NG>
 __global__ __launch_bounds__(64) void k_block_records_wide(
-    const int64_t *__restrict__ tree_off, int t0, int n_batch, const int32_t *__restrict__ pos,
+    const int64_t *__restrict__ tree_off, int t0, int tl0, int n_batch, const int32_t *__restrict__ pos,
     int64_t npad, const int64_t *__restrict__ st_off, const double *__restrict__ stv,
+    const int64_t *__restrict__ am_off, const argmin_t *__restrict__ am_all,
     int row_begin, int row_end, unsigned char *__restrict__ rec_all) {
     using L = wide_layout<NG>;
     const int blk = blockIdx.x;
-    const int tl = blockIdx.y;
+    const int tl = tl0 + blockIdx.y;
     const int lane = threadIdx.x;
     const int m = (int)(tree_off[t0 + tl + 1] - tree_off[t0 + tl]) - 1;
     const int row = row_begin + blk * SCS_TR + lane;
@@ -52,16 +53,7 @@
     const double *st = stv + st_off[tl];
     double g = 0.0;
     int argpos = 0;
-    if (lane < cnt - 1) {
-        g = rmq_min<double>(st, m, spos, next_pos);
-        int lo = spos, hi = next_pos;
-        while (hi - lo > 1) {
-            const int mid = (lo + hi) >> 1;
-            if (rmq_min<double>(st, m, lo, mid) == g) hi = mid;
-            else lo = mid;
-        }
-        argpos = lo;
-    }
+    if (lane < cnt - 1) g = rmq_min_at(st, am_all + am_off[tl], m, spos, next_pos, argpos);
     unsigned char *rec = rec_all + ((int64_t)blk * n_batch + tl) * L::BYTES;
     ((int *)(rec + L::SPOS))[lane] = spos;
     ((double *)(rec + L::G))[lane] = g;
```
